# titu1994/tfdiffeq

Hardware: AMD Instinct MI355X
Metric: state-elements/sec (batch x dim / wall-s) Dopri5 float64 (higher is better)
Workload: dtype f64

## Files before the change

include/mi_ode.h:

```cpp
#ifndef MI_ODE_H
#define MI_ODE_H

#include <stddef.h>
#include <stdint.h>

#ifdef __cplusplus
extern "C" {
#endif

#define MI_ODE_ABI_VERSION 13
#define MI_ODE_MAX_STAGES 13
#define MI_ODE_MAX_K (MI_ODE_MAX_STAGES + 1)
#define MI_ODE_MAX_LINCOMB 14
#define MI_ODE_MAX_SEGMENTS 8

#define MI_ODE_OK 0
#define MI_ODE_ST_DT_UNDERFLOW 0x1u
#define MI_ODE_ST_NONFINITE 0x2u
#define MI_ODE_ST_MAX_STEPS 0x4u
#define MI_ODE_ST_SYNC_TIMEOUT 0x10u
#define MI_ODE_ST_BAD_T 0x8u
#define MI_ODE_E_INVALID (-1)
#define MI_ODE_E_HIP (-2)
#define MI_ODE_E_NODEVICE (-3)
// ... 77 lines not shown
  double seg_rtol[MI_ODE_MAX_SEGMENTS], seg_atol[MI_ODE_MAX_SEGMENTS];
  int32_t multistep;
  int32_t ms_max_order;
  int32_t ms_max_iters;
  int32_t ms_min_order;
  const double* ms_ab;
  const double* ms_am;
  const double* ms_am0;
  const double* ms_gamma_star;
} mi_ode_desc;
#define MI_ODE_SEGMENT_ALIGN 256

typedef struct mi_ode_stats {
  int64_t n_attempts, n_accepted, n_rejected, nfe;
  double t, dt;
  double last_ratio;
  uint32_t status;
  int32_t n_polls;
  int64_t n_launches;
  double clock_mhz;
  double handoff_us;
} mi_ode_stats;

typedef struct mi_ode_solver* mi_ode_handle;

int mi_ode_abi_version(void);
const char* mi_ode_status_string(uint32_t status_bits);
const char* mi_ode_last_error(void);
int64_t mi_ode_reduce_workspace_bytes(void);
int64_t mi_ode_sizeof(int32_t which);

int mi_ode_create(const mi_ode_desc* desc, mi_ode_handle* out);
int mi_ode_destroy(mi_ode_handle h);

int mi_ode_begin(mi_ode_handle h, const void* y0_dev, double t0, void* stream);
int mi_ode_advance(mi_ode_handle h, const double* t_out_host, int32_t n_out, void* out_dev, void* stream);
int mi_ode_integrate(mi_ode_handle h, const void* y0_dev, const double* t_host, int32_t T, void* out_dev,
                     mi_ode_stats* stats, void* stream);
int mi_ode_integrate_rows(mi_ode_handle h, const void* rows_plugin, const void* y0_dev, const double* t_host, int32_t T,
                          void* out_dev, int64_t* row_stats_dev, mi_ode_stats* stats, void* stream);
int mi_ode_integrate_rows_t(mi_ode_handle h, const void* rows_t_plugin, const void* y0_dev, const double* t_dev, int32_t T,
                            const int32_t* len_dev, const double* rtol_dev, const double* atol_dev, void* out_dev,
                            int64_t* row_stats_dev, mi_ode_stats* stats, void* stream);
int mi_ode_integrate_fixed_rows_t(mi_ode_handle h, const void* fixed_rows_t_plugin, const void* y0_dev, const double* t_dev, int32_t T,
                                  const int32_t* len_dev, void* out_dev, mi_ode_stats* stats, void* stream);
int mi_ode_fixed_grid_integrate(mi_ode_handle h, const void* y0_dev, const double* t_host, int32_t T,
                                void* out_dev, mi_ode_stats* stats, void* stream);
int mi_ode_fixed_grid_integrate_on(mi_ode_handle h, const void* y0_dev, const double* grid_host, int32_t G,
                                   const double* t_host, int32_t T, double eps, void* out_dev, mi_ode_stats* stats, void* stream);
int mi_ode_rk_step_fused(mi_ode_handle h, const void* y0_dev, const void* f0_dev, double t0, double dt,
                         void* y1_dev, void* f1_dev, double* err_norms_host, void* k_out_dev, void* stream);
int mi_ode_eval_rhs(mi_ode_handle h, const void* y_dev, double t, void* f_dev, void* stream);
int mi_ode_get_stats(mi_ode_handle h, mi_ode_stats* stats, void* stream);
int mi_ode_get_profile(mi_ode_handle h, double* out4);
int mi_ode_get_state(mi_ode_handle h, void* y_dev, void* f_dev, void* stream);

int64_t mi_ode_xrank_bytes(int32_t world_size);
int mi_ode_xrank_selftest(mi_ode_handle h, void* stream);
int mi_ode_xrank_enable(mi_ode_handle h, int32_t on);

#define MI_ODE_IPC_HANDLE_BYTES 64
int mi_ode_xpeer_prepare(mi_ode_handle h, void* ipc_handle_out);
int mi_ode_xpeer_connect(mi_ode_handle h, const void* all_ipc_handles, int32_t world_size);

#define MI_ODE_RCCL_ID_BYTES 128
int mi_ode_rccl_unique_id(void* id_out);
int mi_ode_rccl_connect(mi_ode_handle h, const void* id, int32_t world_size, int32_t rank);

typedef struct mi_ode_adjoint_desc {
  int64_t batch;
  int32_t dim, hidden;
  mi_ode_tableau tableau;
  double rtol, atol;
  double safety, ifactor, dfactor;
  int32_t order, init_order;
  int64_t max_num_steps;
  int32_t time_dependent;
  int32_t reserved;
} mi_ode_adjoint_desc;
typedef struct mi_ode_adjoint* mi_ode_adjoint_handle;
int mi_ode_adjoint_create(const mi_ode_adjoint_desc* desc, mi_ode_adjoint_handle* out);
int mi_ode_adjoint_destroy(mi_ode_adjoint_handle h);
int64_t mi_ode_adjoint_num_params(mi_ode_adjoint_handle h);
int mi_ode_adjoint_segment(mi_ode_adjoint_handle h, const mi_ode_rhs* rhs, const void* y_dev, const void* adj_y_dev,
                           const void* adj_t_dev, const void* adj_params_dev, double t_start, double t_end, void* y_out_dev,
                           void* adj_y_out_dev, void* adj_t_out_dev, void* adj_params_out_dev, mi_ode_stats* stats, void* stream);
int mi_ode_adjoint_dynamics(mi_ode_adjoint_handle h, const mi_ode_rhs* rhs, const void* y_dev, const void* adj_y_dev,
                            void* f_out_dev, void* vjp_y_out_dev, void* vjp_params_out_dev, void* stream);
int mi_ode_adjoint_dynamics_at(mi_ode_adjoint_handle h, const mi_ode_rhs* rhs, double t, const void* y_dev, const void* adj_y_dev,
                               void* f_out_dev, void* vjp_y_out_dev, void* vjp_params_out_dev, void* stream);

int64_t mi_ode_outer_workspace_bytes(int32_t dtype, int64_t batch, int32_t dim);
int mi_ode_outer_reduce(int32_t dtype, int64_t batch, int32_t dim, const void* y_dev, const void* a_dev, double scale,
                        void* out_w_dev, void* out_b_dev, void* workspace_dev, void* stream);

typedef struct mi_ode_linadj_desc {
  int64_t batch;
  int32_t dim;
  int32_t dtype;
  mi_ode_tableau tableau;
  double rtol, atol;
  double safety, ifactor, dfactor;
  int32_t order, init_order;
  int64_t max_num_steps;
} mi_ode_linadj_desc;
typedef struct mi_ode_linadj* mi_ode_linadj_handle;
// ... 267 lines not shown
```

tfdiffeq_amd/_native.py:

```python
import ctypes as C
import os
import subprocess

_HERE = os.path.dirname(os.path.abspath(__file__))
LIB_PATH = os.environ.get('TFDIFFEQ_AMD_LIB') or os.path.join(_HERE, 'libmi_ode.so')
CSRC = os.path.join(_HERE, 'csrc')

MAX_STAGES = 13
MAX_K = MAX_STAGES + 1
MAX_LINCOMB = 14
REC = 8

F32, F64 = 0, 1
RHS_LINEAR, RHS_CUBIC_LINEAR, RHS_LOTKA_VOLTERRA, RHS_LORENZ, RHS_MLP_TANH, RHS_PLUGIN = 1, 2, 3, 4, 5, 6
CTRL_MISC, CTRL_TSIT5 = 0, 1
INTERP_QUARTIC_MID, INTERP_TSIT5, INTERP_TSIT5_REF = 0, 1, 2
ABI_VERSION = 13
MAX_SEGMENTS = 8
SEGMENT_ALIGN = 256
IPC_HANDLE_BYTES = 64
RCCL_ID_BYTES = 128
ST_DT_UNDERFLOW, ST_NONFINITE, ST_MAX_STEPS, ST_BAD_T, ST_SYNC_TIMEOUT = 1, 2, 4, 8, 16
E_INVALID, E_HIP, E_NODEVICE, E_EXCHANGE = -1, -2, -3, -4

# ... 143 lines not shown

class ConvDesc(C.Structure):
    _fields_ = [('dtype', C.c_int32), ('activation', C.c_int32), ('time_dependent', C.c_int32), ('reserved', C.c_int32),
                ('sign', C.c_double), ('batch', C.c_int64),
                ('channels', C.c_int32), ('height', C.c_int32), ('width', C.c_int32), ('filters', C.c_int32),
                ('w1', C.c_void_p), ('b1', C.c_void_p), ('w2', C.c_void_p), ('w2t', C.c_void_p), ('b2', C.c_void_p),
                ('w3', C.c_void_p), ('b3', C.c_void_p)]


class Stats(C.Structure):
    _fields_ = [('n_attempts', C.c_int64), ('n_accepted', C.c_int64), ('n_rejected', C.c_int64), ('nfe', C.c_int64),
                ('t', C.c_double), ('dt', C.c_double), ('last_ratio', C.c_double),
                ('status', C.c_uint32), ('n_polls', C.c_int32), ('n_launches', C.c_int64), ('clock_mhz', C.c_double),
                ('handoff_us', C.c_double)]

    def as_dict(self):
        return {k: getattr(self, k) for k, _ in self._fields_}


_PROTOS = {
    'mi_ode_abi_version': (C.c_int, []),
    'mi_ode_status_string': (C.c_char_p, [C.c_uint32]),
    'mi_ode_last_error': (C.c_char_p, []),
    'mi_ode_reduce_workspace_bytes': (C.c_int64, []),
    'mi_ode_sizeof': (C.c_int64, [C.c_int32]),
    'mi_ode_create': (C.c_int, [C.POINTER(Desc), C.POINTER(C.c_void_p)]),
    'mi_ode_destroy': (C.c_int, [C.c_void_p]),
    'mi_ode_begin': (C.c_int, [C.c_void_p, C.c_void_p, C.c_double, C.c_void_p]),
    'mi_ode_advance': (C.c_int, [C.c_void_p, C.POINTER(C.c_double), C.c_int32, C.c_void_p, C.c_void_p]),
    'mi_ode_integrate': (C.c_int, [C.c_void_p, C.c_void_p, C.POINTER(C.c_double), C.c_int32, C.c_void_p,
                                   C.POINTER(Stats), C.c_void_p]),
    'mi_ode_integrate_rows': (C.c_int, [C.c_void_p, C.c_void_p, C.c_void_p, C.POINTER(C.c_double), C.c_int32, C.c_void_p, C.c_void_p,
                                        C.POINTER(Stats), C.c_void_p]),
    'mi_ode_integrate_rows_t': (C.c_int, [C.c_void_p, C.c_void_p, C.c_void_p, C.c_void_p, C.c_int32, C.c_void_p, C.c_void_p, C.c_void_p,
                                          C.c_void_p, C.c_void_p, C.POINTER(Stats), C.c_void_p]),
    'mi_ode_integrate_fixed_rows_t': (C.c_int, [C.c_void_p, C.c_void_p, C.c_void_p, C.c_void_p, C.c_int32, C.c_void_p, C.c_void_p,
                                                C.POINTER(Stats), C.c_void_p]),
    'mi_ode_fixed_grid_integrate': (C.c_int, [C.c_void_p, C.c_void_p, C.POINTER(C.c_double), C.c_int32, C.c_void_p,
                                              C.POINTER(Stats), C.c_void_p]),
    'mi_ode_fixed_grid_integrate_on': (C.c_int, [C.c_void_p, C.c_void_p, C.POINTER(C.c_double), C.c_int32, C.POINTER(C.c_double), C.c_int32,
                                                 C.c_double, C.c_void_p, C.POINTER(Stats), C.c_void_p]),
    'mi_ode_rk_step_fused': (C.c_int, [C.c_void_p, C.c_void_p, C.c_void_p, C.c_double, C.c_double, C.c_void_p,
                                       C.c_void_p, C.POINTER(C.c_double), C.c_void_p, C.c_void_p]),
    'mi_ode_eval_rhs': (C.c_int, [C.c_void_p, C.c_void_p, C.c_double, C.c_void_p, C.c_void_p]),
    'mi_ode_xrank_bytes': (C.c_int64, [C.c_int32]),
    'mi_ode_xrank_selftest': (C.c_int, [C.c_void_p, C.c_void_p]),
    'mi_ode_xrank_enable': (C.c_int, [C.c_void_p, C.c_int32]),
    'mi_ode_xpeer_prepare': (C.c_int, [C.c_void_p, C.c_void_p]),
    'mi_ode_xpeer_connect': (C.c_int, [C.c_void_p, C.c_void_p, C.c_int32]),
    'mi_ode_rccl_unique_id': (C.c_int, [C.c_void_p]),
    'mi_ode_rccl_connect': (C.c_int, [C.c_void_p, C.c_void_p, C.c_int32, C.c_int32]),
    'mi_ode_get_stats': (C.c_int, [C.c_void_p, C.POINTER(Stats), C.c_void_p]),
    'mi_ode_get_state': (C.c_int, [C.c_void_p, C.c_void_p, C.c_void_p, C.c_void_p]),
    'mi_ode_get_profile': (C.c_int, [C.c_void_p, C.POINTER(C.c_double)]),
    'mi_ode_adjoint_create': (C.c_int, [C.POINTER(AdjointDesc), C.POINTER(C.c_void_p)]),
    'mi_ode_adjoint_destroy': (C.c_int, [C.c_void_p]),
    'mi_ode_adjoint_num_params': (C.c_int64, [C.c_void_p]),
    'mi_ode_adjoint_segment': (C.c_int, [C.c_void_p, C.POINTER(Rhs), C.c_void_p, C.c_void_p, C.c_void_p, C.c_void_p, C.c_double, C.c_double,
                                         C.c_void_p, C.c_void_p, C.c_void_p, C.c_void_p, C.POINTER(Stats), C.c_void_p]),
    'mi_ode_adjoint_dynamics': (C.c_int, [C.c_void_p, C.POINTER(Rhs), C.c_void_p, C.c_void_p, C.c_void_p, C.c_void_p, C.c_void_p,
                                          C.c_void_p]),
    'mi_ode_adjoint_dynamics_at': (C.c_int, [C.c_void_p, C.POINTER(Rhs), C.c_double, C.c_void_p, C.c_void_p, C.c_void_p, C.c_void_p,
                                             C.c_void_p, C.c_void_p]),
    'mi_ode_outer_workspace_bytes': (C.c_int64, [C.c_int32, C.c_int64, C.c_int32]),
    'mi_ode_outer_reduce': (C.c_int, [C.c_int32, C.c_int64, C.c_int32, C.c_void_p, C.c_void_p, C.c_double, C.c_void_p, C.c_void_p,
                                      C.c_void_p, C.c_void_p]),
    'mi_ode_linadj_create': (C.c_int, [C.POINTER(LinAdjDesc), C.POINTER(C.c_void_p)]),
    'mi_ode_linadj_destroy': (C.c_int, [C.c_void_p]),
    'mi_ode_linadj_segment': (C.c_int, [C.c_void_p, C.c_void_p, C.c_void_p, C.c_void_p, C.c_void_p, C.c_void_p, C.c_void_p, C.c_void_p, C.c_double,
                                        C.c_double, C.c_void_p, C.c_void_p, C.c_void_p, C.c_void_p, C.POINTER(C.c_double), C.POINTER(Stats), C.c_void_p]),
    'mi_ode_linadj_profile': (C.c_int, [C.c_void_p, C.POINTER(C.c_double)]),
    'mi_ode_discrete_create': (C.c_int, [C.POINTER(DiscreteDesc), C.POINTER(C.c_void_p)]),
    'mi_ode_discrete_create_td': (C.c_int, [C.POINTER(DiscreteDesc), C.c_int32, C.POINTER(C.c_void_p)]),
    'mi_ode_discrete_destroy': (C.c_int, [C.c_void_p]),
    'mi_ode_discrete_num_params': (C.c_int64, [C.c_void_p]),
    'mi_ode_discrete_sweep': (C.c_int, [C.c_void_p, C.POINTER(Rhs), C.POINTER(C.c_double), C.c_void_p, C.c_void_p, C.c_void_p, C.c_void_p,
                                        C.POINTER(Stats), C.c_void_p]),
    'mi_ode_discrete64_create': (C.c_int, [C.POINTER(DiscreteDesc), C.c_int32, C.POINTER(C.c_void_p)]),
    'mi_ode_discrete64_destroy': (C.c_int, [C.c_void_p]),
    'mi_ode_discrete64_num_params': (C.c_int64, [C.c_void_p]),
    'mi_ode_discrete64_sweep': (C.c_int, [C.c_void_p, C.POINTER(Rhs), C.POINTER(C.c_double), C.c_void_p, C.c_void_p, C.c_void_p, C.c_void_p,
                                          C.POINTER(Stats), C.c_void_p]),
    'mi_ode_discrete64_profile': (C.c_int, [C.c_void_p, C.POINTER(C.c_double)]),
    'mi_ode_discrete_row_sweep': (C.c_int, [C.POINTER(DiscreteRowDesc), C.POINTER(Rhs), C.c_void_p, C.c_void_p, C.c_void_p, C.c_void_p,
                                            C.POINTER(Stats), C.c_void_p]),
    'mi_ode_discrete_row_sweep_t': (C.c_int, [C.POINTER(DiscreteRowTDesc), C.POINTER(Rhs), C.c_void_p, C.c_void_p, C.c_void_p, C.c_void_p,
                                              C.POINTER(Stats), C.c_void_p]),
    'mi_ode_discrete_row_t_sizeof': (C.c_int64, []),
    'mi_ode_adjoint_rows': (C.c_int, [C.POINTER(AdjointRowsDesc), C.POINTER(Rhs), C.c_void_p, C.c_void_p, C.c_void_p, C.c_void_p, C.c_void_p,
                                      C.POINTER(Stats), C.c_void_p]),
    'mi_ode_adjoint_rows_sizeof': (C.c_int64, []),
    'mi_ode_adjoint_rows_t': (C.c_int, [C.POINTER(AdjointRowsTDesc), C.POINTER(Rhs), C.c_void_p, C.c_void_p, C.c_void_p, C.c_void_p,
                                        C.POINTER(Stats), C.c_void_p]),
    'mi_ode_adjoint_rows_t_sizeof': (C.c_int64, []),
    'mi_ode_discrete_linear_create': (C.c_int, [C.POINTER(DiscreteLinearDesc), C.POINTER(C.c_void_p)]),
    'mi_ode_discrete_linear_destroy': (C.c_int, [C.c_void_p]),
    'mi_ode_discrete_linear_sweep': (C.c_int, [C.c_void_p, C.POINTER(Rhs), C.POINTER(C.c_double), C.c_void_p, C.c_void_p, C.c_void_p, C.c_void_p,
                                               C.c_void_p, C.POINTER(Stats), C.c_void_p]),
    'mi_ode_discrete_linear_profile': (C.c_int, [C.c_void_p, C.POINTER(C.c_double)]),
    'mi_ode_discrete_linear_grid_validate': (C.c_int, [C.POINTER(DiscreteLinearGridDesc), C.POINTER(C.c_double), C.POINTER(C.c_int32),
                                                       C.POINTER(C.c_double)]),
    'mi_ode_discrete_linear_grid_create': (C.c_int, [C.POINTER(DiscreteLinearGridDesc), C.POINTER(C.c_void_p)]),
    'mi_ode_discrete_linear_grid_destroy': (C.c_int, [C.c_void_p]),
    'mi_ode_discrete_linear_grid_sweep': (C.c_int, [C.c_void_p, C.POINTER(Rhs), C.POINTER(C.c_double), C.POINTER(C.c_int32), C.POINTER(C.c_double),
                                                    C.c_void_p, C.c_void_p, C.c_void_p, C.c_void_p, C.c_void_p, C.POINTER(Stats), C.c_void_p]),
    'mi_ode_discrete_linear_grid_profile': (C.c_int64, [C.c_void_p, C.POINTER(C.c_double), C.POINTER(C.c_int64)]),
# ... 146 lines not shown
```

tfdiffeq_amd/csrc/mi_ode_api.hip:

```cpp
#include <dlfcn.h>
#include <math.h>
#include <stdarg.h>
#include <stdio.h>
#include <stdlib.h>
#include <string.h>

#include "mi_ode_control.h"
#include "mi_ode_host.h"
#include "mi_ode_plane.h"
#include "mi_ode_step_fused.h"
#include "mi_ode_persist.h"
#include "mi_ode_adams.h"
#include "mi_ode_adams_vc.h"
#include "mi_ode_adams_planes.h"
#include "mi_ode_mlp.h"
#include "mi_ode_plugin.h"

using namespace mi;

static thread_local char g_err[512] = "";

void mi_set_error(const char* fmt, ...) {
  va_list ap;
  va_start(ap, fmt);
  vsnprintf(g_err, sizeof(g_err), fmt, ap);
  va_end(ap);
}

extern "C" const char* mi_ode_last_error(void) { return g_err; }
extern "C" int mi_ode_abi_version(void) { return MI_ODE_ABI_VERSION; }

extern "C" const char* mi_ode_status_string(uint32_t s) {
  if (s & MI_ODE_ST_BAD_T) return "t must be strictly increasing or decrasing";
  if (s & MI_ODE_ST_NONFINITE) return "non-finite values in state `y`";
  if (s & MI_ODE_ST_MAX_STEPS) return "max_num_steps exceeded";
  if (s & MI_ODE_ST_DT_UNDERFLOW) return "underflow in dt";
  if (s & MI_ODE_ST_SYNC_TIMEOUT) return "engine: grid hand-off timed out (whole-integration kernel)";
  return "ok";
}

extern "C" int64_t mi_ode_reduce_workspace_bytes(void) { return (int64_t)kMaxBlocks * kRec * sizeof(double); }
extern "C" int64_t mi_ode_sizeof(int32_t which) {
  switch (which) {
    case 0: return (int64_t)sizeof(mi_ode_desc);
    case 1: return (int64_t)sizeof(mi_ode_stats);
    case 2: return (int64_t)sizeof(mi_ode_tableau);
    case 3: return (int64_t)sizeof(mi_ode_rhs);
    case 4: return (int64_t)sizeof(mi_ode_solver);
    case 5: return (int64_t)sizeof(mi_ode_ctrl_params);
    case 6: return (int64_t)sizeof(mi_ode_adjoint_desc);
    case 7: return (int64_t)sizeof(mi_ode_opq_desc);
    case 8: return (int64_t)sizeof(mi_ode_linadj_desc);
    case 9: return (int64_t)sizeof(mi_ode_discrete_desc);
    case 10: return (int64_t)sizeof(mi_ode_discrete_row_desc);
    case 11: return (int64_t)sizeof(mi_ode_discrete_linear_desc);
    case 12: return (int64_t)sizeof(mi_ode_discrete_linear_grid_desc);
    default: return -1;
  }
}

typedef int (*nccl_get_unique_id_fn)(void*);
// ... 279 lines not shown
      if (!h->d.adaptive && (h->d.multistep != 0 || (h->d.tableau.n_stages != 0 && h->d.tableau.n_stages != 3))) {
        mi_set_error("fused MLP kernels on a fixed grid: euler or rk4 (3/8 rule) in one launch (k_fixed_mlp); no multistep kernel");
        return MI_ODE_E_INVALID;
      }
      if (D < 1 || D > 64 || hd < 1 || hd > 128 || !r.w[0] || !r.w[1] || !r.w[2]) {
        mi_set_error("fused MLP kernel supports dim <= 64, hidden <= 128 (got %d, %d)", D, hd);
        return MI_ODE_E_INVALID;
      }
      h->mlp_dp = D <= 16 ? 16 : 64;
      h->mlp_hp = hd <= 16 ? 16 : 128;
      if (!h->is_f32 && h->mlp_dp != (h->mlp_hp == 16 ? 16 : 64)) { h->mlp_dp = 64; h->mlp_hp = 128; }
      h->family = FAM_MLP; return 0;
    }
    default:
      mi_set_error("RHS kind %d has no fused kernel yet", r.kind);
      return MI_ODE_E_INVALID;
  }
}

static bool multistep_family(const mi_ode_solver* h) {
  const bool rowlocal = h->family == FAM_CUBIC2 || h->family == FAM_LINEAR2 || h->family == FAM_LV || h->family == FAM_LORENZ ||
                        h->family == FAM_PLUGIN;
  const bool coop = (h->family == FAM_LINEAR_MFMA || h->family == FAM_LINEAR_VALU) && h->d.dim >= 1 && h->d.dim <= 256;
  return rowlocal || coop || h->family == FAM_MLP_COOP || h->family == FAM_PLUGIN_COOP;
}
static long long multistep_grid(const mi_ode_solver* h) {
  if (h->family == FAM_LINEAR_MFMA || h->family == FAM_LINEAR_VALU) {
    const long long tpw = 256 / h->d.dim;
    return (h->d.batch + tpw - 1) / tpw;
  }
  if (h->family == FAM_MLP_COOP) {
    const long long tpw = RhsMlpCoop<float>::tpw(h->rhs, (int)h->d.dim);
    return (h->d.batch + tpw - 1) / tpw;
  }
  if (h->family == FAM_PLUGIN_COOP) {
    const long long tpw = 256 / h->d.dim;
    return (h->d.batch + tpw - 1) / tpw;
  }
  return (h->d.batch + 255) / 256;
}
static void multistep_rhs(const mi_ode_solver* h, RhsParams& r) {
  if (h->family == FAM_LINEAR_MFMA || h->family == FAM_LINEAR_VALU) r.hidden = (int)h->d.dim;
  if (h->family == FAM_MLP_COOP) r.cube = (int)h->d.dim;
}

static void fill_step_args(mi_ode_solver* h, StepArgs& A) {
  memset(&A, 0, sizeof(A));
  A.ctl = h->ctl; A.planes = h->planes; A.stride = h->stride; A.batch = h->d.batch; A.dim = (int)h->d.dim;
  A.interp = h->d.interp; A.out = h->cur_out; A.t_out = h->t_out_dev; A.n_plane = h->n;
  fill_tableau(A, h->d.tableau, h->S);
  A.partials = h->partials; A.rhs = h->rhs;
  A.ticket = h->fused_ctl ? h->ticket : nullptr;
  A.cp = h->cp;
}

static void fill_mlp_args(mi_ode_solver* h, MlpArgs& M) {
  memset(&M, 0, sizeof(M));
  fill_step_args(h, M.step);
  M.rtol = h->d.rtol; M.atol = h->d.atol; M.hidden = h->d.rhs.hidden;
}

static void close_peers(mi_ode_solver* h) {
  for (int q = 0; q < h->xpeer_world && q < 64; ++q)
    if (h->xpeer_open[q] != nullptr && h->xpeer_open[q] != h->xpeer_local) (void)hipIpcCloseMemHandle(h->xpeer_open[q]);
  memset(h->xpeer_open, 0, sizeof(h->xpeer_open));
  h->xpeer_world = 0;
  if (h->xpeer_tab_dev) { (void)hipFree(h->xpeer_tab_dev); h->xpeer_tab_dev = nullptr; }
}

extern "C" int mi_ode_destroy(mi_ode_handle h) {
  if (h != nullptr) {
    close_peers(h);
    if (h->xpeer_local) { (void)hipFree(h->xpeer_local); h->xpeer_local = nullptr; }
    if (h->nccl_comm && g_nccl.ok) { (void)g_nccl.destroy(h->nccl_comm); h->nccl_comm = nullptr; }
  }
  if (h != nullptr && h->xrank_registered) { (void)hipHostUnregister(h->d.xrank_host); h->xrank_registered = 0; }
  if (h != nullptr && h->gbuf) { (void)hipFree(h->gbuf); h->gbuf = nullptr; }
  if (h == nullptr) return 0;
  if (h->planes) (void)hipFree(h->planes);
  if (h->partials) (void)hipFree(h->partials);
  if (h->adams_tab) (void)hipFree(h->adams_tab);
  if (h->mlp_pack) (void)hipFree(h->mlp_pack);
  if (h->lin_pack) (void)hipFree(h->lin_pack);
  if (h->adams_res) (void)hipHostFree(h->adams_res);
  if (h->rank_rec && h->own_exchange) (void)hipFree(h->rank_rec);
  if (h->gathered && h->own_exchange) (void)hipFree(h->gathered);
  if (h->ctl) (void)hipFree(h->ctl);
  if (h->ticket) (void)hipFree(h->ticket);
  if (h->t_out_dev) (void)hipFree(h->t_out_dev);
  if (h->ev_ready) for (int i = 0; i < 64; ++i) { (void)hipEventDestroy(h->ev_a[i]); (void)hipEventDestroy(h->ev_b[i]); (void)hipEventDestroy(h->ev_c[i]); }
  if (h->ctl_host) (void)hipHostFree(h->ctl_host);
  if (h->t_out_host) (void)hipHostFree(h->t_out_host);
  delete h;
  return 0;
}

extern "C" int mi_ode_create(const mi_ode_desc* desc, mi_ode_handle* out) {
  if (desc == nullptr || out == nullptr) { mi_set_error("null argument"); return MI_ODE_E_INVALID; }
  *out = nullptr;
  int ndev = 0;
  if (hipGetDeviceCount(&ndev) != hipSuccess || ndev == 0) { mi_set_error("no HIP device"); return MI_ODE_E_NODEVICE; }
  if (desc->dtype != MI_ODE_F32 && desc->dtype != MI_ODE_F64) { mi_set_error("bad dtype"); return MI_ODE_E_INVALID; }
  if (desc->batch <= 0 || desc->dim <= 0) { mi_set_error("empty state"); return MI_ODE_E_INVALID; }
  const mi_ode_tableau& tb = desc->tableau;
  if (tb.n_stages < 0 || tb.n_stages > MI_ODE_MAX_STAGES) { mi_set_error("bad n_stages"); return MI_ODE_E_INVALID; }
  if (desc->adaptive) {
    const bool classic = tb.fsal && (tb.n_stages == 3 || tb.n_stages == 6);
    const bool wide = (tb.fsal && tb.n_stages == 13) || (!tb.fsal && tb.n_stages == 1);
    if (!classic && !wide && desc->multistep != 3) { mi_set_error("fused adaptive engine: no kernels for a %d-row %s tableau", tb.n_stages, tb.fsal ? "FSAL-shaped" : "non-FSAL"); return MI_ODE_E_INVALID; }
    if (desc->interp != MI_ODE_INTERP_QUARTIC_MID && tb.n_stages != 6) { mi_set_error("tsit5 dense output needs 7 stage derivatives"); return MI_ODE_E_INVALID; }
  }
  mi_ode_solver* h = new mi_ode_solver();
  memset(h, 0, sizeof(*h));
  h->d = *desc;
  if (h->d.world_size < 1) h->d.world_size = 1;
  h->is_f32 = desc->dtype == MI_ODE_F32;
  h->elt = h->is_f32 ? 4 : 8;
  h->n = desc->batch * desc->dim;
  h->stride = ((h->n * (long long)h->elt + 255) / 256) * 256;
  h->S = tb.n_stages;
  int dev = 0;
  hipDeviceProp_t prop;
  if (hipGetDevice(&dev) != hipSuccess || hipGetDeviceProperties(&prop, dev) != hipSuccess) {
    mi_set_error("cannot query device");
    mi_ode_destroy(h);
    return MI_ODE_E_HIP;
  }
  h->num_cus = prop.multiProcessorCount;
  fill_rhs(h->rhs, desc->rhs);
  h->rhs.sign = desc->rhs.sign == 0.0 ? 1.0 : desc->rhs.sign;
  int rc = pick_family(h);
  if (rc != 0) { mi_ode_destroy(h); return rc; }
  if (h->family == FAM_LINEAR_MFMA && h->lin_dp == 256) {
    if (hipMalloc(&h->lin_pack, (size_t)256 * 256 * (size_t)h->elt) != hipSuccess) {
      (void)hipGetLastError();
      mi_set_error("linear tile kernels (dim > 128): cannot allocate the copy of W");
// ... 52 lines not shown
      if (g > cap || g > kPersistMaxGrid) {
        mi_set_error("adams in one launch: %lld workgroups cannot be co-resident on this device (%d)", g, cap);
        mi_ode_destroy(h); return MI_ODE_E_INVALID;
      }
    }
    memcpy(h->adams_gamma_star, desc->ms_gamma_star, sizeof(h->adams_gamma_star));
    hipError_t ea = hipHostMalloc((void**)&h->adams_res, 4 * sizeof(long long), hipHostMallocDefault);
    if (ea != hipSuccess) { mi_set_error("multistep result record: %s", hipGetErrorString(ea)); mi_ode_destroy(h); return MI_ODE_E_HIP; }
    for (int i = 0; i < 4; ++i) h->adams_res[i] = 0;
    h->d.ms_gamma_star = nullptr;
  } else
  if (desc->multistep != 0) {
    const bool rowlocal_cat = multistep_family(h);
    if (desc->adaptive || !rowlocal_cat || (desc->multistep != 1 && desc->multistep != 2) || desc->ms_ab == nullptr || desc->ms_am == nullptr ||
        desc->ms_am0 == nullptr || desc->ms_max_order < 1 || desc->ms_max_order > kAdamsMaxOrder || desc->ms_max_iters < 1 ||
        desc->ms_min_order < 1 || h->d.world_size > 1 || h->nseg > 1) {
      mi_set_error("multistep: fixed grid, a row-local catalogue system or a matrix RHS of dim <= 256, one rank, one tensor; 1 <= max_order <= %d, max_iters >= 1, coefficient tables", kAdamsMaxOrder);
      mi_ode_destroy(h); return MI_ODE_E_INVALID;
    }
    const long long g = multistep_grid(h);
    if (desc->multistep == 2 && g > 1) {
      const int cap = h->is_f32 ? mi_adams_capacity_f32(h) : mi_adams_capacity_f64(h);
      if (g > cap || g > kPersistMaxGrid) {
        mi_set_error("fixed_adams in one launch: %lld workgroups cannot be co-resident on this device (%d)", g, cap);
        mi_ode_destroy(h); return MI_ODE_E_INVALID;
      }
    }
    double tab[2 * 13 * 12 + 13];
    memcpy(tab, desc->ms_ab, sizeof(double) * 13 * 12);
    memcpy(tab + 13 * 12, desc->ms_am, sizeof(double) * 13 * 12);
    memcpy(tab + 2 * 13 * 12, desc->ms_am0, sizeof(double) * 13);
    hipError_t ea = hipMalloc((void**)&h->adams_tab, sizeof(tab));
    if (ea == hipSuccess) ea = hipMemcpy(h->adams_tab, tab, sizeof(tab), hipMemcpyHostToDevice);
    if (ea == hipSuccess) ea = hipHostMalloc((void**)&h->adams_res, 2 * sizeof(long long), hipHostMallocDefault);
    if (ea != hipSuccess) { mi_set_error("multistep tables: %s", hipGetErrorString(ea)); mi_ode_destroy(h); return MI_ODE_E_HIP; }
    h->adams_res[0] = h->adams_res[1] = 0;
    h->d.ms_ab = h->d.ms_am = h->d.ms_am0 = nullptr;
  }
  {
    const bool can = desc->adaptive && (h->family == FAM_CUBIC2 || h->family == FAM_LINEAR2 || h->family == FAM_LV ||
                                        h->family == FAM_LORENZ || h->family == FAM_LINEAR_MFMA || h->family == FAM_MLP ||
                                        h->family == FAM_PLUGIN);
    if (h->family == FAM_PLUGIN && desc->fusion == 1) { mi_set_error("RHS plugins have no per-stage kernels (fusion = 1)"); mi_ode_destroy(h); return MI_ODE_E_INVALID; }
    if (h->family == FAM_MLP && desc->fusion == 1) { mi_set_error("the MLP family only has a whole-attempt kernel"); mi_ode_destroy(h); return MI_ODE_E_INVALID; }
    const bool can_fixed = !desc->adaptive && (h->family == FAM_CUBIC2 || h->family == FAM_LINEAR2 || h->family == FAM_LV ||
                                               h->family == FAM_LORENZ || h->family == FAM_LINEAR_MFMA || h->family == FAM_MLP ||
                                               h->family == FAM_PLUGIN);
    if (desc->fusion == 2 && !can && !can_fixed) { mi_set_error("fusion=2: no whole-attempt kernel for this problem"); mi_ode_destroy(h); return MI_ODE_E_INVALID; }
    h->step_fused = (can && desc->fusion != 1) ? 1 : 0;
    h->ts_dense = (desc->interp != MI_ODE_INTERP_QUARTIC_MID) ? 1 : 0;
    const bool light_many = (h->family != FAM_LINEAR_MFMA && h->family != FAM_MLP) && h->step_grid > 32;
    h->fused_ctl = (h->step_fused && h->d.world_size <= 1 && desc->allgather == nullptr && desc->fusion != 3 &&
                    !(light_many && desc->fusion == 0)) ? 1 : 0;
  }
  {
    const bool rowlocal = h->family == FAM_CUBIC2 || h->family == FAM_LINEAR2 || h->family == FAM_LV || h->family == FAM_LORENZ ||
                          h->family == FAM_PLUGIN;
    const bool mfma = h->family == FAM_LINEAR_MFMA && h->step_fused;
    const bool mlp = h->family == FAM_MLP;
    const bool coop = (h->family == FAM_MLP_COOP || h->family == FAM_PLUGIN_COOP) && desc->multistep == 0;
    h->init_tiles16 = mfma ? 1 : 0;
    long long g = (mfma || mlp) ? (long long)h->step_grid : coop ? multistep_grid(h) : (desc->batch + 255) / 256;
    const bool single = h->d.world_size <= 1 && desc->allgather == nullptr;
    if (desc->xrank_host != nullptr) {
      if (h->d.world_size > kXMaxWorld || desc->xrank_bytes < mi_ode_xrank_bytes(h->d.world_size)) {
        mi_set_error("xrank_host: world_size <= %d and at least %lld bytes are needed", kXMaxWorld, (long long)mi_ode_xrank_bytes(h->d.world_size));
        mi_ode_destroy(h); return MI_ODE_E_INVALID;
      }
      void* dptr = nullptr;
      hipError_t re = hipHostRegister(desc->xrank_host, (size_t)desc->xrank_bytes, hipHostRegisterMapped | hipHostRegisterPortable);
      if (re == hipSuccess) { h->xrank_registered = 1; re = hipHostGetDevicePointer(&dptr, desc->xrank_host, 0); }
      if (re != hipSuccess) {
        (void)hipGetLastError();
        if (h->xrank_registered) { (void)hipHostUnregister(desc->xrank_host); h->xrank_registered = 0; }
        dptr = nullptr;
      }
      h->xrank_dev = (double*)dptr;
    }
    const bool clamp_ok = mfma && single && (double)((desc->batch + 15) / 16) * (double)h->lin_dp * (double)h->lin_dp <= 8.0e6;
    if (clamp_ok && g > kPersistMaxGrid) g = kPersistMaxGrid;
    bool capable = desc->adaptive && (rowlocal || mfma || mlp || coop) && g <= kPersistMaxGrid;
    if (capable) {
      const int cap = mlp ? (h->is_f32 ? mi_persist_capacity_mlp_f32(h) : mi_persist_capacity_mlp_f64(h))
                          : (h->is_f32 ? mi_persist_capacity_f32(h) : mi_persist_capacity_f64(h));
      if (clamp_ok && cap > 0 && g > cap) g = cap;
      capable = cap > 0 && g <= cap;
    }
    if (!capable && desc->adaptive && (rowlocal || coop)) {
      h->persist_planes = 1;
      h->persist_planes_block = 256;
      if (const char* eb = getenv("MI_ODE_PERSIST_PLANES_BLOCK")) { const int v = atoi(eb); if ((v == 256 || v == 512) && !coop) h->persist_planes_block = v; }
      const int cap = h->is_f32 ? mi_persist_capacity_f32(h) : mi_persist_capacity_f64(h);
      long long gp = cap < kPersistMaxGrid ? cap : kPersistMaxGrid;
      if (gp > h->num_cus && !coop) gp = h->num_cus;
      if (const char* eg = getenv("MI_ODE_PERSIST_PLANES_GRID")) { const long long v = atoll(eg); if (v >= 1 && v <= gp) gp = v; }
      const long long gneed = coop ? multistep_grid(h) : (desc->batch + h->persist_planes_block - 1) / h->persist_planes_block;
      if (gp > gneed) gp = gneed;
      if (h->nseg > 1 && gp < h->nseg) gp = 0;
      if (cap > 0 && gp >= 1) { capable = true; g = gp; }
      else h->persist_planes = 0;
      if (h->persist_planes && h->nseg > 1) {
        long long total = 0;
        for (int k = 0; k < h->nseg; ++k) total += desc->seg_rows[k];
        int used = 0;
        for (int k = 0; k < h->nseg; ++k) {
          long long share = (long long)((double)g * (double)desc->seg_rows[k] / (double)total);
          const long long need = (desc->seg_rows[k] + h->persist_planes_block - 1) / h->persist_planes_block;
          if (share > need) share = need;
          if (share < 1) share = 1;
          const int left_for_rest = h->nseg - 1 - k;
          if (used + share > g - left_for_rest) share = g - left_for_rest - used;
          h->seg_blk[k] = used;
          used += (int)share;
        }
        h->seg_blk[h->nseg] = used;
        g = used;
      }
    }
    h->persist_capable = capable ? 1 : 0;
    const bool can = capable && (single || h->xrank_dev != nullptr);
    if (desc->fusion == 4 && !can && single) { mi_set_error("fusion=4: no whole-integration kernel for this problem (row-local or MFMA-linear RHS, single rank, every workgroup co-resident)"); mi_ode_destroy(h); return MI_ODE_E_INVALID; }
    h->persist = (can && (desc->fusion == 4 || desc->fusion == 0)) ? 1 : 0;
    if (coop && desc->adaptive && !h->persist) {
      mi_set_error("cooperative kernel: %lld workgroups cannot be co-resident on this device (the whole-call kernel is its only schedule)", g);
      mi_ode_destroy(h); return MI_ODE_E_INVALID;
    }
    if (h->nseg > 1 && !h->persist) {
      mi_set_error("tuple states run on the whole-call kernel only, and its grid (%lld workgroups) is not co-resident on this device", g);
      mi_ode_destroy(h); return MI_ODE_E_INVALID;
    }
    h->persist_grid = (int)g;
    h->persist_sleep_first = g <= 32 ? 16 : 32;
    h->persist_sleep_poll = 2;
    if (const char* e0 = getenv("MI_ODE_PERSIST_SLEEP0")) h->persist_sleep_first = atoi(e0);
    if (const char* e1 = getenv("MI_ODE_PERSIST_SLEEP1")) h->persist_sleep_poll = atoi(e1);
    h->persist_spin_limit = 1 << 17;
    h->persist_spin_first = 1 << 12;
    if (const char* e3 = getenv("MI_ODE_PERSIST_SPIN_FIRST")) h->persist_spin_first = atoi(e3);
    if (const char* e2 = getenv("MI_ODE_PERSIST_SPIN_LIMIT")) h->persist_spin_limit = atoi(e2);
    h->persist_xspin_limit = 1 << 22;
    if (const char* e4 = getenv("MI_ODE_PERSIST_XSPIN_LIMIT")) h->persist_xspin_limit = atoi(e4);
    if (getenv("MI_ODE_PERSIST_SPIN_LIMIT") && !getenv("MI_ODE_PERSIST_XSPIN_LIMIT")) h->persist_xspin_limit = h->persist_spin_limit;
  }
  h->cp.rtol = desc->rtol; h->cp.atol = desc->atol;
  h->cp.safety = desc->safety; h->cp.ifactor = desc->ifactor; h->cp.dfactor = desc->dfactor;
  h->cp.inv_ifactor = 1.0 / desc->ifactor; h->cp.inv_dfactor = 1.0 / desc->dfactor;
  h->cp.max_num_steps = desc->max_num_steps > 0 ? desc->max_num_steps : 2147483647LL;
  h->cp.n_local = h->n;
  h->cp.order = desc->order; h->cp.init_order = desc->init_order;
  h->cp.controller = desc->controller;
  h->cp.is_f32 = h->is_f32;
  h->cp.n_stages = h->S;
  h->cp.auto_first_step = isnan(desc->first_step) ? 1 : 0;
  h->ip.kind = desc->interp;
  h->ip.nk = h->S + 1;
  for (int j = 0; j < kMaxK; ++j) h->ip.c_mid[j] = tb.c_mid[j];
  hipError_t e = hipSuccess;
  e = hipMalloc((void**)&h->planes, (size_t)h->stride * (2 + h->S + 1));
  if (e == hipSuccess) e = hipMalloc((void**)&h->partials, (size_t)kMaxBlocks * kRec * sizeof(double));
  if (e == hipSuccess) e = hipMemset(h->partials, 0, (size_t)kMaxBlocks * kRec * sizeof(double));
  if (desc->exchange_send_dev != nullptr && desc->exchange_recv_dev != nullptr) {
    h->rank_rec = desc->exchange_send_dev;
    h->gathered = desc->exchange_recv_dev;
    h->own_exchange = 0;
  } else {
    h->own_exchange = 1;
    if (e == hipSuccess) e = hipMalloc((void**)&h->rank_rec, kRec * sizeof(double));
    if (e == hipSuccess) e = hipMalloc((void**)&h->gathered, (size_t)h->d.world_size * kRec * sizeof(double));
  }
  if (e == hipSuccess) e = hipMalloc((void**)&h->ctl, sizeof(Ctl));
  if (e == hipSuccess) e = hipMalloc((void**)&h->gbuf, 2 * kPRec * sizeof(double));
  if (e == hipSuccess) e = hipMemset(h->gbuf, 0, 2 * kPRec * sizeof(double));
  if (e == hipSuccess) e = hipMalloc((void**)&h->ticket, 64);
  if (e == hipSuccess) e = hipMemset(h->ticket, 0, 64);
  if (e == hipSuccess) e = hipHostMalloc((void**)&h->ctl_host, sizeof(Ctl), hipHostMallocDefault);
  if (e != hipSuccess) {
    mi_set_error("workspace allocation failed: %s", hipGetErrorString(e));
    mi_ode_destroy(h);
    return MI_ODE_E_HIP;
  }
  memset(h->ctl_host, 0, sizeof(Ctl));
  if (h->d.profile) {
    for (int i = 0; i < 64 && e == hipSuccess; ++i) {
      e = hipEventCreate(&h->ev_a[i]);
      if (e == hipSuccess) e = hipEventCreate(&h->ev_b[i]);
      if (e == hipSuccess) e = hipEventCreate(&h->ev_c[i]);
    }
    if (e != hipSuccess) { mi_set_error("event creation failed"); mi_ode_destroy(h); return MI_ODE_E_HIP; }
    h->ev_ready = 1;
  }
  *out = h;
  return 0;
}

static int ensure_t_out(mi_ode_solver* h, int n) {
  if (n > h->t_out_cap) {
    if (h->t_out_dev) (void)hipFree(h->t_out_dev);
    h->t_out_dev = nullptr;
    int cap = n < 64 ? 64 : n;
    MI_HIP(hipMalloc((void**)&h->t_out_dev, (size_t)cap * sizeof(double)));
    h->t_out_cap = cap;
  }
  if (n > h->t_out_host_cap) {
    if (h->t_out_host) (void)hipHostFree(h->t_out_host);
    h->t_out_host = nullptr;
    int cap = n < 64 ? 64 : n;
    MI_HIP(hipHostMalloc((void**)&h->t_out_host, (size_t)cap * sizeof(double), hipHostMallocDefault));
    h->t_out_host_cap = cap;
  }
  return 0;
}

static int begin_impl(mi_ode_handle h, const void* y0_dev, double t0, void* first_out_dev, void* stream);

extern "C" int mi_ode_begin(mi_ode_handle h, const void* y0_dev, double t0, void* stream) {
  return begin_impl(h, y0_dev, t0, nullptr, stream);
}

static int begin_impl(mi_ode_handle h, const void* y0_dev, double t0, void* first_out_dev, void* stream) {
  if (h == nullptr || y0_dev == nullptr) { mi_set_error("null argument"); return MI_ODE_E_INVALID; }
  if (!h->d.adaptive) { mi_set_error("mi_ode_begin on a fixed-grid handle"); return MI_ODE_E_INVALID; }
  if (h->d.multistep != 0) { mi_set_error("multistep handles run through mi_ode_integrate / mi_ode_fixed_grid_integrate only"); return MI_ODE_E_INVALID; }
  if (h->nseg > 1) { mi_set_error("tuple states: mi_ode_integrate with at least two times only (whole-call kernel)"); return MI_ODE_E_INVALID; }
  hipStream_t st = (hipStream_t)stream;
  MI_HIP(hipStreamSynchronize(st));
  Ctl* c = h->ctl_host;
  memset(c, 0, sizeof(Ctl));
  c->t0 = c->t1 = t0;
  c->dt = h->cp.auto_first_step ? 0.0 : h->d.first_step;
  c->idx_y0 = 0; c->idx_y1 = 1;
  for (int j = 0; j < kMaxK; ++j) c->idx_k[j] = 2 + j;
  h->n_launches = 0; h->n_polls = 0;
  h->enq_attempts = 0; h->prof_done = 0;
  MI_HIP(hipMemcpyAsync(h->ctl, c, sizeof(Ctl), hipMemcpyHostToDevice, st));
  if (h->family == FAM_MLP) {
    MlpArgs M;
    fill_mlp_args(h, M);
    M.x_y0 = y0_dev; M.copy_a = h->planes; M.copy_b = first_out_dev;
    int rcm = h->is_f32 ? mi_launch_mlp_f32(h, MLP_F0, M, st) : mi_launch_mlp_f64(h, MLP_F0, M, st);
    if (rcm != 0) return rcm;
    rcm = enqueue_controller(h, PH_F0, st);
    if (rcm != 0) return rcm;
    if (h->cp.auto_first_step) {
      fill_mlp_args(h, M);
      rcm = h->is_f32 ? mi_launch_mlp_f32(h, MLP_INITB, M, st) : mi_launch_mlp_f64(h, MLP_INITB, M, st);
      if (rcm != 0) return rcm;
      rcm = enqueue_controller(h, PH_INITB, st);
      if (rcm != 0) return rcm;
    }
    h->begun = 1;
    return 0;
  }
  if (h->init_tiles16) {
    InitArgs I;
    memset(&I, 0, sizeof(I));
    fill_step_args(h, I.s);
    I.y0 = y0_dev; I.copy_b = first_out_dev;
    int rci = h->is_f32 ? mi_launch_init_linear_f32(h, 0, I, st) : mi_launch_init_linear_f64(h, 0, I, st);
    if (rci != 0) return rci;
    rci = enqueue_controller(h, PH_F0, st);
    if (rci != 0) return rci;
    if (h->cp.auto_first_step) {
      rci = h->is_f32 ? mi_launch_init_linear_f32(h, 1, I, st) : mi_launch_init_linear_f64(h, 1, I, st);
      if (rci != 0) return rci;
      rci = enqueue_controller(h, PH_INITB, st);
      if (rci != 0) return rci;
    }
    h->begun = 1;
    return 0;
  }
  StageArgs A;
  fill_common(h, A);
  A.explicit_mode = 1; A.ctl = nullptr;
  A.x_y0 = y0_dev; A.x_t0 = t0; A.x_dt = 0.0;
  A.x_kout = h->planes + 2 * h->stride;
  A.copy_a = h->planes;
  A.copy_b = first_out_dev;
  int rc = launch_stage(h, M_F0, 0, A, st);
  if (rc != 0) return rc;
  rc = enqueue_controller(h, PH_F0, st);
  if (rc != 0) return rc;
  if (h->cp.auto_first_step) {
    fill_common(h, A);
    A.k_out_slot = 1;
    A.alpha = 1.0;
    rc = launch_stage(h, M_INITB, 1, A, st);
    if (rc != 0) return rc;
    rc = enqueue_controller(h, PH_INITB, st);
    if (rc != 0) return rc;
  }
  h->begun = 1;
  return 0;
}

extern "C" int mi_ode_advance(mi_ode_handle h, const double* t_out_host, int32_t n_out, void* out_dev, void* stream) {
  if (h == nullptr || (n_out > 0 && (t_out_host == nullptr || out_dev == nullptr))) { mi_set_error("null argument"); return MI_ODE_E_INVALID; }
  if (h->d.multistep != 0) { mi_set_error("multistep handles run through mi_ode_integrate / mi_ode_fixed_grid_integrate only"); return MI_ODE_E_INVALID; }
  if (!h->begun) { mi_set_error("mi_ode_advance before mi_ode_begin"); return MI_ODE_E_INVALID; }
  hipStream_t st = (hipStream_t)stream;
  if (n_out <= 0) return 0;
  for (int i = 1; i < n_out; ++i)
    if (!(t_out_host[i] > t_out_host[i - 1])) { mi_set_error("output times must increase"); return MI_ODE_ST_BAD_T; }
  int rc = ensure_t_out(h, n_out);
  if (rc != 0) return rc;
  if (h->t_out_busy) { MI_HIP(hipStreamSynchronize(st)); h->t_out_busy = 0; }
  memcpy(h->t_out_host, t_out_host, (size_t)n_out * sizeof(double));
  MI_HIP(hipMemcpyAsync(h->t_out_dev, h->t_out_host, (size_t)n_out * sizeof(double), hipMemcpyHostToDevice, st));
  h->cp.t_out = h->t_out_dev;
  h->cur_out = out_dev;
  MI_HIP(hipMemsetAsync(h->ticket, 0, 4, st));
// ... 267 lines not shown
      mi_set_error("hipIpcOpenMemHandle(rank %d) failed: %s", q, hipGetErrorString(e));
      close_peers(h);
      return MI_ODE_E_HIP;
    }
    h->xpeer_open[q] = p;
  }
  hipError_t e = hipMalloc((void**)&h->xpeer_tab_dev, (size_t)kXMaxWorld * sizeof(double*));
  if (e == hipSuccess) e = hipMemcpy(h->xpeer_tab_dev, h->xpeer_open, (size_t)world_size * sizeof(double*), hipMemcpyHostToDevice);
  if (e != hipSuccess) { mi_set_error("peer table upload failed: %s", hipGetErrorString(e)); close_peers(h); return MI_ODE_E_HIP; }
  return 0;
}

extern "C" int mi_ode_rccl_unique_id(void* id_out) {
  if (id_out == nullptr) { mi_set_error("null argument"); return MI_ODE_E_INVALID; }
  int rc = load_rccl();
  if (rc != 0) return rc;
  NcclUniqueId id;
  memset(&id, 0, sizeof(id));
  const int nrc = g_nccl.get_id(&id);
  if (nrc != 0) { mi_set_error("ncclGetUniqueId failed: %s", g_nccl.err ? g_nccl.err(nrc) : "?"); return MI_ODE_E_EXCHANGE; }
  memcpy(id_out, &id, sizeof(id));
  return 0;
}

extern "C" int mi_ode_rccl_connect(mi_ode_handle h, const void* id, int32_t world_size, int32_t rank) {
  if (h == nullptr) { mi_set_error("null argument"); return MI_ODE_E_INVALID; }
  if (id == nullptr) {
    if (h->nccl_comm && g_nccl.ok) (void)g_nccl.destroy(h->nccl_comm);
    h->nccl_comm = nullptr;
    return 0;
  }
  if (world_size != h->d.world_size || rank != h->d.rank) { mi_set_error("rccl_connect: world_size / rank differ from the handle's"); return MI_ODE_E_INVALID; }
  int rc = load_rccl();
  if (rc != 0) return rc;
  if (h->nccl_comm) { (void)g_nccl.destroy(h->nccl_comm); h->nccl_comm = nullptr; }
  NcclUniqueId uid;
  memcpy(&uid, id, sizeof(uid));
  void* comm = nullptr;
  const int nrc = g_nccl.init_rank(&comm, world_size, uid, rank);
  if (nrc != 0 || comm == nullptr) { mi_set_error("ncclCommInitRank failed: %s", g_nccl.err ? g_nccl.err(nrc) : "?"); return MI_ODE_E_EXCHANGE; }
  h->nccl_comm = comm;
  h->fused_ctl = 0;
  return 0;
}

extern "C" int mi_ode_get_stats(mi_ode_handle h, mi_ode_stats* stats, void* stream) {
  if (h == nullptr || stats == nullptr) { mi_set_error("null argument"); return MI_ODE_E_INVALID; }
  int rc = poll_ctl(h, (hipStream_t)stream);
  if (rc != 0) return rc;
  fill_stats(h, stats);
  return 0;
}

extern "C" int mi_ode_get_profile(mi_ode_handle h, double* out4) {
  if (h == nullptr || out4 == nullptr) { mi_set_error("null argument"); return MI_ODE_E_INVALID; }
  out4[0] = h->prof_last_ms; out4[1] = (double)h->prof_n; out4[2] = h->prof_all_ms; out4[3] = (double)h->prof_n;
  return 0;
}

extern "C" int mi_ode_get_state(mi_ode_handle h, void* y_dev, void* f_dev, void* stream) {
  if (h == nullptr) { mi_set_error("null argument"); return MI_ODE_E_INVALID; }
  if (h->d.multistep != 0) { mi_set_error("get_state: the one-launch multistep kernels keep their state in registers (the solution rows are the output)"); return MI_ODE_E_INVALID; }
  hipStream_t st = (hipStream_t)stream;
  int rc = poll_ctl(h, st);
  if (rc != 0) return rc;
  const Ctl* c = h->ctl_host;
  if (y_dev) MI_HIP(hipMemcpyAsync(y_dev, h->planes + (long long)c->idx_y0 * h->stride, (size_t)h->n * h->elt, hipMemcpyDeviceToDevice, st));
  if (f_dev) MI_HIP(hipMemcpyAsync(f_dev, h->planes + (long long)c->idx_k[0] * h->stride, (size_t)h->n * h->elt, hipMemcpyDeviceToDevice, st));
  return 0;
}

static int fixed_impl(mi_ode_handle h, const void* y0_dev, const double* grid_host, int32_t G, const double* t_host, int32_t T, double eps,
                      void* out_dev, mi_ode_stats* stats, void* stream);

extern "C" int mi_ode_fixed_grid_integrate(mi_ode_handle h, const void* y0_dev, const double* t_host, int32_t T,
                                           void* out_dev, mi_ode_stats* stats, void* stream) {
  return fixed_impl(h, y0_dev, t_host, T, t_host, T, 0.0, out_dev, stats, stream);
}

extern "C" int mi_ode_fixed_grid_integrate_on(mi_ode_handle h, const void* y0_dev, const double* grid_host, int32_t G,
                                              const double* t_host, int32_t T, double eps, void* out_dev, mi_ode_stats* stats,
                                              void* stream) {
  if (grid_host == nullptr || G < 1) { mi_set_error("bad grid"); return MI_ODE_E_INVALID; }
  return fixed_impl(h, y0_dev, grid_host, G, t_host, T, eps, out_dev, stats, stream);
}

static int fixed_impl(mi_ode_handle h, const void* y0_dev, const double* grid_host, int32_t G, const double* t_host, int32_t T, double eps,
                      void* out_dev, mi_ode_stats* stats, void* stream) {
  if (h == nullptr || y0_dev == nullptr || t_host == nullptr || out_dev == nullptr || T < 1) { mi_set_error("bad argument"); return MI_ODE_E_INVALID; }
  if (h->d.adaptive) { mi_set_error("fixed-grid call on an adaptive handle"); return MI_ODE_E_INVALID; }
  hipStream_t st = (hipStream_t)stream;
  const bool euler = h->S == 0;
  if (!euler && h->S != 3 && h->d.multistep == 0) { mi_set_error("fixed grid: tableau must be euler (0 rows) or rk4 3/8 (3 rows)"); return MI_ODE_E_INVALID; }
  for (int i = 1; i < T; ++i)
    if (!(t_host[i] > t_host[i - 1])) {
      if (stats) { memset(stats, 0, sizeof(*stats)); stats->status = MI_ODE_ST_BAD_T; }
      return MI_ODE_ST_BAD_T;
    }
  const bool own_grid = grid_host != t_host || eps != 0.0;
  if (own_grid) {
    for (int i = 1; i < G; ++i)
      if (!(grid_host[i] > grid_host[i - 1])) { mi_set_error("the time grid must increase"); return MI_ODE_ST_BAD_T; }
    if (!(grid_host[0] == t_host[0] && grid_host[G - 1] == t_host[T - 1])) {
      mi_set_error("the time grid must start at t[0] and end at t[-1]");
      return MI_ODE_ST_BAD_T;
    }
  }
  h->n_launches = 0; h->n_polls = 0;
  const size_t pbytes = (size_t)h->n * h->elt;
  if (h->d.multistep != 0 && (h->d.fusion == 1 || !multistep_family(h))) {
    mi_set_error("multistep handles run on the one-launch kernels only");
    return MI_ODE_E_INVALID;
  }
  if ((h->family == FAM_CUBIC2 || h->family == FAM_LINEAR2 || h->family == FAM_LV || h->family == FAM_LORENZ ||
       h->family == FAM_LINEAR_MFMA || h->family == FAM_MLP || h->family == FAM_PLUGIN ||
       h->family == FAM_MLP_COOP || h->family == FAM_PLUGIN_COOP || (h->family == FAM_LINEAR_VALU && h->d.multistep != 0)) && h->d.fusion != 1) {
    int rcf = ensure_t_out(h, T + (own_grid ? G : 0));
    if (rcf != 0) return rcf;
    MI_HIP(hipStreamSynchronize(st));
    memcpy(h->t_out_host, t_host, (size_t)T * sizeof(double));
// ... 432 lines not shown
```

tfdiffeq_amd/csrc/mi_ode_ctrl_dev.h:

```cpp
#pragma once
#include "mi_ode_dev.h"

namespace mi {

template <bool SC1>
__device__ __forceinline__ double rec_load(const double* p) {
  if constexpr (SC1) return __hip_atomic_load(p, __ATOMIC_RELAXED, __HIP_MEMORY_SCOPE_AGENT);
  else return *p;
}

template <bool SC1 = false>
__device__ __forceinline__ void reduce_block_records(const double* part, int nblocks, double* out ) {
  if (threadIdx.x < 64) {
    double v0 = 0, v1 = 0, v2 = 0, v3 = 0, v4 = 0;
    for (int b = threadIdx.x; b < nblocks; b += 64) {
      const double* p = part + (long long)b * kRec;
      v0 = fmax(v0, rec_load<SC1>(p + R_MAXA)); v1 = fmax(v1, rec_load<SC1>(p + R_MAXB));
      v2 += rec_load<SC1>(p + R_SUMA); v3 += rec_load<SC1>(p + R_SUMB); v4 = fmax(v4, rec_load<SC1>(p + R_FLAG));
    }
    v0 = wave_max(v0); v1 = wave_max(v1); v2 = wave_sum(v2); v3 = wave_sum(v3); v4 = wave_max(v4);
    if (threadIdx.x == 0) {
      out[R_MAXA] = v0; out[R_MAXB] = v1; out[R_SUMA] = v2; out[R_SUMB] = v3; out[R_FLAG] = v4;
      out[R_N] = 0; out[6] = 0; out[7] = 0;
    }
  }
}

__device__ __forceinline__ double nan_min(double a, double b) { return (isnan(a) || isnan(b)) ? NAN : fmin(a, b); }
__device__ __forceinline__ double nan_max(double a, double b) { return (isnan(a) || isnan(b)) ? NAN : fmax(a, b); }

__device__ __forceinline__ double optimal_step(double last_step, double ratio, const CtrlParams& P) {
  if (ratio == 0.0) return last_step * P.ifactor;
  const double inv_dfac = (ratio < 1.0) ? 1.0 : P.inv_dfactor;
  double er, expo;
  if (P.controller == MI_ODE_CTRL_TSIT5) {
    er = ratio;
    expo = 1.0 / (double)P.order;
  } else {
    er = P.is_f32 ? (double)sqrtf((float)ratio) : sqrt(ratio);
    expo = (double)(float)(1.0 / (double)P.order);
  }
  const double factor = nan_max(P.inv_ifactor, nan_min(pow(er, expo) / P.safety, inv_dfac));
  return last_step / factor;
}

struct AttemptState {
  double t0, t1, dt, ratio, emit_t0, emit_t1, emit_dt;
  long long n_attempt, n_accept, n_reject, nfe, n_steps_out;
  int next_out, n_out, emit_lo, emit_hi, done, accepted;
  unsigned status;
  __device__ __forceinline__ void load(const Ctl& c) {
    t0 = c.t0; t1 = c.t1; dt = c.dt; ratio = c.ratio; emit_t0 = c.emit_t0; emit_t1 = c.emit_t1; emit_dt = c.emit_dt;
    n_attempt = c.n_attempt; n_accept = c.n_accept; n_reject = c.n_reject; nfe = c.nfe; n_steps_out = c.n_steps_out;
    next_out = c.next_out; n_out = c.n_out; emit_lo = c.emit_lo; emit_hi = c.emit_hi; done = c.done; accepted = c.accepted;
    status = c.status;
  }
  __device__ __forceinline__ void store(Ctl& c) const {
    c.t0 = t0; c.t1 = t1; c.dt = dt; c.ratio = ratio; c.emit_t0 = emit_t0; c.emit_t1 = emit_t1; c.emit_dt = emit_dt;
    c.n_attempt = n_attempt; c.n_accept = n_accept; c.n_reject = n_reject; c.nfe = nfe; c.n_steps_out = n_steps_out;
    c.next_out = next_out; c.n_out = n_out; c.emit_lo = emit_lo; c.emit_hi = emit_hi; c.done = done; c.accepted = accepted;
    c.status = status;
  }
};

__device__ __forceinline__ double error_ratio(const double* rec, const CtrlParams& P) {
  const double N = rec[R_N];
  if (P.is_f32) {
    const float tol = (float)P.atol + (float)P.rtol * (float)fmax(rec[R_MAXA], rec[R_MAXB]);
    return (double)(float)(rec[R_SUMA] / (N * (double)tol * (double)tol));
  }
  const double tol = P.atol + P.rtol * fmax(rec[R_MAXA], rec[R_MAXB]);
  return rec[R_SUMA] / (N * tol * tol);
}

__device__ __forceinline__ void attempt_tail(AttemptState& c, double ratio, bool accept, const CtrlParams& P) {
  c.n_attempt += 1;
  c.nfe += P.n_stages;
  c.n_steps_out += 1;
  const double dt = c.dt, t_start = c.t1;
  c.ratio = ratio;
  const double dt_next = optimal_step(dt, ratio, P);
  c.accepted = accept ? 1 : 0;
  c.emit_lo = c.emit_hi = c.next_out;
  if (accept) {
    c.n_accept += 1;
    const double t_new = t_start + dt;
    c.emit_t0 = t_start; c.emit_t1 = t_new; c.emit_dt = dt;
    c.t0 = t_start; c.t1 = t_new;
    int nx = c.next_out;
    while (nx < c.n_out && !(P.t_out[nx] > t_new)) ++nx;
    if (nx > c.next_out) { c.emit_hi = nx; c.next_out = nx; c.n_steps_out = 0; }
  } else {
    c.n_reject += 1;
    c.t0 = t_start;
  }
  c.dt = dt_next;
  if (c.next_out >= c.n_out) { c.done = 1; return; }
  if (c.n_steps_out >= P.max_num_steps) { c.status |= MI_ODE_ST_MAX_STEPS; c.done = 1; return; }
  if (!(c.t1 + dt_next > c.t1)) { c.status |= MI_ODE_ST_DT_UNDERFLOW; c.done = 1; }
}

__device__ __forceinline__ void attempt_core(AttemptState& c, const double* rec, const CtrlParams& P) {
  const double ratio = error_ratio(rec, P);
  attempt_tail(c, ratio, ratio <= 1.0, P);
}

constexpr int kMaxSeg = MI_ODE_MAX_SEGMENTS;
struct SegState { double d1[kMaxSeg]; };

__device__ __forceinline__ double py_max(const double* v, int n) {
  double best = v[0];
  for (int i = 1; i < n; ++i)
    if (v[i] > best) best = v[i];
  return best;
}

__device__ __forceinline__ void controller_apply_seg(Ctl* c, SegState* ss, const double (*rec)[kRec], int nseg, int phase, const CtrlParams& P) {
  if (phase == PH_F0) {
    c->nfe += 1;
    double d0[kMaxSeg], d1[kMaxSeg], q[kMaxSeg];
    bool nonfinite = false;
    for (int k = 0; k < nseg; ++k) {
      const double N = rec[k][R_N];
      nonfinite = nonfinite || rec[k][R_FLAG] != 0.0;
      if (P.is_f32) {
        d0[k] = (double)(sqrtf((float)rec[k][R_SUMA]) / powf((float)N, 0.5f));
        d1[k] = (double)(sqrtf((float)rec[k][R_SUMB]) / powf((float)N, 0.5f));
        q[k] = (double)((float)d0[k] / (float)d1[k]);
      } else {
        d0[k] = sqrt(rec[k][R_SUMA]) / pow(N, 0.5);
        d1[k] = sqrt(rec[k][R_SUMB]) / pow(N, 0.5);
        q[k] = d0[k] / d1[k];
      }
      ss->d1[k] = d1[k];
    }
    c->y0_nonfinite = nonfinite;
    const double m0 = py_max(d0, nseg), m1 = py_max(d1, nseg);
    double h0;
    if (P.is_f32) h0 = ((float)m0 < 1e-5f || (float)m1 < 1e-5f) ? (double)1e-6f : (double)(0.01f * (float)py_max(q, nseg));
    else h0 = (m0 < 1e-5 || m1 < 1e-5) ? 1e-6 : 0.01 * py_max(q, nseg);
    c->d0 = d0[0]; c->d1 = d1[0]; c->h0 = h0;
    return;
  }
  if (phase == PH_INITB) {
    c->nfe += 1;
    double both[2 * kMaxSeg], d2[kMaxSeg];
    for (int k = 0; k < nseg; ++k) {
      const double N = rec[k][R_N];
      if (P.is_f32) d2[k] = (double)((sqrtf((float)rec[k][R_SUMA]) / powf((float)N, 0.5f)) / (float)c->h0);
      else d2[k] = (sqrt(rec[k][R_SUMA]) / pow(N, 0.5)) / c->h0;
      both[k] = ss->d1[k]; both[nseg + k] = d2[k];
    }
    double first;
    if (P.is_f32) {
      const float h0 = (float)c->h0;
      float h1;
      if ((float)py_max(ss->d1, nseg) <= 1e-15f && (float)py_max(d2, nseg) <= 1e-15f) h1 = (float)nan_max((double)1e-6f, (double)(h0 * 1e-3f));
      else h1 = powf(0.01f / (float)py_max(both, 2 * nseg), (float)(1.0 / (double)(P.init_order + 1)));
      first = nan_min((double)(100.0f * h0), (double)h1);
    } else {
      const double h0 = c->h0;
      double h1;
      if (py_max(ss->d1, nseg) <= 1e-15 && py_max(d2, nseg) <= 1e-15) h1 = nan_max(1e-6, h0 * 1e-3);
      else h1 = pow(0.01 / py_max(both, 2 * nseg), 1.0 / (double)(P.init_order + 1));
      first = nan_min(100.0 * h0, h1);
    }
    c->dt = first;
    return;
  }
}

__device__ __forceinline__ void attempt_core_seg(AttemptState& c, const double (*rec)[kRec], int nseg, const CtrlParams& P,
                                                 const double* seg_rtol, const double* seg_atol) {
  if (P.controller == MI_ODE_CTRL_TSIT5) {
    double num = 0.0, den = 0.0;
    for (int k = 0; k < nseg; ++k) {
      double tol;
      if (P.is_f32) tol = (double)((float)P.atol + (float)P.rtol * (float)fmax(rec[k][R_MAXA], rec[k][R_MAXB]));
      else tol = P.atol + P.rtol * fmax(rec[k][R_MAXA], rec[k][R_MAXB]);
      num += rec[k][R_SUMA] / (tol * tol);
      den += rec[k][R_N];
    }
    const double ratio = P.is_f32 ? (double)(float)(num / den) : num / den;
    attempt_tail(c, ratio, ratio <= 1.0, P);
    return;
  }
  double ratios[kMaxSeg];
  bool accept = true;
  for (int k = 0; k < nseg; ++k) {
    CtrlParams Pk = P;
    if (seg_rtol != nullptr) { Pk.rtol = seg_rtol[k]; Pk.atol = seg_atol[k]; }
    ratios[k] = error_ratio(rec[k], Pk);
    accept = accept && (ratios[k] <= 1.0);
  }
  attempt_tail(c, py_max(ratios, nseg), accept, P);
}

__device__ __forceinline__ void controller_apply(Ctl* c, const double* rec, int phase, const CtrlParams& P) {
  const double N = rec[R_N];

  if (phase == PH_F0) {
    c->nfe += 1;
    c->y0_nonfinite = rec[R_FLAG] != 0.0;
    double d0, d1, h0;
    if (P.is_f32) {
      const float f0 = sqrtf((float)rec[R_SUMA]) / powf((float)N, 0.5f);
      const float f1 = sqrtf((float)rec[R_SUMB]) / powf((float)N, 0.5f);
      const float h = (f0 < 1e-5f || f1 < 1e-5f) ? 1e-6f : 0.01f * (f0 / f1);
      d0 = f0; d1 = f1; h0 = h;
    } else {
      d0 = sqrt(rec[R_SUMA]) / pow(N, 0.5);
      d1 = sqrt(rec[R_SUMB]) / pow(N, 0.5);
      h0 = (d0 < 1e-5 || d1 < 1e-5) ? 1e-6 : 0.01 * (d0 / d1);
    }
    c->d0 = d0; c->d1 = d1; c->h0 = h0;
    return;
  }
  if (phase == PH_INITB) {
    c->nfe += 1;
    double first;
    if (P.is_f32) {
      const float h0 = (float)c->h0, d1 = (float)c->d1;
      const float d2 = (sqrtf((float)rec[R_SUMA]) / powf((float)N, 0.5f)) / h0;
      float h1;
      if (d1 <= 1e-15f && d2 <= 1e-15f) h1 = fmaxf(1e-6f, h0 * 1e-3f);
      else h1 = powf(0.01f / fmaxf(d1, d2), (float)(1.0 / (double)(P.init_order + 1)));
      first = (double)fminf(100.0f * h0, h1);
    } else {
      const double h0 = c->h0, d1 = c->d1;
      const double d2 = (sqrt(rec[R_SUMA]) / pow(N, 0.5)) / h0;
      double h1;
      if (d1 <= 1e-15 && d2 <= 1e-15) h1 = fmax(1e-6, h0 * 1e-3);
      else h1 = pow(0.01 / fmax(d1, d2), 1.0 / (double)(P.init_order + 1));
      first = fmin(100.0 * h0, h1);
    }
    c->dt = first;
    return;
  }

  AttemptState a;
  a.load(*c);
  attempt_core(a, rec, P);
  if (a.accepted) {
    c->emit_y0 = c->idx_y0; c->emit_y1 = c->idx_y1;
    for (int j = 0; j <= P.n_stages; ++j) c->emit_k[j] = c->idx_k[j];
    const int iy = c->idx_y0; c->idx_y0 = c->idx_y1; c->idx_y1 = iy;
    const int ik = c->idx_k[0]; c->idx_k[0] = c->idx_k[P.n_stages]; c->idx_k[P.n_stages] = ik;
  }
  a.store(*c);
}

}
```

tfdiffeq_amd/csrc/mi_ode_dev.h:

```cpp
#pragma once
#include <hip/hip_runtime.h>
#include <stdint.h>
#include "../../include/mi_ode.h"

#ifndef MI_LIN_FMA
#define MI_LIN_FMA 1
#endif

namespace mi {

template <bool FMA, typename T>
__device__ __forceinline__ T madd(T c, T k, T acc) {
  if constexpr (FMA) {
    if constexpr (sizeof(T) == 8) return __builtin_fma(c, k, acc);
    else return __builtin_fmaf(c, k, acc);
  } else {
    return acc + c * k;
  }
}
template <typename T>
__device__ __forceinline__ T lin_madd(T c, T k, T acc) { return madd<(MI_LIN_FMA != 0), T>(c, k, acc); }

constexpr int kMaxK = MI_ODE_MAX_K;
constexpr int kNumPlanes = 2 + kMaxK;
constexpr int kMaxBlocks = 2048;
constexpr int kRec = 8;
enum { R_MAXA = 0, R_MAXB = 1, R_SUMA = 2, R_SUMB = 3, R_FLAG = 4, R_N = 5 };

struct Ctl {
  double t0, t1, dt;
  double h0, d0, d1;
  double ratio;
  double emit_t0, emit_t1, emit_dt;
  long long n_attempt, n_accept, n_reject, nfe, n_steps_out;
  int idx_y0, idx_y1;
  int idx_k[kMaxK];
  int emit_y0, emit_y1, emit_k[kMaxK];
  int emit_lo, emit_hi;
  int next_out, n_out;
  int done;
  unsigned status;
  int y0_nonfinite;
  int accepted;
  long long prof[4];
  long long clk_cycles, clk_ticks;
};

enum Mode {
  M_STAGE = 0,
  M_LAST_FSAL = 1,
  M_F0 = 2,
  M_INITB = 3,
  M_FX_EULER = 4,
  M_FX_RK4_2 = 5,
  M_FX_RK4_3 = 6,
  M_FX_RK4_4 = 7
};

struct RhsParams {
  double s[8];
  const void* w[3];
  const void* b[3];
  double sign;
  int hidden;
  int cube;
};

struct StageArgs {
  Ctl* ctl;
  char* planes;
  long long stride;
  const void* x_y0;
  void* x_y1;
  const void* x_k[kMaxK];
  void* x_kout;
  double x_t0, x_dt;
  int explicit_mode;
  int k_out_slot;
  long long batch;
  int dim;
  int pad_;
  double a[kMaxK];
  double e[kMaxK + 1];
  double alpha;
  double rtol, atol;
  double* partials;
  void* copy_a;
  void* copy_b;
  RhsParams rhs;
};

template <typename T>
struct Resolved {
  const T* y0;
  T* y1;
  const T* k[kMaxK];
  T* k_out;
  T hs;
// ... 119 lines not shown
  for (int off = 32; off > 0; off >>= 1) v = fmax(v, __shfl_down(v, off, 64));
  return v;
}

__device__ __forceinline__ void block_reduce_thread0(const Acc& a, double* red, double (&r)[5]) {
  const int lane = threadIdx.x & 63, wave = threadIdx.x >> 6, nw = (blockDim.x + 63) >> 6;
  double v0 = wave_max(a.maxa), v1 = wave_max(a.maxb), v2 = wave_sum(a.suma), v3 = wave_sum(a.sumb);
  double v4 = wave_max((double)a.flag);
  __syncthreads();
  if (lane == 0) {
    red[wave] = v0; red[16 + wave] = v1; red[32 + wave] = v2; red[48 + wave] = v3; red[64 + wave] = v4;
  }
  __syncthreads();
  r[0] = r[1] = r[2] = r[3] = r[4] = 0;
  if (threadIdx.x == 0) {
    for (int w = 0; w < nw; ++w) {
      r[0] = fmax(r[0], red[w]); r[1] = fmax(r[1], red[16 + w]); r[2] += red[32 + w]; r[3] += red[48 + w];
      r[4] = fmax(r[4], red[64 + w]);
    }
  }
}

template <bool SC1 = false>
__device__ __forceinline__ void block_reduce_store(const Acc& a, double* red, double* rec_out) {
  double r[5];
  block_reduce_thread0(a, red, r);
  if (threadIdx.x == 0) {
    if constexpr (SC1) {
      __hip_atomic_store(rec_out + R_MAXA, r[0], __ATOMIC_RELAXED, __HIP_MEMORY_SCOPE_AGENT);
      __hip_atomic_store(rec_out + R_MAXB, r[1], __ATOMIC_RELAXED, __HIP_MEMORY_SCOPE_AGENT);
      __hip_atomic_store(rec_out + R_SUMA, r[2], __ATOMIC_RELAXED, __HIP_MEMORY_SCOPE_AGENT);
      __hip_atomic_store(rec_out + R_SUMB, r[3], __ATOMIC_RELAXED, __HIP_MEMORY_SCOPE_AGENT);
      __hip_atomic_store(rec_out + R_FLAG, r[4], __ATOMIC_RELAXED, __HIP_MEMORY_SCOPE_AGENT);
    } else {
      rec_out[R_MAXA] = r[0]; rec_out[R_MAXB] = r[1]; rec_out[R_SUMA] = r[2]; rec_out[R_SUMB] = r[3];
      rec_out[R_FLAG] = r[4]; rec_out[R_N] = 0; rec_out[6] = 0; rec_out[7] = 0;
    }
  }
}

enum Phase { PH_F0 = 0, PH_INITB = 1, PH_ATTEMPT = 2 };

struct CtrlParams {
  double rtol, atol, safety, ifactor, dfactor;
  double inv_ifactor, inv_dfactor;
  long long max_num_steps;
  long long n_local;
  int order, init_order;
  int controller;
  int is_f32;
  int n_stages;
  int auto_first_step;
  const double* t_out;
};

struct InterpParams {
  int kind;
  int nk;
  double c_mid[MI_ODE_MAX_LINCOMB];
};

}
```

tfdiffeq_amd/csrc/mi_ode_host.h:

```cpp
#pragma once
#include <hip/hip_runtime.h>
#include "mi_ode_dev.h"
namespace mi { struct AdamsArgs; struct AdamsVcArgs; }

namespace mi {
struct StepArgs;
struct MlpArgs;
struct FixedArgs;
struct PersistArgs;
struct InitArgs;

enum Family {
  FAM_NONE = 0,
  FAM_CUBIC2,
  FAM_LINEAR2,
  FAM_LV,
  FAM_LORENZ,
  FAM_LINEAR_VALU,
  FAM_LINEAR_MFMA,
  FAM_MLP,
  FAM_PLUGIN,
  FAM_MLP_COOP,
  FAM_PLUGIN_COOP
};
// ... 16 lines not shown
  size_t elt;
  long long n;
  long long stride;
  int S;
  int num_cus;
  char* planes;
  double* partials;
  double* rank_rec;
  double* gathered;
  mi::Ctl* ctl;
  unsigned* ticket;
  int fused_ctl;
  double* t_out_dev;
  void* cur_out;
  int t_out_cap;
  mi::Ctl* ctl_host;
  double* t_out_host;
  int t_out_host_cap;
  int t_out_busy;
  int stage_grid, stage_block;
  int step_fused;
  int step_grid, step_block;
  int persist;
  int persist_planes;
  int persist_planes_block;
  int persist_capable;
  int persist_grid;
  int persist_sleep_first, persist_sleep_poll;
  int persist_spin_limit;
  int persist_xspin_limit;
  int persist_spin_first;
  int init_tiles16;
  double* xrank_dev;
  double* gbuf;
  int xrank_on;
  int xrank_registered;
  void* xpeer_local;
  void* xpeer_open[64];
  double** xpeer_tab_dev;
  int xpeer_world;
  void* nccl_comm;
  unsigned xrank_tests;
  unsigned seq;
  int ts_dense;
  int mlp_dp, mlp_hp;
  double* mlp_pack;
  int nseg;
  int seg_blk[MI_ODE_MAX_SEGMENTS + 1];
  double* adams_tab;
  long long* adams_res;
  double adams_gamma_star[13];
  int lin_dp;
  void* lin_pack;
  long long n_launches;
  int n_polls;
  int begun;
  long long last_call_attempts;
  int own_exchange;
  hipEvent_t ev_a[64], ev_b[64], ev_c[64];
  int ev_ready;
  long long enq_attempts;
  long long prof_done;
  double prof_last_ms, prof_all_ms;
  long long prof_n;
  mi::RhsParams rhs;
  mi::CtrlParams cp;
  mi::InterpParams ip;
};

int mi_launch_stage_f64(mi_ode_solver* h, int mode, int nk, mi::StageArgs& A, hipStream_t st);
int mi_launch_stage_f32(mi_ode_solver* h, int mode, int nk, mi::StageArgs& A, hipStream_t st);
int mi_launch_step_f64(mi_ode_solver* h, mi::StepArgs& A, hipStream_t st);
int mi_launch_step_f32(mi_ode_solver* h, mi::StepArgs& A, hipStream_t st);
int mi_launch_fixed_f64(mi_ode_solver* h, mi::FixedArgs& A, hipStream_t st);
int mi_launch_adams_f64(mi_ode_solver* h, mi::AdamsArgs& A, int grid, hipStream_t st);
int mi_launch_adams_f32(mi_ode_solver* h, mi::AdamsArgs& A, int grid, hipStream_t st);
int mi_adams_capacity_f64(mi_ode_solver* h);
int mi_launch_adams_vc_f64(mi_ode_solver* h, mi::AdamsVcArgs& A, int grid, hipStream_t st);
int mi_launch_adams_vc_f32(mi_ode_solver* h, mi::AdamsVcArgs& A, int grid, hipStream_t st);
int mi_adams_vc_capacity_f64(mi_ode_solver* h);
int mi_adams_vc_capacity_f32(mi_ode_solver* h);
int mi_adams_capacity_f32(mi_ode_solver* h);
int mi_launch_fixed_f32(mi_ode_solver* h, mi::FixedArgs& A, hipStream_t st);
int mi_launch_persist_f64(mi_ode_solver* h, mi::PersistArgs& A, int grid, hipStream_t st);
int mi_launch_persist_f32(mi_ode_solver* h, mi::PersistArgs& A, int grid, hipStream_t st);
int mi_launch_init_linear_f64(mi_ode_solver* h, int phase, mi::InitArgs& I, hipStream_t st);
int mi_launch_init_linear_f32(mi_ode_solver* h, int phase, mi::InitArgs& I, hipStream_t st);
int mi_persist_capacity_f64(mi_ode_solver* h);
int mi_persist_capacity_f32(mi_ode_solver* h);
int mi_launch_persist_mlp_f32(mi_ode_solver* h, mi::PersistArgs& A, int grid, hipStream_t st);
int mi_persist_capacity_mlp_f32(mi_ode_solver* h);
int mi_launch_mlp_f32(mi_ode_solver* h, int mode, mi::MlpArgs& M, hipStream_t st);
int mi_launch_fixed_mlp_f32(mi_ode_solver* h, mi::FixedArgs& A, hipStream_t st);
int mi_launch_persist_mlp_f64(mi_ode_solver* h, mi::PersistArgs& A, int grid, hipStream_t st);
int mi_persist_capacity_mlp_f64(mi_ode_solver* h);
int mi_launch_mlp_f64(mi_ode_solver* h, int mode, mi::MlpArgs& M, hipStream_t st);
int mi_launch_fixed_mlp_f64(mi_ode_solver* h, mi::FixedArgs& A, hipStream_t st);
int mi_mlp64_pack_doubles(int dp, int hp);
int mi_stage_geometry_f64(mi_ode_solver* h);
int mi_stage_geometry_f32(mi_ode_solver* h);

void mi_set_error(const char* fmt, ...);
#define MI_HIP(call)                                                                     \
  do {                                                                                   \
    hipError_t e_ = (call);                                                              \
    if (e_ != hipSuccess) {                                                              \
      mi_set_error("%s failed: %s (%s:%d)", #call, hipGetErrorString(e_), __FILE__, __LINE__); \
      return MI_ODE_E_HIP;                                                               \
    }                                                                                    \
  } while (0)

namespace mi {

template <class Args>
inline void fill_tableau(Args& A, const mi_ode_tableau& tb, int S) {
  for (int i = 0; i < S; ++i) {
    A.alpha[i] = tb.alpha[i];
    for (int j = 0; j <= i; ++j) A.beta[i][j] = tb.beta[i][j];
  }
  for (int j = 0; j <= S; ++j) { A.e[j] = tb.c_error[j]; A.cmid[j] = tb.c_mid[j]; A.csol[j] = tb.c_sol[j]; }
}

template <class Desc>
inline void fill_ctrl(CtrlParams& cp, const Desc& d, long long n_local, int is_f32, int n_stages) {
  cp.rtol = d.rtol; cp.atol = d.atol; cp.safety = d.safety; cp.ifactor = d.ifactor; cp.dfactor = d.dfactor;
  cp.inv_ifactor = 1.0 / d.ifactor; cp.inv_dfactor = 1.0 / d.dfactor;
  cp.max_num_steps = d.max_num_steps > 0 ? d.max_num_steps : 2147483647LL;
  cp.n_local = n_local;
  cp.order = d.order; cp.init_order = d.init_order;
  cp.controller = MI_ODE_CTRL_MISC; cp.is_f32 = is_f32; cp.n_stages = n_stages; cp.auto_first_step = 1;
}

inline void fill_rhs(RhsParams& r, const mi_ode_rhs& rhs) {
  for (int i = 0; i < 8; ++i) r.s[i] = rhs.scalars[i];
  for (int i = 0; i < 3; ++i) { r.w[i] = rhs.w[i]; r.b[i] = rhs.b[i]; }
  r.hidden = rhs.hidden;
}

}
```

tfdiffeq_amd/csrc/mi_ode_launch.inc:

```
#include <stdio.h>
#include <stdlib.h>
#include "mi_ode_host.h"
#include "mi_ode_stage_linear.h"
#include "mi_ode_stage_rowlocal.h"
#include "mi_ode_step_fused.h"
#include "mi_ode_persist.h"
#include "mi_ode_adams.h"
#include "mi_ode_adams_vc.h"
#include "mi_ode_plugin.h"

namespace {
using namespace mi;
typedef MI_T T;

bool lin_streamed(const mi_ode_solver* h) { return h->family == FAM_LINEAR_MFMA && h->lin_dp == 256; }
int lin_pack(mi_ode_solver* h, RhsParams& r, hipStream_t st) {
  if (!lin_streamed(h)) return 0;
  if (h->lin_pack == nullptr) { mi_set_error("linear tile kernels (dim > 128): no copy of W"); return MI_ODE_E_INVALID; }
  hipLaunchKernelGGL((k_lin_pack<T, 256>), dim3(64), dim3(256), 0, st, (const T*)h->rhs.w[0], (int)h->d.dim, (T*)h->lin_pack);
  if (hipGetLastError() != hipSuccess) { mi_set_error("k_lin_pack launch failed"); return MI_ODE_E_HIP; }
  r.w[0] = h->lin_pack;
  return 0;
}
template <class Fn>
void lin_allow_lds(Fn fn, size_t lds) {
  if (lds > 64 * 1024 && hipFuncSetAttribute((const void*)fn, hipFuncAttributeMaxDynamicSharedMemorySize, (int)lds) != hipSuccess) (void)hipGetLastError();
}

template <int D, int NK, int MODE>
int launch_mfma(mi_ode_solver* h, StageArgs& A, hipStream_t st) {
  auto kern = k_stage_linear_mfma<T, D, NK, MODE, false>;
  const size_t lds = linear_mfma_lds_bytes<T, D, MODE>();
  static bool attr_set = false;
  if (!attr_set) {
    if (lds > 48 * 1024)
      MI_HIP(hipFuncSetAttribute((const void*)kern, hipFuncAttributeMaxDynamicSharedMemorySize, (int)lds));
    attr_set = true;
  }
  hipLaunchKernelGGL(kern, dim3(h->stage_grid), dim3(D * 4), lds, st, A);
  return 0;
}

template <int NK, int MODE>
int launch_combo(mi_ode_solver* h, StageArgs& A, hipStream_t st) {
  const dim3 grid(h->stage_grid), block(h->stage_block);
  switch (h->family) {
    case FAM_CUBIC2:
      hipLaunchKernelGGL((k_stage_rowlocal<T, NK, MODE, RhsCubic2<T>>), grid, block, 0, st, A);
      break;
    case FAM_LINEAR2:
      hipLaunchKernelGGL((k_stage_rowlocal<T, NK, MODE, RhsLinear2<T>>), grid, block, 0, st, A);
      break;
    case FAM_LV:
      hipLaunchKernelGGL((k_stage_rowlocal<T, NK, MODE, RhsLotkaVolterra<T>>), grid, block, 0, st, A);
      break;
    case FAM_LORENZ:
      hipLaunchKernelGGL((k_stage_rowlocal<T, NK, MODE, RhsLorenz<T>>), grid, block, 0, st, A);
      break;
    case FAM_LINEAR_MFMA:
      if (A.dim == h->lin_dp && h->lin_dp <= 128) {
        switch (A.dim) {
          case 16: return launch_mfma<16, NK, MODE>(h, A, st);
          case 32: return launch_mfma<32, NK, MODE>(h, A, st);
          case 64: return launch_mfma<64, NK, MODE>(h, A, st);
          case 128: return launch_mfma<128, NK, MODE>(h, A, st);
          default: mi_set_error("MFMA linear kernel: unsupported dim %d", A.dim); return MI_ODE_E_INVALID;
        }
      }
      [[fallthrough]];
    case FAM_LINEAR_VALU: {
      int p2 = 1;
      while (p2 < A.dim) p2 <<= 1;
      const size_t lds = (size_t)(256 / p2) * A.dim * sizeof(T);
      hipLaunchKernelGGL((k_stage_linear_valu<T, NK, MODE>), grid, block, lds, st, A, p2);
      break;
    }
    default:
      mi_set_error("no fused stage kernel for this RHS family");
      return MI_ODE_E_INVALID;
  }
  return 0;
}

template <int D, int S, bool TS>
int launch_step_mfma(mi_ode_solver* h, StepArgs& A, hipStream_t st) {
  const size_t lds = step_linear_lds_bytes<T, D>();
  if constexpr (D == 256) {
    StepArgs B = A;
    const int rc = lin_pack(h, B.rhs, st);
    if (rc != 0) return rc;
    lin_allow_lds(k_step_linear_mfma<T, D, S, TS>, lds);
    hipLaunchKernelGGL((k_step_linear_mfma<T, D, S, TS>), dim3(h->step_grid), dim3(D * 4), lds, st, B);
  } else {
    hipLaunchKernelGGL((k_step_linear_mfma<T, D, S, TS>), dim3(h->step_grid), dim3(D * 4), lds, st, A);
  }
  return 0;
}

template <int S, bool FSAL>
int launch_step_wide(mi_ode_solver* h, StepArgs& A, hipStream_t st) {
  const dim3 grid(h->step_grid), block(h->step_block);
  switch (h->family) {
    case FAM_CUBIC2: hipLaunchKernelGGL((k_step_rowlocal<T, S, false, RhsCubic2<T>, FSAL>), grid, block, 0, st, A); break;
    case FAM_LINEAR2: hipLaunchKernelGGL((k_step_rowlocal<T, S, false, RhsLinear2<T>, FSAL>), grid, block, 0, st, A); break;
    case FAM_LV: hipLaunchKernelGGL((k_step_rowlocal<T, S, false, RhsLotkaVolterra<T>, FSAL>), grid, block, 0, st, A); break;
    case FAM_LORENZ: hipLaunchKernelGGL((k_step_rowlocal<T, S, false, RhsLorenz<T>, FSAL>), grid, block, 0, st, A); break;
    case FAM_LINEAR_MFMA:
      if constexpr (FSAL && S > 1) {
        switch (h->lin_dp) {
          case 16: return launch_step_mfma<16, S, false>(h, A, st);
          case 32: return launch_step_mfma<32, S, false>(h, A, st);
          case 64: return launch_step_mfma<64, S, false>(h, A, st);
          case 128: return launch_step_mfma<128, S, false>(h, A, st);
          default: break;
        }
      }
      mi_set_error("no whole-attempt tile kernel for this tableau / dim"); return MI_ODE_E_INVALID;
    default: mi_set_error("no whole-attempt kernel for a %d-row tableau in this RHS family", S); return MI_ODE_E_INVALID;
  }
  return 0;
}

template <int S, bool FSAL>
const void* persist_fn_wide(const mi_ode_solver* h) {
  switch (h->family) {
    case FAM_CUBIC2: return (const void*)k_persist_rowlocal<T, S, false, RhsCubic2<T>, FSAL>;
    case FAM_LINEAR2: return (const void*)k_persist_rowlocal<T, S, false, RhsLinear2<T>, FSAL>;
    case FAM_LV: return (const void*)k_persist_rowlocal<T, S, false, RhsLotkaVolterra<T>, FSAL>;
    case FAM_LORENZ: return (const void*)k_persist_rowlocal<T, S, false, RhsLorenz<T>, FSAL>;
    case FAM_MLP_COOP: return (const void*)k_persist_rowlocal<T, S, false, RhsMlpCoop<T>, FSAL>;
    default: return nullptr;
  }
}

template <int S, bool TS>
int launch_step(mi_ode_solver* h, StepArgs& A, hipStream_t st) {
  const dim3 grid(h->step_grid), block(h->step_block);
  switch (h->family) {
    case FAM_CUBIC2: hipLaunchKernelGGL((k_step_rowlocal<T, S, TS, RhsCubic2<T>>), grid, block, 0, st, A); break;
    case FAM_LINEAR2: hipLaunchKernelGGL((k_step_rowlocal<T, S, TS, RhsLinear2<T>>), grid, block, 0, st, A); break;
    case FAM_LV: hipLaunchKernelGGL((k_step_rowlocal<T, S, TS, RhsLotkaVolterra<T>>), grid, block, 0, st, A); break;
    case FAM_LORENZ: hipLaunchKernelGGL((k_step_rowlocal<T, S, TS, RhsLorenz<T>>), grid, block, 0, st, A); break;
    case FAM_LINEAR_MFMA:
      switch (h->lin_dp) {
        case 16: return launch_step_mfma<16, S, TS>(h, A, st);
        case 32: return launch_step_mfma<32, S, TS>(h, A, st);
        case 64: return launch_step_mfma<64, S, TS>(h, A, st);
        case 128: return launch_step_mfma<128, S, TS>(h, A, st);
        case 256: return launch_step_mfma<256, S, TS>(h, A, st);
        default: mi_set_error("step kernel: unsupported dim %d", A.dim); return MI_ODE_E_INVALID;
      }
    default:
      mi_set_error("no whole-attempt kernel for this RHS family");
      return MI_ODE_E_INVALID;
  }
  return 0;
}

template <int S, bool TS>
const void* persist_fn(const mi_ode_solver* h) {
  switch (h->family) {
    case FAM_CUBIC2: return (const void*)k_persist_rowlocal<T, S, TS, RhsCubic2<T>>;
    case FAM_LINEAR2: return (const void*)k_persist_rowlocal<T, S, TS, RhsLinear2<T>>;
    case FAM_LV: return (const void*)k_persist_rowlocal<T, S, TS, RhsLotkaVolterra<T>>;
    case FAM_LORENZ: return (const void*)k_persist_rowlocal<T, S, TS, RhsLorenz<T>>;
    case FAM_MLP_COOP: return (const void*)k_persist_rowlocal<T, S, TS, RhsMlpCoop<T>>;
    default: return nullptr;
  }
}

template <int S, bool TS, bool FSAL>
const void* persist_planes_fn(const mi_ode_solver* h) {
  switch (h->family) {
    case FAM_CUBIC2: return (const void*)k_persist_rowlocal_planes<T, S, TS, RhsCubic2<T>, FSAL>;
    case FAM_LINEAR2: return (const void*)k_persist_rowlocal_planes<T, S, TS, RhsLinear2<T>, FSAL>;
    case FAM_LV: return (const void*)k_persist_rowlocal_planes<T, S, TS, RhsLotkaVolterra<T>, FSAL>;
    case FAM_LORENZ: return (const void*)k_persist_rowlocal_planes<T, S, TS, RhsLorenz<T>, FSAL>;
    case FAM_MLP_COOP: return (const void*)k_persist_rowlocal_planes<T, S, TS, RhsMlpCoop<T>, FSAL>;
    default: return nullptr;
  }
}

template <int S, bool TS>
const void* persist_fn_mfma(const mi_ode_solver* h) {
  switch (h->lin_dp) {
    case 16: return (const void*)k_persist_linear_mfma<T, 16, S, TS>;
    case 32: return (const void*)k_persist_linear_mfma<T, 32, S, TS>;
    case 64: return (const void*)k_persist_linear_mfma<T, 64, S, TS>;
    case 128: return (const void*)k_persist_linear_mfma<T, 128, S, TS>;
    case 256: if constexpr (S <= 6) return (const void*)k_persist_linear_mfma<T, 256, S, TS>; else return nullptr;
    default: return nullptr;
  }
}

const void* persist_fn_any(const mi_ode_solver* h) {
  if (h->family == FAM_PLUGIN) return h->persist_planes ? h->plugin->persist_planes_fn(h->S, h->ts_dense) : h->plugin->persist_fn(h->S, h->ts_dense);
  if (h->family == FAM_PLUGIN_COOP) return h->persist_planes ? h->plugin->persist_planes_fn(h->S, h->ts_dense) : h->plugin->persist_fn(h->S, h->ts_dense);
  if (h->family == FAM_LINEAR_MFMA) {
    if (h->S == 6) return h->ts_dense ? persist_fn_mfma<6, true>(h) : persist_fn_mfma<6, false>(h);
    if (h->S == 3 && !h->ts_dense) return persist_fn_mfma<3, false>(h);
    if (h->S == 13 && h->d.tableau.fsal && !h->ts_dense) return persist_fn_mfma<13, false>(h);
    return nullptr;
  }
  if (h->persist_planes) {
    if (h->S == 6) return h->ts_dense ? persist_planes_fn<6, true, true>(h) : persist_planes_fn<6, false, true>(h);
    if (h->S == 3 && !h->ts_dense) return persist_planes_fn<3, false, true>(h);
    if (h->S == 13 && h->d.tableau.fsal && !h->ts_dense) return persist_planes_fn<13, false, true>(h);
    if (h->S == 1 && !h->d.tableau.fsal && !h->ts_dense) return persist_planes_fn<1, false, false>(h);
    return nullptr;
  }
  if (h->S == 6) return h->ts_dense ? persist_fn<6, true>(h) : persist_fn<6, false>(h);
  if (h->S == 3 && !h->ts_dense) return persist_fn<3, false>(h);
  if (h->S == 13 && h->d.tableau.fsal && !h->ts_dense) return persist_fn_wide<13, true>(h);
  if (h->S == 1 && !h->d.tableau.fsal && !h->ts_dense) return persist_fn_wide<1, false>(h);
  return nullptr;
}

size_t persist_dyn_lds(const mi_ode_solver* h) {
  if (h->family != FAM_LINEAR_MFMA) return 0;
  return (size_t)2 * 16 * lin_ld<T>(h->lin_dp) * sizeof(T);
}
int persist_block(const mi_ode_solver* h) {
  if (h->family == FAM_LINEAR_MFMA) return h->lin_dp * 4;
  if (h->family == FAM_MLP_COOP || h->family == FAM_PLUGIN_COOP) return 256;
  if (h->nseg > 1) return MI_ODE_SEGMENT_ALIGN;
  if (h->persist_planes) return h->persist_planes_block;
  return h->d.batch <= 64 ? 64 : 256;
}

template <int D, int PHASE>
int launch_init_mfma(mi_ode_solver* h, InitArgs& I, hipStream_t st) {
  const size_t lds = step_linear_lds_bytes<T, D>();
  if constexpr (D == 256) {
    InitArgs J = I;
    const int rc = lin_pack(h, J.s.rhs, st);
    if (rc != 0) return rc;
    lin_allow_lds(k_init_linear_mfma<T, D, PHASE>, lds);
// ... 35 lines not shown
  hipError_t e = hipGetLastError();
  if (e != hipSuccess) {
    mi_set_error("stage kernel launch failed (mode %d nk %d): %s", mode, nk, hipGetErrorString(e));
    return MI_ODE_E_HIP;
  }
  return 0;
}

int MI_CAT(mi_launch_step_, MI_SUFFIX)(mi_ode_solver* h, mi::StepArgs& A, hipStream_t st) {
  int rc;
  if (h->S == 6) rc = h->ts_dense ? launch_step<6, true>(h, A, st) : launch_step<6, false>(h, A, st);
  else if (h->S == 3) rc = h->ts_dense ? launch_step<3, true>(h, A, st) : launch_step<3, false>(h, A, st);
  else if (h->S == 13 && h->d.tableau.fsal && !h->ts_dense) rc = launch_step_wide<13, true>(h, A, st);
  else if (h->S == 1 && !h->d.tableau.fsal && !h->ts_dense) rc = launch_step_wide<1, false>(h, A, st);
  else { mi_set_error("step kernel: no instantiation for this tableau"); return MI_ODE_E_INVALID; }
  if (rc != 0) return rc;
  h->n_launches += 1;
  hipError_t e = hipGetLastError();
  if (e != hipSuccess) { mi_set_error("step kernel launch failed: %s", hipGetErrorString(e)); return MI_ODE_E_HIP; }
  return 0;
}

int MI_CAT(mi_persist_capacity_, MI_SUFFIX)(mi_ode_solver* h) {
  const void* fn = persist_fn_any(h);
  if (fn == nullptr) return 0;
  int per_cu = 0;
  if (lin_streamed(h)) lin_allow_lds(fn, persist_dyn_lds(h));
  if (hipOccupancyMaxActiveBlocksPerMultiprocessor(&per_cu, fn, persist_block(h), persist_dyn_lds(h)) != hipSuccess || per_cu < 1) { (void)hipGetLastError(); return 0; }
  return h->num_cus * per_cu;
}

int MI_CAT(mi_launch_init_linear_, MI_SUFFIX)(mi_ode_solver* h, int phase, mi::InitArgs& I, hipStream_t st) {
  int rc = MI_ODE_E_INVALID;
  switch (h->lin_dp * 2 + (phase ? 1 : 0)) {
    case 16 * 2: rc = launch_init_mfma<16, 0>(h, I, st); break;
    case 16 * 2 + 1: rc = launch_init_mfma<16, 1>(h, I, st); break;
    case 32 * 2: rc = launch_init_mfma<32, 0>(h, I, st); break;
    case 32 * 2 + 1: rc = launch_init_mfma<32, 1>(h, I, st); break;
    case 64 * 2: rc = launch_init_mfma<64, 0>(h, I, st); break;
    case 64 * 2 + 1: rc = launch_init_mfma<64, 1>(h, I, st); break;
    case 128 * 2: rc = launch_init_mfma<128, 0>(h, I, st); break;
    case 128 * 2 + 1: rc = launch_init_mfma<128, 1>(h, I, st); break;
    case 256 * 2: rc = launch_init_mfma<256, 0>(h, I, st); break;
    case 256 * 2 + 1: rc = launch_init_mfma<256, 1>(h, I, st); break;
    default: mi_set_error("init kernel: unsupported dim %d", (int)h->d.dim); return MI_ODE_E_INVALID;
  }
  if (rc != 0) return rc;
  h->n_launches += 1;
  hipError_t e = hipGetLastError();
  if (e != hipSuccess) { mi_set_error("init kernel launch failed: %s", hipGetErrorString(e)); return MI_ODE_E_HIP; }
  return 0;
}

int MI_CAT(mi_launch_persist_, MI_SUFFIX)(mi_ode_solver* h, mi::PersistArgs& A, int grid, hipStream_t st) {
  const void* fn = persist_fn_any(h);
  if (fn == nullptr) { mi_set_error("no whole-integration kernel for this problem"); return MI_ODE_E_INVALID; }
  mi::PersistArgs B = A;
  const int rcp = lin_pack(h, B.s.rhs, st);
  if (rcp != 0) return rcp;
  void* args[] = {(void*)&B};
  hipError_t e = hipLaunchKernel(fn, dim3((unsigned)grid), dim3((unsigned)persist_block(h)), args, persist_dyn_lds(h), st);
  if (e != hipSuccess) { mi_set_error("whole-integration kernel launch failed: %s", hipGetErrorString(e)); return MI_ODE_E_HIP; }
  h->n_launches += 1;
  return 0;
}

namespace {
template <int D>
int launch_fixed_mfma(mi_ode_solver* h, mi::FixedArgs& A, hipStream_t st) {
  const size_t lds = (size_t)2 * 16 * lin_ld<T>(D) * sizeof(T);
  static int per_cu = 0;
  if (per_cu == 0) {
    lin_allow_lds(k_fixed_linear_mfma<T, D>, lds);
    if (hipOccupancyMaxActiveBlocksPerMultiprocessor(&per_cu, (const void*)k_fixed_linear_mfma<T, D>, D * 4, lds) != hipSuccess || per_cu < 1) per_cu = 1;
    if (per_cu > 8) per_cu = 8;
  }
  const long long nt = (A.batch + 15) / 16;
  long long g = (long long)h->num_cus * per_cu;
  if (g > nt) g = nt;
  if (g < 1) g = 1;
  if (getenv("MI_ODE_DEBUG")) fprintf(stderr, "[mi_ode] k_fixed_linear_mfma<%d>: %d workgroups/CU, grid %lld, %lld tiles\n", D, per_cu, g, nt);
  if constexpr (D == 256) {
    mi::FixedArgs B = A;
    const int rc = lin_pack(h, B.rhs, st);
    if (rc != 0) return rc;
    hipLaunchKernelGGL((k_fixed_linear_mfma<T, D>), dim3((unsigned)g), dim3(D * 4), lds, st, B);
  } else {
    hipLaunchKernelGGL((k_fixed_linear_mfma<T, D>), dim3((unsigned)g), dim3(D * 4), lds, st, A);
  }
  return 0;
}
}

namespace {
const void* adams_fn(const mi_ode_solver* h) {
  if (h->family == FAM_PLUGIN || h->family == FAM_PLUGIN_COOP) return h->plugin->multistep_fn(h->d.multistep);
  switch (h->family) {
    case FAM_CUBIC2: return (const void*)k_fixed_adams_rowlocal<T, RhsCubic2<T>>;
    case FAM_LINEAR2: return (const void*)k_fixed_adams_rowlocal<T, RhsLinear2<T>>;
    case FAM_LV: return (const void*)k_fixed_adams_rowlocal<T, RhsLotkaVolterra<T>>;
    case FAM_LORENZ: return (const void*)k_fixed_adams_rowlocal<T, RhsLorenz<T>>;
    case FAM_LINEAR_MFMA: case FAM_LINEAR_VALU:
      return h->d.dim <= 256 ? (const void*)k_fixed_adams_rowlocal<T, RhsLinearCoop<T>> : nullptr;
    case FAM_MLP_COOP: return (const void*)k_fixed_adams_rowlocal<T, RhsMlpCoop<T>>;
    default: return nullptr;
  }
}
}

int MI_CAT(mi_adams_capacity_, MI_SUFFIX)(mi_ode_solver* h) {
  const void* fn = adams_fn(h);
  int per_cu = 0;
// ... 169 lines not shown
```

tfdiffeq_amd/csrc/mi_ode_linadj.hip:

```cpp
#include <hip/hip_runtime.h>
#include <math.h>
#include <stdio.h>
#include <stdlib.h>
#include <string.h>
#include "mi_ode_handoff_host.h"
#include "mi_ode_linadj.h"

using namespace mi;

struct mi_ode_linadj {
  mi_ode_linadj_desc d;
  int dp;
  int is_f32;
  size_t elt;
  HandoffHost c;
  const void* fn;
  long long ntiles;
  char* planes;
  long long stride;
  double *pw, *cvec, *g0, *lmat, *mmat, *theta, *ktab;
  void *gpart, *wpad;
  long long* skew;
  Ctl* ctl_dev;
  LinAdjResult* res;
  long long n_launches;
};

namespace {

template <typename T>
const void* la_fn(int dp, size_t* lds, int* block) {
  *block = dp * 4;
  switch (dp) {
    case 16: *lds = linadj_lds_bytes<T, 16>(); return (const void*)k_linadj<T, 16>;
    case 32: *lds = linadj_lds_bytes<T, 32>(); return (const void*)k_linadj<T, 32>;
    case 64: *lds = linadj_lds_bytes<T, 64>(); return (const void*)k_linadj<T, 64>;
    default: *lds = linadj_lds_bytes<T, 128>(); return (const void*)k_linadj<T, 128>;
  }
}

int la_pad_dim(int dim) { return dim <= 16 ? 16 : (dim <= 32 ? 32 : (dim <= 64 ? 64 : 128)); }

void stage_polynomials(const mi_ode_tableau& tb, double (*pi)[kLaP]) {
  for (int s = 0; s < kLaP; ++s)
    for (int p = 0; p < kLaP; ++p) pi[s][p] = 0.0;
  pi[0][0] = 1.0;
  for (int s = 1; s <= kLaS; ++s) {
    pi[s][0] = 1.0;
    for (int j = 0; j < s; ++j)
      for (int p = 1; p < kLaP; ++p) pi[s][p] += tb.beta[s - 1][j] * pi[j][p - 1];
  }
}

}

extern "C" int mi_ode_linadj_destroy(mi_ode_linadj_handle h) {
  if (h == nullptr) return 0;
  if (h->planes) (void)hipFree(h->planes);
  if (h->pw) (void)hipFree(h->pw);
  if (h->cvec) (void)hipFree(h->cvec);
  if (h->g0) (void)hipFree(h->g0);
  if (h->lmat) (void)hipFree(h->lmat);
  if (h->mmat) (void)hipFree(h->mmat);
  if (h->theta) (void)hipFree(h->theta);
  if (h->ktab) (void)hipFree(h->ktab);
  if (h->gpart) (void)hipFree(h->gpart);
  if (h->wpad) (void)hipFree(h->wpad);
  if (h->skew) (void)hipFree(h->skew);
  if (h->c.partials) (void)hipFree(h->c.partials);
  if (h->ctl_dev) (void)hipFree(h->ctl_dev);
  if (h->res) (void)hipHostFree(h->res);
  delete h;
  return 0;
}

extern "C" int mi_ode_linadj_create(const mi_ode_linadj_desc* desc, mi_ode_linadj_handle* out) {
  if (desc == nullptr || out == nullptr) { mi_set_error("null argument"); return MI_ODE_E_INVALID; }
  *out = nullptr;
  const mi_ode_tableau& tb = desc->tableau;
  if (desc->batch < 1 || desc->dim < 1 || desc->dim > 128 || (desc->dtype != MI_ODE_F32 && desc->dtype != MI_ODE_F64)) {
    mi_set_error("linear adjoint: batch >= 1, 1 <= dim <= 128, dtype float32 or float64"); return MI_ODE_E_INVALID;
  }
  if (tb.n_stages != kLaS || !tb.fsal) {
    mi_set_error("linear adjoint: a 6-row FSAL-shaped tableau (dopri5) only - other methods take the generic path"); return MI_ODE_E_INVALID;
  }
  mi_ode_linadj* h = new mi_ode_linadj();
  memset(h, 0, sizeof(*h));
  HandoffHost& c = h->c;
  h->d = *desc;
  h->is_f32 = desc->dtype == MI_ODE_F32;
  h->elt = h->is_f32 ? 4 : 8;
  h->dp = la_pad_dim(desc->dim);
  h->fn = h->is_f32 ? la_fn<float>(h->dp, &c.lds, &c.block) : la_fn<double>(h->dp, &c.lds, &c.block);
  h->ntiles = (desc->batch + 15) / 16;
  int cus = 0;
  const int rc = handoff_device(&h->fn, 1, c.block, c.lds, &cus, "linear adjoint");
  if (rc != 0) { mi_ode_linadj_destroy(h); return rc; }
  int g = handoff_cap_grid(h->ntiles, cus, kLaMaxG);
  if (g < 1) g = 1;
  if (const char* eg = getenv("MI_ODE_LINADJ_GRID")) { const int v = atoi(eg); if (v >= 1 && v <= g) g = v; }
  c.grid = g;
  const size_t D = (size_t)h->dp, E = D * D + D;
  const size_t n = (size_t)desc->batch * (size_t)desc->dim;
  h->stride = (long long)((n * h->elt + 255) / 256 * 256);
  hipError_t e = hipMalloc((void**)&h->planes, 8 * (size_t)h->stride);
  if (e == hipSuccess) e = hipMalloc((void**)&h->pw, kLaP * D * D * sizeof(double));
  if (e == hipSuccess) e = hipMalloc((void**)&h->cvec, kLaP * D * sizeof(double));
  if (e == hipSuccess) e = hipMalloc((void**)&h->g0, 2 * E * sizeof(double));
  if (e == hipSuccess) e = hipMalloc((void**)&h->lmat, kLaP * D * D * sizeof(double));
  if (e == hipSuccess) e = hipMalloc((void**)&h->mmat, kLaPP * E * sizeof(double));
  if (e == hipSuccess) e = hipMalloc((void**)&h->theta, 2 * E * sizeof(double));
  if (e == hipSuccess) e = hipMalloc((void**)&h->ktab, 4 * kLaPP * sizeof(double));
  if (e == hipSuccess) e = hipMalloc((void**)&h->gpart, (size_t)c.grid * E * h->elt);
  if (e == hipSuccess) e = hipMalloc((void**)&h->wpad, 2 * D * D * h->elt);
  if (e == hipSuccess) e = hipMalloc((void**)&h->ctl_dev, sizeof(Ctl));
  if (e == hipSuccess) e = hipHostMalloc((void**)&h->res, sizeof(LinAdjResult), hipHostMallocDefault);
  if (e == hipSuccess && getenv("MI_ODE_LINADJ_PROF") != nullptr) e = hipMalloc((void**)&h->skew, 32 * (size_t)kLaMaxG * 2 * sizeof(long long));
  e = handoff_alloc(c, e, 1 << 20);
  if (e == hipSuccess) e = hipMemset(h->mmat, 0, kLaPP * E * sizeof(double));
  if (e == hipSuccess) e = hipMemset(h->cvec, 0, kLaP * D * sizeof(double));
  if (e == hipSuccess) e = hipMemset(h->lmat, 0, kLaP * D * D * sizeof(double));
  double pi[kLaP][kLaP], ktab[4][kLaPP];
  stage_polynomials(tb, pi);
  for (int p = 0; p < kLaP; ++p)
    for (int q = 0; q < kLaP; ++q) {
      double ks = 0.0, ke = 0.0, km = 0.0;
      for (int s = 0; s < kLaP; ++s) {
        const double pp = pi[s][p] * pi[s][q];
        ks += tb.c_sol[s] * pp; ke += tb.c_error[s] * pp; km += tb.c_mid[s] * pp;
      }
      ktab[0][p * kLaP + q] = ks; ktab[1][p * kLaP + q] = ke; ktab[2][p * kLaP + q] = km;
      ktab[3][p * kLaP + q] = pi[kLaS][p] * pi[kLaS][q];
    }
  if (e == hipSuccess) e = hipMemcpy(h->ktab, ktab, sizeof(ktab), hipMemcpyHostToDevice);
  if (e != hipSuccess) {
    mi_set_error("linear adjoint workspace: %s", hipGetErrorString(e));
    (void)hipGetLastError();
    mi_ode_linadj_destroy(h);
    return MI_ODE_E_HIP;
  }
  memset(h->res, 0, sizeof(LinAdjResult));
  *out = h;
  return 0;
}

extern "C" int mi_ode_linadj_segment(mi_ode_linadj_handle h, const void* w_dev, const void* b_dev, const void* y_dev, const void* adj_y_dev,
                                     const void* adj_t_dev, const void* adj_params_dev, const void* grad_out_dev, double t_start, double t_end,
                                     void* adj_y_out_dev, void* adj_t_out_dev, void* adj_params_out_dev, void* dldt_out_dev, double* host_scalars,
                                     mi_ode_stats* stats, void* stream) {
  if (h == nullptr || w_dev == nullptr || y_dev == nullptr || adj_y_dev == nullptr || adj_t_dev == nullptr || adj_params_dev == nullptr ||
      adj_y_out_dev == nullptr || adj_t_out_dev == nullptr || adj_params_out_dev == nullptr) { mi_set_error("null argument"); return MI_ODE_E_INVALID; }
  if (!(t_end != t_start)) {
    if (stats) { memset(stats, 0, sizeof(*stats)); stats->status = MI_ODE_ST_BAD_T; }
    return MI_ODE_ST_BAD_T;
  }
  hipStream_t st = (hipStream_t)stream;
  LinAdjArgs A;
  memset(&A, 0, sizeof(A));
  StepArgs& S = A.p.s;
  S.ctl = h->ctl_dev; S.batch = h->d.batch; S.dim = h->d.dim; S.n_plane = h->d.batch * (long long)h->d.dim;
  S.interp = MI_ODE_INTERP_QUARTIC_MID;
  fill_tableau(S, h->d.tableau, kLaS);
  S.out = adj_y_out_dev;
  const bool reversed = t_end < t_start;
  S.rhs.w[0] = w_dev; S.rhs.b[0] = b_dev;
  S.rhs.sign = reversed ? -1.0 : 1.0;
  fill_ctrl(S.cp, h->d, S.n_plane, h->is_f32, kLaS);
  A.p.t0 = reversed ? -t_start : t_start;
  A.t_end = reversed ? -t_end : t_end;
  A.p.t_small[0] = A.t_end;
  A.p.n_out = 1;
  A.p.nseg = 1;
  handoff_fill(A.p, h->c);
  A.p.xspin_limit = h->c.spin_limit;
  A.y_in = y_dev; A.a_in = adj_y_dev; A.th_in = adj_params_dev; A.adjt_in = adj_t_dev;
  A.th_out = adj_params_out_dev; A.adjt_out = adj_t_out_dev;
// ... 71 lines not shown
```

tfdiffeq_amd/csrc/mi_ode_persist.h:

```cpp
#pragma once
#include "mi_ode_step_fused.h"

namespace mi {

#ifdef MI_PERSIST_PROF
#define MI_TICK(var) const long long var = (long long)wall_clock64()
#define MI_TOCK(slot, a, b) do { if (threadIdx.x == 0 && blockIdx.x == 0) s_c.prof[slot] += (b) - (a); } while (0)
#define MI_SKEW(g, which) do { if (threadIdx.x == 0 && (g) < 8u) ((long long*)(A.s.partials + 8192))[((g) * gridDim.x + blockIdx.x) * 2 + (which)] = (long long)wall_clock64(); } while (0)
#else
#define MI_TICK(var)
#define MI_TOCK(slot, a, b)
#define MI_SKEW(g, which)
#endif
#ifdef MI_PERSIST_PROF
#define MI_HANDOFF_T0()
#define MI_HANDOFF_T1()
#else
#define MI_HANDOFF_T0() long long ho_t0_ = 0; if (threadIdx.x == 0 && blockIdx.x == 0) ho_t0_ = (long long)wall_clock64()
#define MI_HANDOFF_T1() do { if (threadIdx.x == 0 && blockIdx.x == 0) s_c.prof[3] += (long long)wall_clock64() - ho_t0_; } while (0)
#endif

constexpr int kPersistTSmall = 8;
constexpr int kPersistTout = 1024;
constexpr int kEmitShareRows = 8;
// ... 55 lines not shown
    const long long* src = (const long long*)&c;
    long long* dst = (long long*)A.ctl_host;
    for (int i = 0; i < (int)(sizeof(Ctl) / sizeof(long long)); ++i)
      __hip_atomic_store(dst + i, src[i], __ATOMIC_RELAXED, __HIP_MEMORY_SCOPE_SYSTEM);
  }
}

__device__ __forceinline__ void set_outputs_apply(Ctl* c, int n_out) {
  c->next_out = 0; c->n_out = n_out; c->n_steps_out = 0; c->emit_lo = c->emit_hi = 0;
  c->done = 0;
  if (c->status != 0) { c->done = 1; return; }
  if (n_out <= 0) { c->done = 1; return; }
  if (c->y0_nonfinite && c->n_attempt == 0) { c->status |= MI_ODE_ST_NONFINITE; c->done = 1; return; }
  if (!(c->t1 + c->dt > c->t1)) { c->status |= MI_ODE_ST_DT_UNDERFLOW; c->done = 1; }
}

typedef unsigned long long u64x2_t __attribute__((ext_vector_type(2)));
constexpr int kPRec = 16;
constexpr int kPersistMaxGrid = kMaxBlocks * kRec / (2 * kPRec);

__device__ __forceinline__ void store_ll_sc1(double* p, double value, unsigned seq) {
  const unsigned long long b = (unsigned long long)__double_as_longlong(value);
  u64x2_t v = {(b & 0xffffffffull) | ((unsigned long long)seq << 32), (b >> 32) | ((unsigned long long)seq << 32)};
  asm volatile("global_store_dwordx4 %0, %1, off sc1" ::"v"(p), "v"(v) : "memory");
}

__device__ __forceinline__ bool load_record_sc1(const double* p, unsigned seq, double (&val)[5]) {
  u64x2_t v[5];
  asm volatile(
      "global_load_dwordx4 %0, %5, off sc1\n\t"
      "global_load_dwordx4 %1, %5, off offset:16 sc1\n\t"
      "global_load_dwordx4 %2, %5, off offset:32 sc1\n\t"
      "global_load_dwordx4 %3, %5, off offset:48 sc1\n\t"
      "global_load_dwordx4 %4, %5, off offset:64 sc1\n\t"
      "s_waitcnt vmcnt(0)"
      : "=&v"(v[0]), "=&v"(v[1]), "=&v"(v[2]), "=&v"(v[3]), "=&v"(v[4])
      : "v"(p)
      : "memory");
  bool ok = true;
#pragma unroll
  for (int i = 0; i < 5; ++i) {
    ok = ok && ((unsigned)(v[i].x >> 32) == seq) && ((unsigned)(v[i].y >> 32) == seq);
    val[i] = __longlong_as_double((long long)((v[i].x & 0xffffffffull) | (v[i].y << 32)));
  }
  return ok;
}
__device__ __forceinline__ bool load_ll_sc1(const double* p, unsigned seq, double& val) {
  const unsigned long long w0 = (unsigned long long)__hip_atomic_load((const long long*)p, __ATOMIC_RELAXED, __HIP_MEMORY_SCOPE_AGENT);
  const unsigned long long w1 = (unsigned long long)__hip_atomic_load((const long long*)p + 1, __ATOMIC_RELAXED, __HIP_MEMORY_SCOPE_AGENT);
  val = __longlong_as_double((long long)((w0 & 0xffffffffull) | (w1 << 32)));
  return (unsigned)(w0 >> 32) == seq && (unsigned)(w1 >> 32) == seq;
}

__device__ __forceinline__ int uniform_i(int v) { return __builtin_amdgcn_readfirstlane(v); }
__device__ __forceinline__ double uniform_d(double v) {
  const long long b = __double_as_longlong(v);
  const unsigned lo = (unsigned)__builtin_amdgcn_readfirstlane((int)(unsigned)b);
  const unsigned hi = (unsigned)__builtin_amdgcn_readfirstlane((int)(unsigned)((unsigned long long)b >> 32));
  return __longlong_as_double((long long)(((unsigned long long)hi << 32) | lo));
}
template <typename P>
__device__ __forceinline__ P* uniform_p(P* p) {
  const unsigned long long b = (unsigned long long)p;
  const unsigned lo = (unsigned)__builtin_amdgcn_readfirstlane((int)(unsigned)b);
  const unsigned hi = (unsigned)__builtin_amdgcn_readfirstlane((int)(unsigned)(b >> 32));
  return (P*)(((unsigned long long)hi << 32) | lo);
}

struct PersistPub {
  double dt, t1, emit_t0, emit_t1, emit_dt;
  int accepted, emit_lo, emit_hi, done;
};

constexpr int kXRec = 16;
constexpr int kXMaxWorld = 64;

template <int MAXG, int TOUT>
struct PersistSharedT {
  static constexpr int kMaxGrid = MAXG, kTout = TOUT;
  Ctl c;
  PersistPub pub;
  AttemptState st;
  double red[80];
  double coef[kLinCoefMax];
  double vals[5][MAXG];
  double tout[TOUT];
  double xr[6][kXMaxWorld + 1];
  double seg_rec[kMaxSeg][kRec];
  SegState seg;
  int ok;
};
using PersistShared = PersistSharedT<kPersistMaxGrid, kPersistTout>;

__device__ __forceinline__ void ll_store(unsigned long long* p, double v, unsigned seq) {
  const unsigned long long b = (unsigned long long)__double_as_longlong(v);
  __hip_atomic_store(p, (b & 0xffffffffull) | ((unsigned long long)seq << 32), __ATOMIC_RELAXED, __HIP_MEMORY_SCOPE_SYSTEM);
  __hip_atomic_store(p + 1, (b >> 32) | ((unsigned long long)seq << 32), __ATOMIC_RELAXED, __HIP_MEMORY_SCOPE_SYSTEM);
}
__device__ __forceinline__ bool ll_load_record(const unsigned long long* p, unsigned seq, double (&v)[6]) {
  unsigned long long w[12];
#pragma unroll
  for (int i = 0; i < 12; ++i) w[i] = __hip_atomic_load(p + i, __ATOMIC_RELAXED, __HIP_MEMORY_SCOPE_SYSTEM);
  bool ok = true;
#pragma unroll
  for (int i = 0; i < 12; ++i) ok = ok && ((unsigned)(w[i] >> 32) == seq);
#pragma unroll
  for (int i = 0; i < 6; ++i) v[i] = __longlong_as_double((long long)((w[2 * i] & 0xffffffffull) | (w[2 * i + 1] << 32)));
  return ok;
}

template <class SH>
__device__ __forceinline__ void cross_rank(const PersistArgs& A, SH& sh, unsigned gen, double (&r)[5], double& n_tot,
                                           double n_local) {
  const int W = A.world;
  const unsigned seq = A.seq_base + gen + 1u;
  const unsigned bad = seq ^ 0x80000000u;
  double* g = A.gbuf + (long long)(gen & 1u) * kPRec;
  if (blockIdx.x == 0) {
    const unsigned long long* poll = nullptr;
    if (A.xpeers != nullptr) {
// ... 546 lines not shown
        T kn[D];
        rhs(sign * (P.t0 + (T)A.s.alpha[SG - 1] * hs), ys, kn);
#pragma unroll
        for (int d = 0; d < D; ++d) k[SG][d] = sign * kn[d];
      };
      for_stages<1, S>(stage);
      if (!live) continue;
      Row y1, f1;
#pragma unroll
      for (int d = 0; d < D; ++d) {
        T kk[S + 1];
#pragma unroll
        for (int j = 0; j <= S; ++j) kk[j] = k[j][d];
        T err, ymid;
        step_finish<T, S>(y0.v[d], kk, hs, A.s, err, ymid, !TS && P.j_hi > P.j_lo);
        if constexpr (!FSAL) ys[d] = step_y1_general<T, S>(y0.v[d], kk, hs, A.s);
        y1.v[d] = ys[d];
        f1.v[d] = k[S][d];
        acc.maxa = fmax(acc.maxa, (double)fabs(y0.v[d]));
        acc.maxb = fmax(acc.maxb, (double)fabs(ys[d]));
        acc.suma += (double)err * (double)err;
        step_emit<T, S, TS>(A.s, P, y0.v[d], ys[d], kk, ymid, e0 + d, t_out);
      }
      *(Row*)(P.y1 + e0) = y1;
      *(Row*)(P.f1 + e0) = f1;
    }
    ok = grid_reduce(A, acc, sh, gen++, r, n_tot);
    if (threadIdx.x == 0) {
      AttemptState st = sh.st;
      if (!ok) { st.status |= MI_ODE_ST_SYNC_TIMEOUT; st.done = 1; st.accepted = 0; }
      else if (nseg > 1) { seg_counts(); attempt_core_seg(st, sh.seg_rec, nseg, cp, A.seg_tol ? A.seg_rtol : nullptr, A.seg_atol); }
      else { fill_record(rec, r, n_tot); attempt_core(st, rec, cp); }
      publish(st);
      sh.st = st;
    }
    __syncthreads();
    if (uniform_i(sh.pub.accepted)) { cur_y = P.y1; cur_f = P.f1; }
  }

  if (cur_y == y_user) {
    for (long long row = first; row < batch; row += pitch) {
      long long e0;
      if (locate(row, e0)) *(Row*)(ya + e0) = *(const Row*)(y_user + e0);
    }
  }
  if (blockIdx.x == 0 && threadIdx.x == 0) {
    sh.st.store(s_c);
    s_c.idx_y0 = (cur_y == yb) ? 1 : 0; s_c.idx_y1 = (cur_y == yb) ? 0 : 1;
    s_c.idx_k[0] = (cur_f == fa) ? 2 : 2 + S; s_c.idx_k[S] = (cur_f == fa) ? 2 + S : 2;
    persist_write_back(A, s_c);
  }
}

template <typename T, int D, int S, bool TS>
__global__ __launch_bounds__(D * 4) void k_persist_linear_mfma(PersistArgs A) {
  extern __shared__ __attribute__((aligned(16))) char smem_raw[];
  __shared__ PersistShared sh;
  Ctl& s_c = sh.c;
  LinCtx<T, D> cx;
  cx.init(A.s.rhs, (T*)smem_raw, A.s.dim);
  CtrlParams cp = A.s.cp;
  cp.t_out = persist_stage_tout(A, sh.tout);
  const double* t_out = cp.t_out;
  unsigned gen = 0;
  double r[5], rec[kRec], n_tot = 0.0;
  if (threadIdx.x == 0) { persist_init_ctl(s_c, A); sh.ok = 1; }
  __syncthreads();

  T* const ya = (T*)(A.s.planes);
  T* const yb = (T*)(A.s.planes + A.s.stride);
  T* const fa = (T*)(A.s.planes + 2 * A.s.stride);
  T* const fb = (T*)(A.s.planes + (long long)(2 + S) * A.s.stride);
  const T* const y_user = (const T*)A.y0;

  bool ok;
  {
    Acc acc;
    MI_TICK(tf0);
    lin_f0_pass<T, D, true>(A.s, y_user, fa, (T*)nullptr, (T*)A.out0, cx, acc);
    MI_TICK(tf1);
    MI_TOCK(0, tf0, tf1);
    MI_SKEW(gen, 0);
    MI_HANDOFF_T0();
    ok = grid_reduce(A, acc, sh, gen++, r, n_tot);
    MI_HANDOFF_T1();
    MI_SKEW(gen - 1u, 1);
    if (threadIdx.x == 0 && ok) { fill_record(rec, r, n_tot); controller_apply(&s_c, rec, PH_F0, cp); }
    __syncthreads();
  }
  if (cp.auto_first_step && ok) {
    Acc acc;
    MI_TICK(ti0);
    lin_initb_pass<T, D, true>(A.s, y_user, fa, (T)uniform_d(s_c.h0), cx, acc);
    MI_TICK(ti1);
    MI_TOCK(1, ti0, ti1);
    MI_SKEW(gen, 0);
    MI_HANDOFF_T0();
    ok = grid_reduce(A, acc, sh, gen++, r, n_tot);
    MI_HANDOFF_T1();
    MI_SKEW(gen - 1u, 1);
    if (threadIdx.x == 0 && ok) { fill_record(rec, r, n_tot); controller_apply(&s_c, rec, PH_INITB, cp); }
  }
  auto publish = [&](const AttemptState& st) {
    sh.pub.dt = st.dt; sh.pub.t1 = st.t1; sh.pub.accepted = st.accepted; sh.pub.done = st.done;
    int j = st.next_out;
    const double t_new = st.t1 + st.dt;
    while (j < st.n_out && !(t_out[j] > t_new)) ++j;
    sh.pub.emit_lo = st.next_out; sh.pub.emit_hi = j;
  };
  if (threadIdx.x == 0) {
    if (!ok) { s_c.status |= MI_ODE_ST_SYNC_TIMEOUT; s_c.done = 1; }
    else set_outputs_apply(&s_c, A.n_out);
    AttemptState st;
    st.load(s_c);
    st.accepted = 0;
    publish(st);
    sh.st = st;
  }
  __syncthreads();

  const T* cur_y = y_user;
  T* cur_f = fa;
  while (!uniform_i(sh.pub.done)) {
    StepPlanes<T, S> P;
    const double dt_u = uniform_d(sh.pub.dt), t1_u = uniform_d(sh.pub.t1);
    P.y0 = cur_y; P.f0 = cur_f;
    P.y1 = (cur_y == ya) ? yb : ya;
    P.f1 = (cur_f == fa) ? fb : fa;
    P.hs = (T)dt_u; P.t0 = (T)t1_u;
    P.t_start = t1_u; P.dt64 = dt_u; P.t_new = t1_u + dt_u;
    P.j_lo = uniform_i(sh.pub.emit_lo); P.j_hi = uniform_i(sh.pub.emit_hi);
    Acc acc;
    MI_TICK(ta0);
#ifdef MI_TRACE
    if (blockIdx.x == 0 && (threadIdx.x == 0 || threadIdx.x == 256) && gen == 3u) { cx.tr = (long long*)(A.s.partials + 8192) + (threadIdx.x ? 256 : 0); cx.tn = 0; }
    else cx.tr = nullptr;
#endif
    lin_attempt_pass<T, D, S, TS, true>(A.s, P, cx, acc, t_out, (T*)sh.coef);
#ifdef MI_TRACE
    if (cx.tr != nullptr) {
      for (int q = 0; q + 3 < cx.tn && q < 4 * 14; q += 4)
        printf("[trace] wave %d eval %2d: write+barrier %5lld  mfma %5lld  barrier2 %5lld  | since prev eval end %5lld\n", (int)threadIdx.x >> 6, q / 4,
               cx.tr[q + 1] - cx.tr[q], cx.tr[q + 2] - cx.tr[q + 1], cx.tr[q + 3] - cx.tr[q + 2], q ? cx.tr[q] - cx.tr[q - 1] : 0LL);
    }
#endif
    MI_TICK(ta1);
    MI_SKEW(gen, 0);
    MI_HANDOFF_T0();
    ok = grid_reduce(A, acc, sh, gen++, r, n_tot);
    MI_HANDOFF_T1();
    MI_SKEW(gen - 1u, 1);
    MI_TICK(ta2);
    MI_TOCK(2, ta0, ta1); MI_TOCK(3, ta1, ta2);
    if (threadIdx.x == 0) {
      AttemptState st = sh.st;
      if (!ok) { st.status |= MI_ODE_ST_SYNC_TIMEOUT; st.done = 1; st.accepted = 0; }
      else { fill_record(rec, r, n_tot); attempt_core(st, rec, cp); }
      publish(st);
      sh.st = st;
    }
    __syncthreads();
    if (uniform_i(sh.pub.accepted)) { cur_y = P.y1; cur_f = P.f1; }
  }

  if (cur_y == y_user) {
    const long long n = A.s.batch * A.s.dim;
    for (long long i = (long long)blockIdx.x * blockDim.x + threadIdx.x; i < n; i += (long long)gridDim.x * blockDim.x) ya[i] = y_user[i];
  }
  if (blockIdx.x == 0 && threadIdx.x == 0) {
    sh.st.store(s_c);
    s_c.idx_y0 = (cur_y == yb) ? 1 : 0; s_c.idx_y1 = (cur_y == yb) ? 0 : 1;
    s_c.idx_k[0] = (cur_f == fa) ? 2 : 2 + S; s_c.idx_k[S] = (cur_f == fa) ? 2 + S : 2;
    persist_write_back(A, s_c);
  }
}

template <typename T, int D>
constexpr size_t persist_linear_lds_bytes() {
  return (size_t)2 * 16 * lin_ld<T>(D) * sizeof(T);
}

template <int UNUSED>
__global__ __launch_bounds__(64) void k_xrank_selftest(PersistArgs A, int rounds, int* result) {
  __shared__ PersistShared sh;
  if (threadIdx.x == 0) sh.ok = 1;
  __syncthreads();
  bool good = true;
  for (int round = 0; round < rounds; ++round) {
    double r[5], n_tot = 0.0;
#pragma unroll
    for (int i = 0; i < 5; ++i) r[i] = (double)(A.rank * 10 + i + round);
    cross_rank(A, sh, (unsigned)round, r, n_tot, (double)(A.rank + 1));
    if (threadIdx.x == 0) {
      const int W = A.world;
      double s0 = 0, s1 = 0, n = 0;
      for (int q = 0; q < W; ++q) { s0 += (double)(q * 10 + 2 + round); s1 += (double)(q * 10 + 3 + round); n += (double)(q + 1); }
      good = good && sh.ok && r[0] == (double)((W - 1) * 10 + round) && r[1] == (double)((W - 1) * 10 + 1 + round) && r[2] == s0 &&
             r[3] == s1 && r[4] == (double)((W - 1) * 10 + 4 + round) && n_tot == n;
    }
    __syncthreads();
    if (!sh.ok) break;
  }
  if (threadIdx.x == 0) *result = good ? 1 : 0;
}

}
```

tfdiffeq_amd/csrc/mi_ode_step_fused.h:

```cpp
#pragma once
#include <type_traits>
#include "mi_ode_ctrl_dev.h"
#include "mi_ode_dense.h"
#include "mi_ode_dev.h"
#include "mi_ode_stage_linear.h"
#include "mi_ode_stage_rowlocal.h"

#ifndef MI_ABL
#define MI_ABL 0
#endif

namespace mi {

struct StepArgs {
  Ctl* ctl;
  char* planes;
  long long stride;
  long long batch;
  int dim;
  int interp;
  void* out;
  const double* t_out;
  long long n_plane;
  double beta[MI_ODE_MAX_STAGES][MI_ODE_MAX_STAGES];
  double alpha[MI_ODE_MAX_STAGES];
  double e[kMaxK];
  double csol[kMaxK];
  double cmid[kMaxK];
  double* partials;
  RhsParams rhs;
  unsigned* ticket;
  CtrlParams cp;
};

__device__ __forceinline__ void finish_attempt(const StepArgs& A, const Acc& acc, double* red) {
  if (A.ticket == nullptr) {
    block_reduce_store<false>(acc, red, A.partials + (long long)blockIdx.x * kRec);
    return;
  }
  block_reduce_store<true>(acc, red, A.partials + (long long)blockIdx.x * kRec);
  __shared__ int s_last;
  if (threadIdx.x == 0) {
    asm volatile("s_waitcnt vmcnt(0)" ::: "memory");
    const unsigned t = __hip_atomic_fetch_add(A.ticket, 1u, __ATOMIC_RELAXED, __HIP_MEMORY_SCOPE_AGENT);
    s_last = (t == gridDim.x - 1);
  }
  __syncthreads();
  if (!s_last) return;
  __shared__ double rec[kRec];
  reduce_block_records<true>(A.partials, (int)gridDim.x, rec);
  if (threadIdx.x == 0) {
    rec[R_N] = (double)A.cp.n_local;
    controller_apply(A.ctl, rec, PH_ATTEMPT, A.cp);
    __hip_atomic_store(A.ticket, 0u, __ATOMIC_RELAXED, __HIP_MEMORY_SCOPE_AGENT);
  }
}

template <typename T, int S>
struct StepPlanes {
  const T* y0;
  const T* f0;
  T* y1;
  T* f1;
  T hs, t0;
  double t_start, t_new, dt64;
  int j_lo, j_hi;
};

template <typename T, int S>
__device__ __forceinline__ bool resolve_step(const StepArgs& A, StepPlanes<T, S>& P) {
  const Ctl* c = A.ctl;
  if (c->done) return false;
  char* base = A.planes;
  P.y0 = (const T*)(base + (long long)c->idx_y0 * A.stride);
  P.y1 = (T*)(base + (long long)c->idx_y1 * A.stride);
  P.f0 = (const T*)(base + (long long)c->idx_k[0] * A.stride);
  P.f1 = (T*)(base + (long long)c->idx_k[S] * A.stride);
  P.hs = (T)c->dt;
  P.t0 = (T)c->t1;
  P.t_start = c->t1; P.dt64 = c->dt; P.t_new = c->t1 + c->dt;
  int j = c->next_out;
  P.j_lo = j;
  if (A.t_out != nullptr)
    while (j < c->n_out && !(A.t_out[j] > P.t_new)) ++j;
  P.j_hi = j;
  return true;
// ... 245 lines not shown
  bool has_bias;
  bool plain;
  T* s_ys;
  int cur = 0;
#ifdef MI_TRACE
  long long* tr = nullptr;
  int tn = 0;
  __device__ __forceinline__ void stamp() { if (tr != nullptr && tn < 256) tr[tn++] = (long long)__builtin_readcyclecounter(); }
#else
  __device__ __forceinline__ void stamp() {}
#endif

  __device__ __forceinline__ void init(const RhsParams& rhs, T* lds, int dim) {
    if constexpr (STREAM) {
      const int tid = threadIdx.x;
      lane = tid & 63; wave = tid >> 6; li = lane & 15; lg = lane >> 4;
      col = 16 * wave + li;
      d = dim; colok = col < dim;
      if constexpr (UNI) { wp = (const CH*)rhs.w[0] + (long long)__builtin_amdgcn_readfirstlane(wave) * NCH * 64; wl = lane; }
      else { wp = (const CH*)rhs.w[0] + (long long)wave * NCH * 64 + lane; wl = 0; }
      trips = (dim + 16 * VEC - 1) / (16 * VEC);
      active = __builtin_amdgcn_readfirstlane(16 * wave) < dim;
      if (active) { r0 = wp[wl]; r1 = wp[64 + wl]; }
      bf[0] = (T)0;
      const T* bias = (const T*)rhs.b[0];
      has_bias = bias != nullptr;
      bias_v = (has_bias && colok) ? bias[col] : (T)0;
      sign = (T)rhs.sign;
      plain = bias == nullptr && rhs.sign == 1.0;
      s_ys = lds;
    } else {
      init_matrix((const T*)rhs.w[0], (const T*)rhs.b[0], rhs.sign, false, lds, dim);
    }
  }
  __device__ __forceinline__ void init_matrix(const T* W, const T* bias, double sgn, bool transposed, T* lds, int dim) {
    static_assert(!STREAM, "streamed W: init() takes the packed copy");
    const int tid = threadIdx.x;
    lane = tid & 63; wave = tid >> 6; li = lane & 15; lg = lane >> 4;
    col = 16 * wave + li;
    d = dim; colok = col < dim;
    const int cc = colok ? col : 0;
#pragma unroll
    for (int s = 0; s < KS; ++s) {
      const int kk = lg * KS + s, kc = kk < dim ? kk : 0;
      const T v = transposed ? W[(long long)cc * dim + kc] : W[(long long)kc * dim + cc];
      bf[s] = (colok && kk < dim) ? v : (T)0;
    }
    has_bias = bias != nullptr;
    bias_v = (has_bias && colok) ? bias[col] : (T)0;
    sign = (T)sgn;
    plain = bias == nullptr && sgn == 1.0;
    s_ys = lds;
  }
  __device__ __forceinline__ void init_padded(const T* Mpad, const T* bias, double sgn, T* lds, int dim) {
    static_assert(!STREAM, "streamed W: init() takes the packed copy");
    const int tid = threadIdx.x;
    lane = tid & 63; wave = tid >> 6; li = lane & 15; lg = lane >> 4;
    col = 16 * wave + li;
    d = dim; colok = col < dim;
#pragma unroll
    for (int s = 0; s < KS; ++s) bf[s] = Mpad[(lg * KS + s) * D + col];
    has_bias = bias != nullptr;
    bias_v = (has_bias && colok) ? bias[col] : (T)0;
    sign = (T)sgn;
    plain = bias == nullptr && sgn == 1.0;
    s_ys = lds;
  }
  __device__ __forceinline__ int row_of(int i) const { return TR::acc_row(lane, i); }
  __device__ __forceinline__ unsigned off_of(int i) const { return (unsigned)(TR::acc_row(lane, i) * d + col); }
  __device__ __forceinline__ int rows_here(long long tile_i, long long batch) const {
    const long long left = batch - tile_i * R_;
    return left < R_ ? (int)left : R_;
  }

  __device__ __forceinline__ void rhs_eval(const T (&ys)[4], T (&kn)[4]) { rhs_eval(ys, kn, [] {}); }
  template <class F>
  __device__ __forceinline__ void rhs_eval(const T (&ys)[4], T (&kn)[4], F&& under_chain) {
    stamp();
    T* tile = s_ys + cur * TILE;
    int aoff = cur * TILE + li * LD + lg * (STREAM ? 4 * VEC * trips : KS);
    if constexpr (STREAM) asm volatile("" : "+v"(aoff));
    cur ^= 1;
#pragma unroll
    for (int i = 0; i < 4; ++i) tile[TR::acc_row(lane, i) * LD + col] = ys[i];
    if (!(MI_ABL & 4)) lds_barrier();
    stamp();
    under_chain();
    acc_t c0 = {0, 0, 0, 0};
    const T* ap = s_ys + aoff;
#if (MI_ABL & 1)
    c0[0] = ap[0] * bf[0]; c0[1] = ap[1] * bf[0]; c0[2] = ap[2] * bf[0]; c0[3] = ap[3] * bf[0];
#else
    if constexpr (STREAM) {
      static_assert(NCH % 4 == 0, "two chunk pairs per trip");
      const CH* wq = wp;
#ifndef MI_STREAM_ABL
#define MI_STREAM_ABL 0
#endif
#if (MI_STREAM_ABL & 2)
      CH fa = *(const CH*)ap;
#define MI_LDA(p) fa
#else
#define MI_LDA(p) (*(const CH*)(p))
#endif
#if (MI_STREAM_ABL & 1)
#define MI_LDW(p, keep) keep
// ... 45 lines not shown
#pragma unroll
      for (int i = 0; i < 4; ++i) {
        T k_ = c0[i];
        if (has_bias) k_ = k_ + bias_v;
        kn[i] = sign * k_;
      }
    }
    stamp();
  }
};

template <typename T, int D>
__global__ __launch_bounds__(256) void k_lin_pack(const T* W, int dim, T* pack) {
  constexpr int VEC = MfmaTraits<T>::VEC, KS = D / 4, NCH = KS / VEC;
  for (int e = blockIdx.x * blockDim.x + threadIdx.x; e < D * D; e += gridDim.x * blockDim.x) {
    const int v = e % VEC, lane = (e / VEC) % 64, m = (e / (VEC * 64)) % NCH, w = e / (VEC * 64 * NCH);
    const int ks = 4 * VEC * ((dim + 16 * VEC - 1) / (16 * VEC));
    const int k = (lane >> 4) * ks + m * VEC + v, c = 16 * w + (lane & 15);
    pack[e] = (m * VEC < ks && k < dim && c < dim) ? W[(long long)k * dim + c] : (T)0;
  }
}

template <int S>
struct LinCoef {
  static constexpr int kErr = S * (S + 1) / 2, kMid = kErr + S + 1, kCount = kMid + S + 1;
  static constexpr int row(int s) { return s * (s - 1) / 2; }
};
constexpr int kLinCoefMax = 128;

template <typename T, int S>
__device__ __forceinline__ void lin_fill_coef(const StepArgs& A, T hs, T* coef) {
  using CF = LinCoef<S>;
  for (int q = threadIdx.x; q < CF::kCount; q += blockDim.x) {
    double c;
    if (q < CF::kErr) {
      int s_ = 1;
      while (CF::row(s_ + 1) <= q) ++s_;
      c = A.beta[s_ - 1][q - CF::row(s_)];
    } else if (q < CF::kMid) c = A.e[q - CF::kErr];
    else c = A.cmid[q - CF::kMid];
    coef[q] = hs * (T)c;
  }
}

template <bool SC0, typename T>
__device__ __forceinline__ T stream_load(const T* p) {
  if constexpr (SC0) return __hip_atomic_load(p, __ATOMIC_RELAXED, __HIP_MEMORY_SCOPE_WORKGROUP);
  else return *p;
}

template <typename T, int D, int S, bool TS, bool SC0>
__device__ __forceinline__ void lin_attempt_pass(const StepArgs& A, const StepPlanes<T, S>& P, LinCtx<T, D>& cx, Acc& acc,
                                                 const double* t_out, T* coef , int blk = (int)blockIdx.x,
                                                 int nblk = (int)gridDim.x) {
  constexpr int R_ = LinCtx<T, D>::R_;
  using CF = LinCoef<S>;
  const long long ntiles = (A.batch + R_ - 1) / R_;
  lin_fill_coef<T, S>(A, P.hs, coef);
  lds_barrier();
  constexpr bool PF = LinCtx<T, D>::PF;
  T y0n[4], f0n[4];
  auto fetch = [&](long long t_i) {
    const T* ty = P.y0 + t_i * R_ * cx.d;
    const T* tf = P.f0 + t_i * R_ * cx.d;
    const int nr = cx.rows_here(t_i, A.batch);
#pragma unroll
    for (int i = 0; i < 4; ++i) {
      const bool ok = cx.row_of(i) < nr && cx.colok && !(MI_ABL & 8);
      y0n[i] = ok ? stream_load<SC0>(ty + cx.off_of(i)) : (T)0;
      f0n[i] = ok ? stream_load<SC0>(tf + cx.off_of(i)) : (T)0;
    }
  };
  if (PF && (long long)blk < ntiles) fetch(blk);
  const T c_first = coef[CF::row(1)];
  T cnx[PF ? S + 1 : 1];

  for (long long tile_i = blk; tile_i < ntiles; tile_i += nblk) {
    const long long row0 = tile_i * R_;
    T y0e[4], k[S + 1][4], ys[4];
    if constexpr (!PF) fetch(tile_i);
#pragma unroll
    for (int i = 0; i < 4; ++i) { y0e[i] = y0n[i]; k[0][i] = f0n[i]; }
    if (PF && tile_i + nblk < ntiles) fetch(tile_i + nblk);

    auto stage = [&](auto sg_c) {
      constexpr int SG = decltype(sg_c)::value;
      T cb[SG];
#pragma unroll
      for (int j = 0; j < SG; ++j) cb[j] = (SG == 1) ? c_first : (PF ? cnx[PF ? j : 0] : coef[CF::row(SG) + j]);
#pragma unroll
      for (int i = 0; i < 4; ++i) {
        T a_ = cb[0] * k[0][i];
#pragma unroll
        for (int j = 1; j < SG; ++j) a_ = lin_madd(cb[j], k[j][i], a_);
        ys[i] = y0e[i] + a_;
      }
      cx.rhs_eval(ys, k[SG], [&] {
        if constexpr (PF) {
#pragma unroll
          for (int j = 0; j <= SG; ++j) cnx[j] = coef[(SG < S ? CF::row(SG + 1) : CF::kErr) + j];
        }
      });
    };
    for_stages<1, S>(stage);
    const bool need_mid = !TS && P.j_hi > P.j_lo;
    T err4[4], ym4[4];
#pragma unroll
    for (int j = 0; j <= S; ++j) {
      const T ce = PF ? cnx[PF ? j : 0] : coef[CF::kErr + j];
#pragma unroll
      for (int i = 0; i < 4; ++i) err4[i] = (j == 0) ? ce * k[0][i] : lin_madd(ce, k[j][i], err4[i]);
    }
    if (need_mid) {
#pragma unroll
      for (int j = 0; j <= S; ++j) {
        const T cm = coef[CF::kMid + j];
#pragma unroll
        for (int i = 0; i < 4; ++i) ym4[i] = (j == 0) ? cm * k[0][i] : ym4[i] + cm * k[j][i];
      }
    }
    const int nr = cx.rows_here(tile_i, A.batch);
    T* ty1 = P.y1 + row0 * cx.d;
    T* tf1 = P.f1 + row0 * cx.d;
#pragma unroll
    for (int i = 0; i < 4; ++i) {
      if (cx.row_of(i) < nr && cx.colok) {
        T kk[S + 1];
#pragma unroll
        for (int j = 0; j <= S; ++j) kk[j] = k[j][i];
        const T err = err4[i];
        const T ymid = need_mid ? y0e[i] + ym4[i] : y0e[i];
        const long long idx = row0 * cx.d + cx.off_of(i);
        if (!(MI_ABL & 8) || err == (T)123.456) {
          ty1[cx.off_of(i)] = ys[i];
          tf1[cx.off_of(i)] = k[S][i];
        }
        step_emit<T, S, TS>(A, P, y0e[i], ys[i], kk, ymid, idx, t_out);
        acc.maxa = fmax(acc.maxa, (double)fabs(y0e[i]));
        acc.maxb = fmax(acc.maxb, (double)fabs(ys[i]));
        acc.suma += (double)err * (double)err;
      }
    }
  }
}

template <typename T, int D, bool SC0, bool DOT = false>
__device__ __forceinline__ void lin_f0_pass(const StepArgs& A, const T* y0, T* f0_out, T* copy_a, T* copy_b, LinCtx<T, D>& cx,
                                            Acc& acc, int blk = (int)blockIdx.x, int nblk = (int)gridDim.x, const T* gdot = nullptr,
                                            double* dot = nullptr) {
  constexpr int R_ = LinCtx<T, D>::R_;
  const long long ntiles = (A.batch + R_ - 1) / R_;
  T y0n[4], gn[DOT ? 4 : 1];
  auto fetch = [&](long long t_i) {
    const T* ty = y0 + t_i * R_ * cx.d;
    const int nr = cx.rows_here(t_i, A.batch);
#pragma unroll
    for (int i = 0; i < 4; ++i) {
      const bool ok = cx.row_of(i) < nr && cx.colok;
      y0n[i] = ok ? stream_load<SC0>(ty + cx.off_of(i)) : (T)0;
      if constexpr (DOT) gn[i] = ok ? (gdot + t_i * R_ * cx.d)[cx.off_of(i)] : (T)0;
    }
  };
  constexpr bool PF = LinCtx<T, D>::PF;
  if (PF && (long long)blk < ntiles) fetch(blk);
  for (long long tile_i = blk; tile_i < ntiles; tile_i += nblk) {
    T y0e[4], kn[4], ge[DOT ? 4 : 1];
    if constexpr (!PF) fetch(tile_i);
#pragma unroll
    for (int i = 0; i < 4; ++i) { y0e[i] = y0n[i]; if constexpr (DOT) ge[i] = gn[i]; }
    if (PF && tile_i + nblk < ntiles) fetch(tile_i + nblk);
    cx.rhs_eval(y0e, kn);
    const int nr = cx.rows_here(tile_i, A.batch);
    const long long tb = tile_i * R_ * cx.d;
#pragma unroll
    for (int i = 0; i < 4; ++i) {
      if (cx.row_of(i) < nr && cx.colok) {
        (f0_out + tb)[cx.off_of(i)] = kn[i];
        if (copy_a != nullptr) (copy_a + tb)[cx.off_of(i)] = y0e[i];
        if (copy_b != nullptr) (copy_b + tb)[cx.off_of(i)] = y0e[i];
        const T sc = (T)A.cp.atol + fabs(y0e[i]) * (T)A.cp.rtol;
        const double q0 = (double)(y0e[i] / sc);
        acc.suma += q0 * q0;
        if (!finite_(y0e[i])) acc.flag = 1;
        const double q1 = (double)(kn[i] / sc);
        acc.sumb += q1 * q1;
        if constexpr (DOT) *dot += (double)kn[i] * (double)ge[i];
      }
    }
  }
}

template <typename T, int D, bool SC0>
__device__ __forceinline__ void lin_initb_pass(const StepArgs& A, const T* y0, const T* f0, T h0, LinCtx<T, D>& cx, Acc& acc,
                                               int blk = (int)blockIdx.x, int nblk = (int)gridDim.x) {
  constexpr int R_ = LinCtx<T, D>::R_;
  const long long ntiles = (A.batch + R_ - 1) / R_;
  T y0n[4], f0n[4];
  auto fetch = [&](long long t_i) {
    const T* ty = y0 + t_i * R_ * cx.d;
    const T* tf = f0 + t_i * R_ * cx.d;
    const int nr = cx.rows_here(t_i, A.batch);
#pragma unroll
    for (int i = 0; i < 4; ++i) {
      const bool ok = cx.row_of(i) < nr && cx.colok;
      y0n[i] = ok ? stream_load<SC0>(ty + cx.off_of(i)) : (T)0;
      f0n[i] = ok ? stream_load<SC0>(tf + cx.off_of(i)) : (T)0;
    }
  };
  if ((long long)blk < ntiles) fetch(blk);
  for (long long tile_i = blk; tile_i < ntiles; tile_i += nblk) {
    T y0e[4], f0e[4], ys[4], kn[4];
#pragma unroll
    for (int i = 0; i < 4; ++i) { y0e[i] = y0n[i]; f0e[i] = f0n[i]; ys[i] = y0e[i] + h0 * f0e[i]; }
    if (tile_i + nblk < ntiles) fetch(tile_i + nblk);
    cx.rhs_eval(ys, kn);
    const int nr = cx.rows_here(tile_i, A.batch);
#pragma unroll
    for (int i = 0; i < 4; ++i) {
      if (cx.row_of(i) < nr && cx.colok) {
        const T sc = (T)A.cp.atol + fabs(y0e[i]) * (T)A.cp.rtol;
        const double q = (double)((kn[i] - f0e[i]) / sc);
        acc.suma += q * q;
      }
    }
  }
}

template <typename T, int D, int S, bool TS>
__global__ __launch_bounds__(D * 4) void k_step_linear_mfma(StepArgs A) {
  StepPlanes<T, S> P;
  if (!resolve_step<T, S>(A, P)) return;
  extern __shared__ __attribute__((aligned(16))) char smem_raw[];
  T* s_ys = (T*)smem_raw;
  double* red = (double*)(s_ys + LinCtx<T, D>::kBufs * LinCtx<T, D>::TILE);
  LinCtx<T, D> cx;
  cx.init(A.rhs, s_ys, A.dim);
  Acc acc;
  lin_attempt_pass<T, D, S, TS, false>(A, P, cx, acc, A.t_out, (T*)(red + 80));
  finish_attempt(A, acc, red);
}

struct InitArgs {
  StepArgs s;
  const void* y0;
  void* copy_b;
};

template <typename T, int D, int PHASE>
__global__ __launch_bounds__(D * 4) void k_init_linear_mfma(InitArgs I) {
  const StepArgs& A = I.s;
  const Ctl* c = A.ctl;
  extern __shared__ __attribute__((aligned(16))) char smem_raw[];
  T* s_ys = (T*)smem_raw;
  double* red = (double*)(s_ys + LinCtx<T, D>::kBufs * LinCtx<T, D>::TILE);
  LinCtx<T, D> cx;
  cx.init(A.rhs, s_ys, A.dim);
  Acc acc;
  T* plane_y = (T*)(A.planes + (long long)c->idx_y0 * A.stride);
  T* plane_f = (T*)(A.planes + (long long)c->idx_k[0] * A.stride);
  if constexpr (PHASE == 0) lin_f0_pass<T, D, false>(A, (const T*)I.y0, plane_f, plane_y, (T*)I.copy_b, cx, acc);
  else lin_initb_pass<T, D, false>(A, plane_y, plane_f, (T)c->h0, cx, acc);
  block_reduce_store<false>(acc, red, A.partials + (long long)blockIdx.x * kRec);
}

template <typename T, int D>
__global__ __launch_bounds__(D * 4) void k_fixed_linear_mfma(FixedArgs A) {
  extern __shared__ __attribute__((aligned(16))) char smem_raw[];
  LinCtx<T, D> cx;
  cx.init(A.rhs, (T*)smem_raw, A.dim);
  constexpr int R_ = LinCtx<T, D>::R_;
  const long long ntiles = (A.batch + R_ - 1) / R_;
  const long long n = A.batch * A.dim;
  const T* y0p = (const T*)A.y0;
  T* out = (T*)A.out;
  FixedClk clk;
  clk.begin();
  for (long long tile_i = blockIdx.x; tile_i < ntiles; tile_i += gridDim.x) {
    T y[4];
    long long idx[4];
    bool ok[4];
#pragma unroll
    for (int i = 0; i < 4; ++i) {
      const long long row = tile_i * R_ + cx.row_of(i);
      ok[i] = row < A.batch && cx.colok;
      idx[i] = row * cx.d + cx.col;
      y[i] = ok[i] ? y0p[idx[i]] : (T)0;
      if (ok[i]) out[idx[i]] = y[i];
    }
    int j = 1;
    for (int s = 0; s < A.M; ++s) {
      const T t0 = (T)A.grid[s];
// ... 43 lines not shown
```

tfdiffeq_amd/solvers.py:

```python
import abc
import os
import collections
import ctypes as C
import math
import sys

import numpy as np
import torch

from . import _native as N
from . import dispatch as D
from .misc import (_assert_increasing, _handle_unused_kwargs, _lincomb, _np_dtype, _scalar_tensor, _Exchange)
from .rk_common import _is_fsal_shaped


def _fill_tableau(tb_struct, tableau, c_mid):
    S = len(tableau.alpha)
    if S > N.MAX_STAGES:
        raise ValueError('fused engine supports at most %d tableau rows' % N.MAX_STAGES)
    tb_struct.n_stages = S
    tb_struct.fsal = 1 if (S > 0 and _is_fsal_shaped(tableau)) else 0
    for i in range(S):
        tb_struct.alpha[i] = float(tableau.alpha[i])
        for j, v in enumerate(tableau.beta[i]):
# ... 282 lines not shown
                                                        self._stream()), 'mi_ode_integrate_rows')
        return out, rows, rc

    def integrate_rows_t(self, rt, y0=None, rows_t_plugin=None):
        y0 = self._check_y0(y0)
        for x, dt in ((rt.t, torch.float64), (rt.lengths, torch.int32), (rt.rtol, torch.float64), (rt.atol, torch.float64)):
            if x is not None and (x.device != self.device or x.dtype != dt or not x.is_contiguous()):
                raise ValueError('per-row inputs: contiguous %s tensors on %s are needed' % (dt, self.device))
        if tuple(rt.t.shape) != (self.batch, rt.T) or any(x is not None and tuple(x.shape) != (self.batch,) for x in (rt.lengths, rt.rtol, rt.atol)):
            raise ValueError('per-row inputs: t [%d, T] and [%d] lengths / tolerances are needed' % (self.batch, self.batch))

        def ptr(x):
            return C.c_void_p(x.data_ptr() if x is not None else 0)
        out = torch.empty((rt.T,) + self.shape, dtype=self.dtype, device=self.device)
        rows = torch.empty((self.batch, 4), dtype=torch.int64, device=self.device)
        with torch.cuda.device(self.device):
            rc = N.check(self.lib.mi_ode_integrate_rows_t(self.h, C.c_void_p(rows_t_plugin[1] if rows_t_plugin is not None else 0),
                                                          C.c_void_p(y0.data_ptr()), ptr(rt.t), rt.T, ptr(rt.lengths), ptr(rt.rtol), ptr(rt.atol),
                                                          C.c_void_p(out.data_ptr()), C.c_void_p(rows.data_ptr()), C.byref(self.stats),
                                                          self._stream()), 'mi_ode_integrate_rows_t')
        return out, rows, rc

    def integrate_fixed_rows_t(self, rt, y0=None, plugin=None):
        y0 = self._check_y0(y0)
        for x, dt in ((rt.t, torch.float64), (rt.lengths, torch.int32)):
            if x is not None and (x.device != self.device or x.dtype != dt or not x.is_contiguous()):
                raise ValueError('per-row inputs: contiguous %s tensors on %s are needed' % (dt, self.device))
        if len(self.shape) != 2 or tuple(rt.t.shape) != (self.batch, rt.T) or (rt.lengths is not None and tuple(rt.lengths.shape) != (self.batch,)):
            raise ValueError('per-row inputs: a [%d, dim] state, t [%d, T] and [%d] lengths are needed' % (self.batch, self.batch, self.batch))
        out = torch.empty((rt.T,) + self.shape, dtype=self.dtype, device=self.device)
        with torch.cuda.device(self.device):
            N.check(self.lib.mi_ode_integrate_fixed_rows_t(self.h, C.c_void_p(plugin[1] if plugin is not None else 0), C.c_void_p(y0.data_ptr()),
                                                           C.c_void_p(rt.t.data_ptr()), rt.T,
                                                           C.c_void_p(rt.lengths.data_ptr() if rt.lengths is not None else 0),
                                                           C.c_void_p(out.data_ptr()), C.byref(self.stats), self._stream()),
                    'mi_ode_integrate_fixed_rows_t')
        return out

    def begin(self, t0, y0=None):
        y0 = self._check_y0(y0)
        with torch.cuda.device(self.device):
            N.check(self.lib.mi_ode_begin(self.h, C.c_void_p(y0.data_ptr()), float(t0), self._stream()), 'mi_ode_begin')

    def advance(self, times):
        arr, p = self._times(times)
        out = torch.empty((arr.shape[0],) + self.shape, dtype=self.dtype, device=self.device)
        with torch.cuda.device(self.device):
            rc = N.check(self.lib.mi_ode_advance(self.h, p, arr.shape[0], C.c_void_p(out.data_ptr()), self._stream()),
                         'mi_ode_advance')
            N.check(self.lib.mi_ode_get_stats(self.h, C.byref(self.stats), self._stream()), 'mi_ode_get_stats')
        self._raise_for_status(rc)
        return out

    def profile(self):
        out = (C.c_double * 4)()
        N.check(self.lib.mi_ode_get_profile(self.h, out), 'mi_ode_get_profile')
        return [out[i] for i in range(4)]

    def eval_rhs(self, y, t=0.0):
        f = torch.empty_like(y)
        with torch.cuda.device(self.device):
            N.check(self.lib.mi_ode_eval_rhs(self.h, C.c_void_p(y.data_ptr()), float(t), C.c_void_p(f.data_ptr()),
                                             self._stream()), 'mi_ode_eval_rhs')
        return f

    def rk_step(self, y0, f0, t0, dt, want_k=False):
        y1, f1 = torch.empty_like(y0), torch.empty_like(y0)
        S = self.desc.tableau.n_stages
        k = torch.empty((S + 1,) + tuple(y0.shape), dtype=y0.dtype, device=y0.device) if want_k else None
        norms = (C.c_double * 4)()
        with torch.cuda.device(self.device):
            N.check(self.lib.mi_ode_rk_step_fused(self.h, C.c_void_p(y0.data_ptr()), C.c_void_p(f0.data_ptr()), float(t0),
                                                  float(dt), C.c_void_p(y1.data_ptr()), C.c_void_p(f1.data_ptr()), norms,
                                                  C.c_void_p(k.data_ptr()) if want_k else C.c_void_p(0), self._stream()),
                    'mi_ode_rk_step_fused')
        return y1, f1, [norms[i] for i in range(4)], k


_ENGINE_CACHE = collections.OrderedDict()
_ENGINE_CACHE_MAX = 8


def clear_engine_cache():
    _NO_ENGINE.clear()
    while _ENGINE_CACHE:
        _, eng = _ENGINE_CACHE.popitem()
        eng.close()
    import sys
    disc = sys.modules.get(__package__ + '.discrete')
    if disc is not None:
        disc.clear_engines()


class SyncTimeout(RuntimeError):
    """The in-kernel grid hand-off of a one-launch kernel timed out (the GPU is shared with another persistent kernel).  Nothing
    was committed: callers with a per-step loop (the multistep solvers) take it instead."""


_NO_ENGINE = set()


def _cached_engine_or_none(key, factory):
    if key in _NO_ENGINE:
        return None
    try:
        return _cached_engine(key, factory)
# ... 404 lines not shown
        self.stats = dict(eng.stats.as_dict(), engine=engine, per_trajectory=True,
                          rows={'n_attempts': rows[:, 0], 'n_accepted': rows[:, 1], 'nfe': rows[:, 2], 'status': rows[:, 3]})
        if bits:
            bad = torch.nonzero(rows[:, 3]).flatten().tolist()
            first = bad[0]
            msg = N.status_message(int(rows[first, 3]))
            row = y.reshape(-1, rhs.dim)[first:first + 1].contiguous()
            kept = self.rtol, self.atol
            try:
                if rt is not None:
                    times = rt.t[first, :int(rt.lengths[first]) if rt.lengths is not None else rt.T].cpu().numpy()
                    for name, x in (('rtol', rt.rtol), ('atol', rt.atol)):
                        if x is not None:
                            setattr(self, name, float(x[first]) if self.pooled_ratio else [float(x[first])])
                self._make_engine(route, row).integrate(times, row)
            except AssertionError as e:
                msg = str(e)
            finally:
                self.rtol, self.atol = kept
            raise AssertionError('%s [per_trajectory: %d of %d rows failed; rows %s%s, the message is row %d\'s]' % (
                msg, len(bad), int(rows.shape[0]), ', '.join(str(i) for i in bad[:8]), ', ...' if len(bad) > 8 else '', first))
        return (out,)

    def _integrate_on(self, route, t):
        if route.kind == 'fused_rows':
            return self._integrate_rows(route, t)
        fused = route.kind in ('fused', 'fused_tuple', 'fused_coop')
        eng = self._make_engine(route) if fused else None
        if eng is not None and route.kind == 'fused_coop':
            try:
                out = eng.integrate(t.to(torch.float64).numpy(), self.y0[0]) if len(t) > 1 else None
            except SyncTimeout:
                out = None
            if out is not None:
                self.stats = dict(eng.stats.as_dict(), cross_rank=eng.transport,
                                  engine='cooperative whole-call kernel (one launch, a thread per state element)')
                return (out,)
            eng = None
        if eng is None:
            host = D.after(route, D.device_controlled(self.y0, len(self.tableau.alpha), **self._options())) if fused else route
            if host.told is not None:
                host.told.warn_limits(self.y0[0])
            if host.kind == 'callable':
                return self._integrate_device_controlled(t)
            out = super(_AdaptiveRKSolver, self).integrate(t)
            self.stats = {'engine': 'plane kernels', 'n_attempts': getattr(self, '_n_attempts', 0),
                          'n_accepted': getattr(self, '_n_accepted', 0), 'status': 0}
            return out
        prof0 = eng.profile() if self._profile else None
        try:
            out = eng.integrate(t.to(torch.float64).numpy(), self.y0[0] if self._packed is None else self._packed[0])
        finally:
            self.stats = eng.stats.as_dict()
            self.stats['cross_rank'] = eng.transport
            if eng.transport_log:
                self.stats['cross_rank_log'] = list(eng.transport_log)
            if self._profile:
                self.stats['profile'] = [a - b for a, b in zip(eng.profile(), prof0)]
        if self._packed is not None:
            _, rows, offs = self._packed
            self.stats['components'] = len(rows)
            return tuple(out[:, o:o + r].reshape((out.shape[0],) + tuple(c.shape)) for c, r, o in zip(self.y0, rows, offs))
        return (out,)

    def _integrate_device_controlled(self, t):
        from .graph_step import DeviceControlledRK, _credit_nfe, keep_recorded, recorded_engine
        t64 = t.to(torch.float64)
        self.before_integrate(t64)
        reuse = self._graph == 'reuse'
        eng = recorded_engine(self) if reuse else None
        if eng is None:
            eng = DeviceControlledRK(self, graph=True if reuse else self._graph)
        try:
            outs = eng.integrate(t64.numpy(), self.y0, self.rk_state.f1, float(self.rk_state.dt))
            st = eng.stats.as_dict()
            info = dict(eng.info)
            py_calls = eng.py_calls
        except BaseException:
            eng.close()
            raise
        if reuse and eng.captured and eng.graph is not None:
            keep_recorded(self, eng)
        else:
            eng.close()
        self.stats = st
        self.stats.update(info)
        self.stats['n_polls'] = info.get('polls', 0)
        _credit_nfe(self.func, int(st['nfe']) - py_calls)
        bits = int(st['status'])
        if bits:
            raise AssertionError(N.status_text(bits, self.max_num_steps, st['dt']))
        return outs

    def before_integrate(self, t):
        from .misc import _convert_to_tensor, _select_initial_step
        from .rk_common import _RungeKuttaState
        like = self.y0[0]
        t0 = float(t[0])
        if self.pooled_ratio:
            if self.first_step is None:
                first = np.float64(_select_initial_step(self.func, t0, self.y0, self.init_order, self.rtol, self.atol,
                                                        exchange=self._exchange))
            else:
                first = _convert_to_tensor(self.first_step, dtype=np.float64)
            f0 = self.func(torch.full((), t0, dtype=torch.float64, device=like.device), self.y0)
        else:
# ... 94 lines not shown
```

Baseline: 6.492 billion.

## Collapse linear-RHS Dopri5 attempt into precomputed matrix-power polynomial pass

For a linear f64 RHS solved with an adaptive 6-stage FSAL tableau, precompute powers of W (and bias rows) once per integration. Each attempt then evaluates the solution, error and midpoint as fixed polynomials in W, so it needs only a few matrix products instead of one per stage. The derivative at the new point is left stale and recomputed lazily, either when falling back to the stage-by-stage path (when many outputs land in a step) or in get_state. This adds a setup launch, extra buffers, a product counter and more kernel instantiations, and it changes the rounding behaviour relative to the staged evaluation.

```diff
diff --git a/include/mi_ode.h b/include/mi_ode.h
--- a/include/mi_ode.h
+++ b/include/mi_ode.h
@@ -153,6 +153,7 @@
                          void* y1_dev, void* f1_dev, double* err_norms_host, void* k_out_dev, void* stream);
 int mi_ode_eval_rhs(mi_ode_handle h, const void* y_dev, double t, void* f_dev, void* stream);
 int mi_ode_get_stats(mi_ode_handle h, mi_ode_stats* stats, void* stream);
+int64_t mi_ode_matrix_products(mi_ode_handle h);
 int mi_ode_get_profile(mi_ode_handle h, double* out4);
 int mi_ode_get_state(mi_ode_handle h, void* y_dev, void* f_dev, void* stream);
 
diff --git a/tfdiffeq_amd/_native.py b/tfdiffeq_amd/_native.py
--- a/tfdiffeq_amd/_native.py
+++ b/tfdiffeq_amd/_native.py
@@ -219,6 +219,7 @@
     'mi_ode_rccl_connect': (C.c_int, [C.c_void_p, C.c_void_p, C.c_int32, C.c_int32]),
     'mi_ode_get_stats': (C.c_int, [C.c_void_p, C.POINTER(Stats), C.c_void_p]),
     'mi_ode_get_state': (C.c_int, [C.c_void_p, C.c_void_p, C.c_void_p, C.c_void_p]),
+    'mi_ode_matrix_products': (C.c_int64, [C.c_void_p]),
     'mi_ode_get_profile': (C.c_int, [C.c_void_p, C.POINTER(C.c_double)]),
     'mi_ode_adjoint_create': (C.c_int, [C.POINTER(AdjointDesc), C.POINTER(C.c_void_p)]),
     'mi_ode_adjoint_destroy': (C.c_int, [C.c_void_p]),
diff --git a/tfdiffeq_amd/csrc/mi_ode_api.hip b/tfdiffeq_amd/csrc/mi_ode_api.hip
--- a/tfdiffeq_amd/csrc/mi_ode_api.hip
+++ b/tfdiffeq_amd/csrc/mi_ode_api.hip
@@ -7,6 +7,7 @@
 
 #include "mi_ode_control.h"
 #include "mi_ode_host.h"
+#include "mi_ode_linear_poly_host.h"
 #include "mi_ode_plane.h"
 #include "mi_ode_step_fused.h"
 #include "mi_ode_persist.h"
@@ -392,6 +393,12 @@
   A.partials = h->partials; A.rhs = h->rhs;
   A.ticket = h->fused_ctl ? h->ticket : nullptr;
   A.cp = h->cp;
+  if (h->lin_poly == 2) {
+    const int D = h->lin_dp;
+    A.poly_pk = (const double*)h->lin_pow + LinPowLayout::pk(D, 1);
+    A.poly_q = (const double*)h->lin_pow + LinPowLayout::q(D, 0);
+    A.poly_g = (const double*)h->lin_pow + LinPowLayout::g(D);
+  }
 }
 
 static void fill_mlp_args(mi_ode_solver* h, MlpArgs& M) {
@@ -422,6 +429,7 @@
   if (h->adams_tab) (void)hipFree(h->adams_tab);
   if (h->mlp_pack) (void)hipFree(h->mlp_pack);
   if (h->lin_pack) (void)hipFree(h->lin_pack);
+  if (h->lin_pow) (void)hipFree(h->lin_pow);
   if (h->adams_res) (void)hipHostFree(h->adams_res);
   if (h->rank_rec && h->own_exchange) (void)hipFree(h->rank_rec);
   if (h->gathered && h->own_exchange) (void)hipFree(h->gathered);
@@ -580,6 +588,16 @@
     const bool light_many = (h->family != FAM_LINEAR_MFMA && h->family != FAM_MLP) && h->step_grid > 32;
     h->fused_ctl = (h->step_fused && h->d.world_size <= 1 && desc->allgather == nullptr && desc->fusion != 3 &&
                     !(light_many && desc->fusion == 0)) ? 1 : 0;
+  }
+  if (h->family == FAM_LINEAR_MFMA && h->step_fused && desc->adaptive) {
+    const mi_ode_tableau& tbl = desc->tableau;
+    h->lin_poly = 1;
+    LinPolyTables tabs;
+    if (!h->is_f32 && h->lin_dp <= 128 && h->S == 6 && tbl.fsal && desc->interp == MI_ODE_INTERP_QUARTIC_MID && desc->linear_variant == 4 &&
+        lin_poly_tables(tbl, &tabs)) {
+      h->lin_poly = 2;
+      for (int p = 0; p < 8; ++p) { h->lin_g[0][p] = tabs.g_sol[p]; h->lin_g[1][p] = tabs.g_err[p]; h->lin_g[2][p] = tabs.g_mid[p]; h->lin_g[3][p] = tabs.pi_last[p]; }
+    }
   }
   {
     const bool rowlocal = h->family == FAM_CUBIC2 || h->family == FAM_LINEAR2 || h->family == FAM_LV || h->family == FAM_LORENZ ||
@@ -680,6 +698,9 @@
   h->cp.is_f32 = h->is_f32;
   h->cp.n_stages = h->S;
   h->cp.auto_first_step = isnan(desc->first_step) ? 1 : 0;
+  h->cp.lin_poly = h->lin_poly;
+  h->cp.lin_ndense = kLinNDense;
+  if (const char* en = getenv("MI_ODE_LIN_NDENSE")) { const int v = atoi(en); if (v >= 0 && v <= 64) h->cp.lin_ndense = v; }
   h->ip.kind = desc->interp;
   h->ip.nk = h->S + 1;
   for (int j = 0; j < kMaxK; ++j) h->ip.c_mid[j] = tb.c_mid[j];
@@ -687,6 +708,11 @@
   e = hipMalloc((void**)&h->planes, (size_t)h->stride * (2 + h->S + 1));
   if (e == hipSuccess) e = hipMalloc((void**)&h->partials, (size_t)kMaxBlocks * kRec * sizeof(double));
   if (e == hipSuccess) e = hipMemset(h->partials, 0, (size_t)kMaxBlocks * kRec * sizeof(double));
+  if (e == hipSuccess && h->lin_poly == 2) {
+    e = hipMalloc(&h->lin_pow, LinPowLayout::count(h->lin_dp) * sizeof(double));
+    if (e == hipSuccess) e = hipMemset(h->lin_pow, 0, LinPowLayout::count(h->lin_dp) * sizeof(double));
+    if (e == hipSuccess) e = hipMemcpy((double*)h->lin_pow + LinPowLayout::g(h->lin_dp), h->lin_g, sizeof(h->lin_g), hipMemcpyHostToDevice);
+  }
   if (desc->exchange_send_dev != nullptr && desc->exchange_recv_dev != nullptr) {
     h->rank_rec = desc->exchange_send_dev;
     h->gathered = desc->exchange_recv_dev;
@@ -784,6 +810,10 @@
     memset(&I, 0, sizeof(I));
     fill_step_args(h, I.s);
     I.y0 = y0_dev; I.copy_b = first_out_dev;
+    if (h->lin_poly == 2) {
+      const int rcw = mi_launch_lin_powers_f64(h, st);
+      if (rcw != 0) return rcw;
+    }
     int rci = h->is_f32 ? mi_launch_init_linear_f32(h, 0, I, st) : mi_launch_init_linear_f64(h, 0, I, st);
     if (rci != 0) return rci;
     rci = enqueue_controller(h, PH_F0, st);
@@ -1157,6 +1187,10 @@
   return 0;
 }
 
+extern "C" int64_t mi_ode_matrix_products(mi_ode_handle h) {
+  return (h != nullptr && h->lin_poly && h->ctl_host != nullptr) ? (int64_t)h->ctl_host->n_products : 0;
+}
+
 extern "C" int mi_ode_get_profile(mi_ode_handle h, double* out4) {
   if (h == nullptr || out4 == nullptr) { mi_set_error("null argument"); return MI_ODE_E_INVALID; }
   out4[0] = h->prof_last_ms; out4[1] = (double)h->prof_n; out4[2] = h->prof_all_ms; out4[3] = (double)h->prof_n;
@@ -1171,6 +1205,13 @@
   if (rc != 0) return rc;
   const Ctl* c = h->ctl_host;
   if (y_dev) MI_HIP(hipMemcpyAsync(y_dev, h->planes + (long long)c->idx_y0 * h->stride, (size_t)h->n * h->elt, hipMemcpyDeviceToDevice, st));
+  if (f_dev && c->f_stale) {
+    StageArgs A;
+    fill_common(h, A);
+    A.explicit_mode = 1; A.ctl = nullptr;
+    A.x_y0 = h->planes + (long long)c->idx_y0 * h->stride; A.x_kout = f_dev; A.x_t0 = c->t1; A.x_dt = 0.0;
+    return launch_stage(h, M_STAGE, 0, A, st);
+  }
   if (f_dev) MI_HIP(hipMemcpyAsync(f_dev, h->planes + (long long)c->idx_k[0] * h->stride, (size_t)h->n * h->elt, hipMemcpyDeviceToDevice, st));
   return 0;
 }
diff --git a/tfdiffeq_amd/csrc/mi_ode_ctrl_dev.h b/tfdiffeq_amd/csrc/mi_ode_ctrl_dev.h
--- a/tfdiffeq_amd/csrc/mi_ode_ctrl_dev.h
+++ b/tfdiffeq_amd/csrc/mi_ode_ctrl_dev.h
@@ -49,17 +49,19 @@
   long long n_attempt, n_accept, n_reject, nfe, n_steps_out;
   int next_out, n_out, emit_lo, emit_hi, done, accepted;
   unsigned status;
+  long long n_products;
+  int f_stale;
   __device__ __forceinline__ void load(const Ctl& c) {
     t0 = c.t0; t1 = c.t1; dt = c.dt; ratio = c.ratio; emit_t0 = c.emit_t0; emit_t1 = c.emit_t1; emit_dt = c.emit_dt;
     n_attempt = c.n_attempt; n_accept = c.n_accept; n_reject = c.n_reject; nfe = c.nfe; n_steps_out = c.n_steps_out;
     next_out = c.next_out; n_out = c.n_out; emit_lo = c.emit_lo; emit_hi = c.emit_hi; done = c.done; accepted = c.accepted;
-    status = c.status;
+    status = c.status; n_products = c.n_products; f_stale = c.f_stale;
   }
   __device__ __forceinline__ void store(Ctl& c) const {
     c.t0 = t0; c.t1 = t1; c.dt = dt; c.ratio = ratio; c.emit_t0 = emit_t0; c.emit_t1 = emit_t1; c.emit_dt = emit_dt;
     c.n_attempt = n_attempt; c.n_accept = n_accept; c.n_reject = n_reject; c.nfe = nfe; c.n_steps_out = n_steps_out;
     c.next_out = next_out; c.n_out = n_out; c.emit_lo = emit_lo; c.emit_hi = emit_hi; c.done = done; c.accepted = accepted;
-    c.status = status;
+    c.status = status; c.n_products = n_products; c.f_stale = f_stale;
   }
 };
 
@@ -105,6 +107,19 @@
   attempt_tail(c, ratio, ratio <= 1.0, P);
 }
 
+__device__ __forceinline__ int lin_outputs_in_span(int next_out, int n_out, double t1, double dt, const double* t_out) {
+  int j = next_out;
+  const double t_new = t1 + dt;
+  if (t_out != nullptr)
+    while (j < n_out && !(t_out[j] > t_new)) ++j;
+  return j - next_out;
+}
+__device__ __forceinline__ bool lin_takes_poly(int n_in, const CtrlParams& P) { return P.lin_poly == 2 && n_in <= P.lin_ndense; }
+__device__ __forceinline__ void lin_count_attempt(AttemptState& c, int n_in, bool poly, const CtrlParams& P) {
+  c.n_products += poly ? 2 + n_in : P.n_stages + (c.f_stale ? 1 : 0);
+  if (c.accepted) c.f_stale = poly ? 1 : 0;
+}
+
 constexpr int kMaxSeg = MI_ODE_MAX_SEGMENTS;
 struct SegState { double d1[kMaxSeg]; };
 
@@ -201,6 +216,7 @@
 
   if (phase == PH_F0) {
     c->nfe += 1;
+    if (P.lin_poly) c->n_products += 1;
     c->y0_nonfinite = rec[R_FLAG] != 0.0;
     double d0, d1, h0;
     if (P.is_f32) {
@@ -218,6 +234,7 @@
   }
   if (phase == PH_INITB) {
     c->nfe += 1;
+    if (P.lin_poly) c->n_products += 1;
     double first;
     if (P.is_f32) {
       const float h0 = (float)c->h0, d1 = (float)c->d1;
@@ -240,7 +257,9 @@
 
   AttemptState a;
   a.load(*c);
+  const int n_in = P.lin_poly ? lin_outputs_in_span(a.next_out, a.n_out, a.t1, a.dt, P.t_out) : 0;
   attempt_core(a, rec, P);
+  if (P.lin_poly) lin_count_attempt(a, n_in, lin_takes_poly(n_in, P), P);
   if (a.accepted) {
     c->emit_y0 = c->idx_y0; c->emit_y1 = c->idx_y1;
     for (int j = 0; j <= P.n_stages; ++j) c->emit_k[j] = c->idx_k[j];
diff --git a/tfdiffeq_amd/csrc/mi_ode_dev.h b/tfdiffeq_amd/csrc/mi_ode_dev.h
--- a/tfdiffeq_amd/csrc/mi_ode_dev.h
+++ b/tfdiffeq_amd/csrc/mi_ode_dev.h
@@ -44,6 +44,9 @@
   int accepted;
   long long prof[4];
   long long clk_cycles, clk_ticks;
+  long long n_products;
+  int f_stale;
+  int lin_pad_;
 };
 
 enum Mode {
@@ -269,6 +272,8 @@
   int n_stages;
   int auto_first_step;
   const double* t_out;
+  int lin_poly = 0;
+  int lin_ndense = 0;
 };
 
 struct InterpParams {
diff --git a/tfdiffeq_amd/csrc/mi_ode_host.h b/tfdiffeq_amd/csrc/mi_ode_host.h
--- a/tfdiffeq_amd/csrc/mi_ode_host.h
+++ b/tfdiffeq_amd/csrc/mi_ode_host.h
@@ -92,6 +92,9 @@
   double adams_gamma_star[13];
   int lin_dp;
   void* lin_pack;
+  int lin_poly;
+  void* lin_pow;
+  double lin_g[4][8];
   long long n_launches;
   int n_polls;
   int begun;
@@ -128,6 +131,8 @@
 int mi_launch_init_linear_f32(mi_ode_solver* h, int phase, mi::InitArgs& I, hipStream_t st);
 int mi_persist_capacity_f64(mi_ode_solver* h);
 int mi_persist_capacity_f32(mi_ode_solver* h);
+int mi_launch_lin_powers_f64(mi_ode_solver* h, hipStream_t st);
+int mi_launch_lin_powers_f32(mi_ode_solver* h, hipStream_t st);
 int mi_launch_persist_mlp_f32(mi_ode_solver* h, mi::PersistArgs& A, int grid, hipStream_t st);
 int mi_persist_capacity_mlp_f32(mi_ode_solver* h);
 int mi_launch_mlp_f32(mi_ode_solver* h, int mode, mi::MlpArgs& M, hipStream_t st);
@@ -169,6 +174,7 @@
   cp.n_local = n_local;
   cp.order = d.order; cp.init_order = d.init_order;
   cp.controller = MI_ODE_CTRL_MISC; cp.is_f32 = is_f32; cp.n_stages = n_stages; cp.auto_first_step = 1;
+  cp.lin_poly = 0; cp.lin_ndense = 0;
 }
 
 inline void fill_rhs(RhsParams& r, const mi_ode_rhs& rhs) {
diff --git a/tfdiffeq_amd/csrc/mi_ode_launch.inc b/tfdiffeq_amd/csrc/mi_ode_launch.inc
--- a/tfdiffeq_amd/csrc/mi_ode_launch.inc
+++ b/tfdiffeq_amd/csrc/mi_ode_launch.inc
@@ -1,5 +1,6 @@
 #include <stdio.h>
 #include <stdlib.h>
+#include <string.h>
 #include "mi_ode_host.h"
 #include "mi_ode_stage_linear.h"
 #include "mi_ode_stage_rowlocal.h"
@@ -92,6 +93,12 @@
     lin_allow_lds(k_step_linear_mfma<T, D, S, TS>, lds);
     hipLaunchKernelGGL((k_step_linear_mfma<T, D, S, TS>), dim3(h->step_grid), dim3(D * 4), lds, st, B);
   } else {
+    if constexpr (lin_poly_capable<T, D, S, TS>()) {
+      if (h->lin_poly == 2) {
+        hipLaunchKernelGGL((k_step_linear_mfma<T, D, S, TS, true>), dim3(h->step_grid), dim3(D * 4), lds, st, A);
+        return 0;
+      }
+    }
     hipLaunchKernelGGL((k_step_linear_mfma<T, D, S, TS>), dim3(h->step_grid), dim3(D * 4), lds, st, A);
   }
   return 0;
@@ -183,6 +190,17 @@
 
 template <int S, bool TS>
 const void* persist_fn_mfma(const mi_ode_solver* h) {
+  if constexpr (lin_poly_capable<T, 128, S, TS>()) {
+    if (h->lin_poly == 2) {
+      switch (h->lin_dp) {
+        case 16: return (const void*)k_persist_linear_mfma<T, 16, S, TS, true>;
+        case 32: return (const void*)k_persist_linear_mfma<T, 32, S, TS, true>;
+        case 64: return (const void*)k_persist_linear_mfma<T, 64, S, TS, true>;
+        case 128: return (const void*)k_persist_linear_mfma<T, 128, S, TS, true>;
+        default: break;
+      }
+    }
+  }
   switch (h->lin_dp) {
     case 16: return (const void*)k_persist_linear_mfma<T, 16, S, TS>;
     case 32: return (const void*)k_persist_linear_mfma<T, 32, S, TS>;
@@ -324,12 +342,79 @@
   return 0;
 }
 
+namespace {
+template <int D>
+int launch_lin_powers(mi_ode_solver* h, hipStream_t st) {
+  if constexpr (sizeof(T) != 8) {
+    mi_set_error("polynomial attempt pass: float64 only"); return MI_ODE_E_INVALID;
+  } else {
+    using L = mi::LinPowLayout;
+    T* base = (T*)h->lin_pow;
+    const T* W = (const T*)h->rhs.w[0];
+    const T* b = (const T*)h->rhs.b[0];
+    const int dim = (int)h->d.dim;
+    auto mat = [&](int p, const T** ptr, int* ld) { if (p == 1) { *ptr = W; *ld = dim; } else { *ptr = base + L::rm(D, p); *ld = D; } };
+    auto row = [&](int p, const T** ptr) { *ptr = p == 0 ? b : base + L::q(D, p); };
+    static const int prod[3][3][3] = {{{2, 1, 1}, {0, 0, 0}, {0, 0, 0}}, {{3, 2, 1}, {4, 2, 2}, {0, 0, 0}}, {{5, 4, 1}, {6, 4, 2}, {7, 4, 3}}};
+    static const int rows[3][3][3] = {{{1, 0, 1}, {0, 0, 0}, {0, 0, 0}}, {{2, 0, 2}, {3, 1, 2}, {0, 0, 0}}, {{4, 0, 4}, {5, 1, 4}, {6, 2, 4}}};
+    for (int lv = 0; lv < 3; ++lv) {
+      mi::LinPowArgs A;
+      memset(&A, 0, sizeof(A));
+      A.dim = dim;
+      int n = 0;
+      if (lv == 0) {
+        mi::LinPowJob& J = A.job[n++];
+        J.b = W; J.ldb = dim; J.ar = dim; J.pk = base + L::pk(D, 1);
+        if (b != nullptr) {
+          mi::LinPowJob& K = A.job[n++];
+          K.b = b; K.ldb = dim; K.ar = 1; K.rm = base + L::q(D, 0);
+        }
+      }
+      for (int i = 0; i < 3; ++i) {
+        if (prod[lv][i][0] == 0) continue;
+        mi::LinPowJob& J = A.job[n++];
+        const T *pa, *pb;
+        mat(prod[lv][i][1], &pa, &J.lda); mat(prod[lv][i][2], &pb, &J.ldb);
+        J.a = pa; J.b = pb; J.ar = dim;
+        J.rm = base + L::rm(D, prod[lv][i][0]); J.pk = base + L::pk(D, prod[lv][i][0]);
+      }
+      for (int i = 0; i < 3 && b != nullptr; ++i) {
+        if (rows[lv][i][0] == 0) continue;
+        mi::LinPowJob& J = A.job[n++];
+        const T *pa, *pb;
+        row(rows[lv][i][1], &pa); mat(rows[lv][i][2], &pb, &J.ldb);
+        J.a = pa; J.lda = D; J.b = pb; J.ar = 1;
+        J.rm = base + L::q(D, rows[lv][i][0]); J.pk = nullptr;
+      }
+      hipLaunchKernelGGL((mi::k_lin_powers<T, D>), dim3(D * D / 256, n), dim3(256), 0, st, A);
+    }
+    if (hipGetLastError() != hipSuccess) { mi_set_error("k_lin_powers launch failed"); return MI_ODE_E_HIP; }
+    return 0;
+  }
+}
+}
+
+int MI_CAT(mi_launch_lin_powers_, MI_SUFFIX)(mi_ode_solver* h, hipStream_t st) {
+  if (h->lin_pow == nullptr) { mi_set_error("polynomial attempt pass: no power buffer"); return MI_ODE_E_INVALID; }
+  switch (h->lin_dp) {
+    case 16: return launch_lin_powers<16>(h, st);
+    case 32: return launch_lin_powers<32>(h, st);
+    case 64: return launch_lin_powers<64>(h, st);
+    case 128: return launch_lin_powers<128>(h, st);
+    default: mi_set_error("polynomial attempt pass: tile widths 16 .. 128"); return MI_ODE_E_INVALID;
+  }
+}
+
 int MI_CAT(mi_launch_persist_, MI_SUFFIX)(mi_ode_solver* h, mi::PersistArgs& A, int grid, hipStream_t st) {
   const void* fn = persist_fn_any(h);
   if (fn == nullptr) { mi_set_error("no whole-integration kernel for this problem"); return MI_ODE_E_INVALID; }
   mi::PersistArgs B = A;
   const int rcp = lin_pack(h, B.s.rhs, st);
   if (rcp != 0) return rcp;
+  if (h->family == FAM_LINEAR_MFMA && h->lin_poly == 2) {
+    const int rcw = MI_CAT(mi_launch_lin_powers_, MI_SUFFIX)(h, st);
+    if (rcw != 0) return rcw;
+  }
   void* args[] = {(void*)&B};
   hipError_t e = hipLaunchKernel(fn, dim3((unsigned)grid), dim3((unsigned)persist_block(h)), args, persist_dyn_lds(h), st);
   if (e != hipSuccess) { mi_set_error("whole-integration kernel launch failed: %s", hipGetErrorString(e)); return MI_ODE_E_HIP; }
diff --git a/tfdiffeq_amd/csrc/mi_ode_linadj.hip b/tfdiffeq_amd/csrc/mi_ode_linadj.hip
--- a/tfdiffeq_amd/csrc/mi_ode_linadj.hip
+++ b/tfdiffeq_amd/csrc/mi_ode_linadj.hip
@@ -5,6 +5,7 @@
 #include <string.h>
 #include "mi_ode_handoff_host.h"
 #include "mi_ode_linadj.h"
+#include "mi_ode_linear_poly_host.h"
 
 using namespace mi;
 
@@ -40,17 +41,6 @@
 }
 
 int la_pad_dim(int dim) { return dim <= 16 ? 16 : (dim <= 32 ? 32 : (dim <= 64 ? 64 : 128)); }
-
-void stage_polynomials(const mi_ode_tableau& tb, double (*pi)[kLaP]) {
-  for (int s = 0; s < kLaP; ++s)
-    for (int p = 0; p < kLaP; ++p) pi[s][p] = 0.0;
-  pi[0][0] = 1.0;
-  for (int s = 1; s <= kLaS; ++s) {
-    pi[s][0] = 1.0;
-    for (int j = 0; j < s; ++j)
-      for (int p = 1; p < kLaP; ++p) pi[s][p] += tb.beta[s - 1][j] * pi[j][p - 1];
-  }
-}
 
 }
 
@@ -121,7 +111,7 @@
   if (e == hipSuccess) e = hipMemset(h->cvec, 0, kLaP * D * sizeof(double));
   if (e == hipSuccess) e = hipMemset(h->lmat, 0, kLaP * D * D * sizeof(double));
   double pi[kLaP][kLaP], ktab[4][kLaPP];
-  stage_polynomials(tb, pi);
+  stage_polynomials<kLaP>(tb, kLaS, pi);
   for (int p = 0; p < kLaP; ++p)
     for (int q = 0; q < kLaP; ++q) {
       double ks = 0.0, ke = 0.0, km = 0.0;
diff --git a/tfdiffeq_amd/csrc/mi_ode_linear_poly.h b/tfdiffeq_amd/csrc/mi_ode_linear_poly.h
--- /dev/null
+++ b/tfdiffeq_amd/csrc/mi_ode_linear_poly.h
@@ -0,0 +1,230 @@
+#pragma once
+
+namespace mi {
+
+constexpr int kPolyP = 7;
+constexpr int kLinNDense = 2;
+template <typename T, int D, int S, bool TS>
+constexpr bool lin_poly_capable() { return sizeof(T) == 8 && D <= 128 && S == 6 && !TS; }
+
+struct LinPowJob {
+  const void* a;
+  const void* b;
+  void* rm;
+  void* pk;
+  int lda, ldb, ar, pad_;
+};
+constexpr int kLinPowJobs = 6;
+struct LinPowArgs {
+  LinPowJob job[kLinPowJobs];
+  int dim;
+};
+struct LinPowLayout {
+  static constexpr size_t rm(int D, int p) { return (size_t)p * D * D; }
+  static constexpr size_t pk(int D, int p) { return (size_t)(8 + p - 1) * D * D; }
+  static constexpr size_t q(int D, int p) { return (size_t)15 * D * D + (size_t)p * D; }
+  static constexpr size_t g(int D) { return (size_t)15 * D * D + (size_t)8 * D; }
+  static constexpr size_t count(int D) { return g(D) + 32; }
+};
+
+template <typename T, int D>
+__global__ __launch_bounds__(256) void k_lin_powers(LinPowArgs A) {
+  constexpr int VEC = MfmaTraits<T>::VEC, KS = D / 4, NCH = KS / VEC;
+  const LinPowJob& J = A.job[blockIdx.y];
+  const int e = blockIdx.x * 256 + threadIdx.x;
+  const int r = e / D, c = e % D;
+  if (r >= (J.pk != nullptr ? D : 1)) return;
+  const T* a = (const T*)J.a;
+  const T* b = (const T*)J.b;
+  T acc = (T)0;
+  if (r < J.ar && c < A.dim) {
+    if (a == nullptr) acc = b[(long long)r * J.ldb + c];
+    else
+      for (int k = 0; k < A.dim; ++k) acc = __builtin_fma(a[(long long)r * J.lda + k], b[(long long)k * J.ldb + c], acc);
+  }
+  if (J.rm != nullptr) ((T*)J.rm)[r * D + c] = acc;
+  if (J.pk != nullptr) {
+    const int lg = r / KS, s = r % KS, m = s / VEC, v = s % VEC, w = c / 16, li = c % 16;
+    ((T*)J.pk)[(((w * NCH + m) * 64) + lg * 16 + li) * VEC + v] = acc;
+  }
+}
+
+template <typename T, int D, bool TWO>
+__device__ __forceinline__ void lin_poly_slice(const LinCtx<T, D>& cx, const T* pk, const T* qv, const T (&a0)[kPolyP], const T (&a1)[kPolyP],
+                                               T (&sl0)[D / 4], T (&sl1)[TWO ? D / 4 : 1], T& r0, T& r1) {
+  using CH = typename LinCtx<T, D>::CH;
+  constexpr int KS = D / 4, VEC = LinCtx<T, D>::VEC, NCH = KS / VEC;
+  const CH* m = (const CH*)pk + cx.wave * (NCH * 64) + cx.lane;
+  int dep[2] = {0, 0};
+  asm volatile("" : "+v"(dep[0]), "+v"(dep[1]));
+#pragma unroll
+  for (int c = 0; c < NCH; ++c) {
+    CH v[kPolyP];
+    const CH* mc = m + dep[c & 1];
+#pragma unroll
+    for (int p = 0; p < kPolyP; ++p) v[p] = mc[(size_t)p * (D * D / VEC) + c * 64];
+#pragma unroll
+    for (int q = 0; q < VEC; ++q) {
+      T s0 = (T)0, s1 = (T)0;
+#pragma unroll
+      for (int p = 0; p < kPolyP; ++p) {
+        s0 = __builtin_fma(a0[p], v[p].v[q], s0);
+        if constexpr (TWO) s1 = __builtin_fma(a1[p], v[p].v[q], s1);
+      }
+      sl0[c * VEC + q] = s0;
+      if constexpr (TWO) sl1[c * VEC + q] = s1;
+    }
+    asm volatile("" : "+v"(dep[c & 1]) : "v"(sl0[c * VEC + VEC - 1]));
+  }
+  r0 = (T)0; r1 = (T)0;
+  if (qv != nullptr) {
+#pragma unroll
+    for (int p = 0; p < kPolyP; ++p) {
+      const T qp = qv[p * D + cx.col];
+      r0 = __builtin_fma(a0[p], qp, r0);
+      if constexpr (TWO) r1 = __builtin_fma(a1[p], qp, r1);
+    }
+  }
+}
+
+template <typename T, int D, bool SC0, bool TWO, class F>
+__device__ __forceinline__ void lin_poly_sweep(long long batch, const T* y0, LinCtx<T, D>& cx, __attribute__((address_space(3))) T* lds,
+                                               const T (&c0)[D / 4], const T (&c1)[TWO ? D / 4 : 1], int blk, int nblk, F&& emit) {
+  using TR = MfmaTraits<T>;
+  using acc_t = typename TR::acc_t;
+  typedef __attribute__((address_space(3))) T lds_T;
+  typedef T vec_t __attribute__((ext_vector_type(MfmaTraits<T>::VEC)));
+  typedef __attribute__((address_space(3))) vec_t lds_vec;
+  constexpr int R_ = LinCtx<T, D>::R_, KS = LinCtx<T, D>::KS, VEC = LinCtx<T, D>::VEC, LD = LinCtx<T, D>::LD, TILE = LinCtx<T, D>::TILE;
+  const long long ntiles = (batch + R_ - 1) / R_;
+  T y0n[4];
+  auto fetch = [&](long long t_i) {
+    const T* ty = y0 + t_i * R_ * cx.d;
+    const int nr = cx.rows_here(t_i, batch);
+#pragma unroll
+    for (int i = 0; i < 4; ++i) y0n[i] = (cx.row_of(i) < nr && cx.colok) ? stream_load<SC0>(ty + cx.off_of(i)) : (T)0;
+  };
+  if ((long long)blk < ntiles) fetch(blk);
+  for (long long tile_i = blk; tile_i < ntiles; tile_i += nblk) {
+    T y0e[4];
+#pragma unroll
+    for (int i = 0; i < 4; ++i) y0e[i] = y0n[i];
+    if (tile_i + nblk < ntiles) fetch(tile_i + nblk);
+    lds_T* tile = lds + cx.cur * TILE;
+    const lds_T* ap = tile + cx.li * LD + cx.lg * KS;
+    cx.cur ^= 1;
+#pragma unroll
+    for (int i = 0; i < 4; ++i) tile[TR::acc_row(cx.lane, i) * LD + cx.col] = y0e[i];
+    lds_barrier();
+    acc_t s0 = {0, 0, 0, 0}, s1 = {0, 0, 0, 0};
+#pragma unroll
+    for (int m = 0; m < KS / VEC; ++m) {
+      const vec_t a0 = *(const lds_vec*)(ap + m * VEC);
+#pragma unroll
+      for (int v = 0; v < VEC; ++v) {
+        s0 = TR::mfma(a0[v], c0[m * VEC + v], s0);
+        if constexpr (TWO) s1 = TR::mfma(a0[v], c1[m * VEC + v], s1);
+      }
+    }
+    const int nr = cx.rows_here(tile_i, batch);
+#pragma unroll
+    for (int i = 0; i < 4; ++i)
+      if (cx.row_of(i) < nr && cx.colok) emit(tile_i, i, y0e[i], s0[i], s1[i]);
+  }
+}
+
+struct LinPolyArgs {
+  const void* pk;
+  const void* qv;
+  const double* g;
+  const void* y0;
+  void* y1;
+  void* out;
+  const double* t_out;
+  long long n_plane, batch;
+  double sh;
+  double t_start, t_new;
+  int dim, j_lo, j_hi, cur, blk, nblk;
+  unsigned lds;
+};
+struct LinPolyOut { double maxa, maxb, suma; int cur; };
+
+template <typename T, int D, bool SC0>
+__device__ __forceinline__ LinPolyOut lin_poly_attempt_pass(LinPolyArgs Q) {
+  constexpr int R_ = LinCtx<T, D>::R_, KS = LinCtx<T, D>::KS;
+  const T* pk = uniform_p((const T*)Q.pk);
+  const T* qv = uniform_p((const T*)Q.qv);
+  const double* g = uniform_p(Q.g);
+  const T* y0 = uniform_p((const T*)Q.y0);
+  T* y1 = uniform_p((T*)Q.y1);
+  T* outp = uniform_p((T*)Q.out);
+  const double* t_out = uniform_p(Q.t_out);
+  const long long n_plane = ((long long)uniform_i((int)(Q.n_plane >> 32)) << 32) | (unsigned)uniform_i((int)Q.n_plane);
+  const long long batch = ((long long)uniform_i((int)(Q.batch >> 32)) << 32) | (unsigned)uniform_i((int)Q.batch);
+  const double t_start = uniform_d(Q.t_start), t_new = uniform_d(Q.t_new);
+  const int j_lo = uniform_i(Q.j_lo), j_hi = uniform_i(Q.j_hi), blk = uniform_i(Q.blk), nblk = uniform_i(Q.nblk);
+  typedef __attribute__((address_space(3))) T lds_T;
+  lds_T* const lds = (lds_T*)(size_t)(unsigned)uniform_i((int)Q.lds);
+  LinCtx<T, D> cx;
+  cx.init_geometry(nullptr, uniform_i(Q.dim), uniform_i(Q.cur));
+  Acc acc;
+  T sp[kPolyP];
+  sp[0] = (T)uniform_d(Q.sh);
+#pragma unroll
+  for (int p = 1; p < kPolyP; ++p) sp[p] = sp[p - 1] * sp[0];
+  {
+    T a_sol[kPolyP], a_err[kPolyP], c_sol[KS], c_err[KS], r_sol, r_err;
+#pragma unroll
+    for (int p = 0; p < kPolyP; ++p) { a_sol[p] = (T)g[p] * sp[p]; a_err[p] = (T)g[8 + p] * sp[p]; }
+    lin_poly_slice<T, D, true>(cx, pk, qv, a_sol, a_err, c_sol, c_err, r_sol, r_err);
+    lin_poly_sweep<T, D, SC0, true>(batch, y0, cx, lds, c_sol, c_err, blk, nblk, [&](long long tile_i, int i, T y0e, T s_sol, T s_err) {
+      const T yn = y0e + (s_sol + r_sol);
+      const T err = s_err + r_err;
+      (y1 + tile_i * R_ * cx.d)[cx.off_of(i)] = yn;
+      acc.maxa = fmax(acc.maxa, (double)fabs(y0e));
+      acc.maxb = fmax(acc.maxb, (double)fabs(yn));
+      acc.suma += (double)err * (double)err;
+    });
+  }
+  for (int j = j_lo; j < j_hi; ++j) {
+    const T x = (T)uniform_d((double)interp_x<T>(t_start, t_new, t_out[j]));
+    const T x2 = x * x, x3 = x2 * x, x4 = x3 * x;
+    const T p1 = (T)-8 * x4 + (T)14 * x3 - (T)5 * x2, pm = (T)16 * x4 - (T)32 * x3 + (T)16 * x2;
+    const T p0 = (T)-2 * x4 + (T)5 * x3 - (T)4 * x2 + x, pS = (T)2 * x4 - (T)3 * x3 + x2;
+    T a_w[kPolyP], c_w[KS], r_w;
+#pragma unroll
+    for (int p = 0; p < kPolyP; ++p) {
+      T gw = p1 * (T)g[p] + pm * (T)g[16 + p] + pS * (T)g[24 + p];
+      if (p == 0) gw = gw + p0;
+      a_w[p] = gw * sp[p];
+    }
+    T none[1] = {(T)0}, r_none;
+    lin_poly_slice<T, D, false>(cx, pk, qv, a_w, a_w, c_w, none, r_w, r_none);
+    T* out = outp + (long long)j * n_plane;
+    lin_poly_sweep<T, D, SC0, false>(batch, y0, cx, lds, c_w, none, blk, nblk, [&](long long tile_i, int i, T y0e, T s_w, T) {
+      (out + tile_i * R_ * cx.d)[cx.off_of(i)] = y0e + (s_w + r_w);
+    });
+  }
+  LinPolyOut o;
+  o.maxa = acc.maxa; o.maxb = acc.maxb; o.suma = acc.suma; o.cur = cx.cur;
+  return o;
+}
+
+template <typename T, int D, int S, bool SC0>
+__device__ __forceinline__ void lin_poly_attempt(const StepArgs& A, const StepPlanes<T, S>& P, LinCtx<T, D>& cx, Acc& acc, const double* t_out,
+                                                 int blk = (int)blockIdx.x, int nblk = (int)gridDim.x) {
+  static_assert(S + 1 == kPolyP && !LinCtx<T, D>::STREAM, "six-row pair on the resident-slice widths");
+  LinPolyArgs Q;
+  Q.pk = A.poly_pk; Q.qv = cx.has_bias ? A.poly_q : nullptr; Q.g = A.poly_g;
+  Q.y0 = P.y0; Q.y1 = P.y1; Q.out = A.out; Q.t_out = t_out;
+  Q.lds = (unsigned)(size_t)(__attribute__((address_space(3))) char*)cx.s_ys;
+  Q.n_plane = A.n_plane; Q.batch = A.batch;
+  Q.sh = (double)(cx.sign * P.hs);
+  Q.t_start = P.t_start; Q.t_new = P.t_new;
+  Q.dim = cx.d; Q.j_lo = P.j_lo; Q.j_hi = P.j_hi; Q.cur = cx.cur; Q.blk = blk; Q.nblk = nblk;
+  const LinPolyOut o = lin_poly_attempt_pass<T, D, SC0>(Q);
+  acc.maxa = fmax(acc.maxa, o.maxa); acc.maxb = fmax(acc.maxb, o.maxb); acc.suma += o.suma;
+  cx.cur = o.cur;
+}
+
+}
diff --git a/tfdiffeq_amd/csrc/mi_ode_linear_poly_host.h b/tfdiffeq_amd/csrc/mi_ode_linear_poly_host.h
--- /dev/null
+++ b/tfdiffeq_amd/csrc/mi_ode_linear_poly_host.h
@@ -0,0 +1,54 @@
+#pragma once
+#include <math.h>
+#include "../../include/mi_ode.h"
+
+namespace mi {
+
+template <int P>
+inline void stage_polynomials(const mi_ode_tableau& tb, int S, double (*pi)[P]) {
+  for (int s = 0; s < P; ++s)
+    for (int p = 0; p < P; ++p) pi[s][p] = 0.0;
+  pi[0][0] = 1.0;
+  for (int s = 1; s <= S && s < P; ++s) {
+    pi[s][0] = 1.0;
+    for (int j = 0; j < s; ++j)
+      for (int p = 1; p < P; ++p) pi[s][p] += tb.beta[s - 1][j] * pi[j][p - 1];
+  }
+}
+
+constexpr int kLinPolyP = 8;
+
+struct LinPolyTables {
+  int n;
+  double g_sol[kLinPolyP];
+  double g_err[kLinPolyP];
+  double g_mid[kLinPolyP];
+  double pi_last[kLinPolyP];
+  int err_zeroed[kLinPolyP];
+};
+
+inline bool lin_poly_tables(const mi_ode_tableau& tb, LinPolyTables* out) {
+  const int S = tb.n_stages;
+  if (S < 1 || S >= kLinPolyP) return false;
+  double pi[kLinPolyP][kLinPolyP];
+  stage_polynomials<kLinPolyP>(tb, S, pi);
+  out->n = S + 1;
+  for (int p = 0; p < kLinPolyP; ++p) {
+    double gs = 0.0, ge = 0.0, gm = 0.0, ae = 0.0;
+    for (int s = 0; s <= S; ++s) {
+      gs += tb.c_sol[s] * pi[s][p];
+      ge += tb.c_error[s] * pi[s][p];
+      ae += fabs(tb.c_error[s] * pi[s][p]);
+      gm += tb.c_mid[s] * pi[s][p];
+    }
+    const bool residue = fabs(ge) <= 16.0 * 1.1102230246251565e-16 * ae;
+    out->g_sol[p] = gs;
+    out->g_err[p] = residue ? 0.0 : ge;
+    out->err_zeroed[p] = (residue && p <= S) ? 1 : 0;
+    out->g_mid[p] = gm;
+    out->pi_last[p] = pi[S][p];
+  }
+  return true;
+}
+
+}
diff --git a/tfdiffeq_amd/csrc/mi_ode_persist.h b/tfdiffeq_amd/csrc/mi_ode_persist.h
--- a/tfdiffeq_amd/csrc/mi_ode_persist.h
+++ b/tfdiffeq_amd/csrc/mi_ode_persist.h
@@ -131,20 +131,6 @@
   return (unsigned)(w0 >> 32) == seq && (unsigned)(w1 >> 32) == seq;
 }
 
-__device__ __forceinline__ int uniform_i(int v) { return __builtin_amdgcn_readfirstlane(v); }
-__device__ __forceinline__ double uniform_d(double v) {
-  const long long b = __double_as_longlong(v);
-  const unsigned lo = (unsigned)__builtin_amdgcn_readfirstlane((int)(unsigned)b);
-  const unsigned hi = (unsigned)__builtin_amdgcn_readfirstlane((int)(unsigned)((unsigned long long)b >> 32));
-  return __longlong_as_double((long long)(((unsigned long long)hi << 32) | lo));
-}
-template <typename P>
-__device__ __forceinline__ P* uniform_p(P* p) {
-  const unsigned long long b = (unsigned long long)p;
-  const unsigned lo = (unsigned)__builtin_amdgcn_readfirstlane((int)(unsigned)b);
-  const unsigned hi = (unsigned)__builtin_amdgcn_readfirstlane((int)(unsigned)(b >> 32));
-  return (P*)(((unsigned long long)hi << 32) | lo);
-}
 
 struct PersistPub {
   double dt, t1, emit_t0, emit_t1, emit_dt;
@@ -797,8 +783,9 @@
   }
 }
 
-template <typename T, int D, int S, bool TS>
+template <typename T, int D, int S, bool TS, bool POLY = false>
 __global__ __launch_bounds__(D * 4) void k_persist_linear_mfma(PersistArgs A) {
+  static_assert(!POLY || lin_poly_capable<T, D, S, TS>(), "no polynomial pass for this instantiation");
   extern __shared__ __attribute__((aligned(16))) char smem_raw[];
   __shared__ PersistShared sh;
   Ctl& s_c = sh.c;
@@ -866,6 +853,7 @@
 
   const T* cur_y = y_user;
   T* cur_f = fa;
+  bool f_stale = false;
   while (!uniform_i(sh.pub.done)) {
     StepPlanes<T, S> P;
     const double dt_u = uniform_d(sh.pub.dt), t1_u = uniform_d(sh.pub.t1);
@@ -881,7 +869,19 @@
     if (blockIdx.x == 0 && (threadIdx.x == 0 || threadIdx.x == 256) && gen == 3u) { cx.tr = (long long*)(A.s.partials + 8192) + (threadIdx.x ? 256 : 0); cx.tn = 0; }
     else cx.tr = nullptr;
 #endif
-    lin_attempt_pass<T, D, S, TS, true>(A.s, P, cx, acc, t_out, (T*)sh.coef);
+    const int n_in = P.j_hi - P.j_lo;
+    bool poly = false;
+    if constexpr (POLY) poly = lin_takes_poly(n_in, cp);
+    if constexpr (POLY) {
+      if (poly) {
+        lin_poly_attempt<T, D, S, true>(A.s, P, cx, acc, t_out);
+      } else {
+        cx.reload_w(A.s.rhs);
+        lin_attempt_pass<T, D, S, TS, true>(A.s, P, cx, acc, t_out, (T*)sh.coef, (int)blockIdx.x, (int)gridDim.x, f_stale);
+      }
+    } else {
+      lin_attempt_pass<T, D, S, TS, true>(A.s, P, cx, acc, t_out, (T*)sh.coef);
+    }
 #ifdef MI_TRACE
     if (cx.tr != nullptr) {
       for (int q = 0; q + 3 < cx.tn && q < 4 * 14; q += 4)
@@ -900,12 +900,20 @@
     if (threadIdx.x == 0) {
       AttemptState st = sh.st;
       if (!ok) { st.status |= MI_ODE_ST_SYNC_TIMEOUT; st.done = 1; st.accepted = 0; }
-      else { fill_record(rec, r, n_tot); attempt_core(st, rec, cp); }
+      else {
+        fill_record(rec, r, n_tot);
+        attempt_core(st, rec, cp);
+        if (cp.lin_poly) lin_count_attempt(st, n_in, poly, cp);
+      }
       publish(st);
       sh.st = st;
     }
     __syncthreads();
-    if (uniform_i(sh.pub.accepted)) { cur_y = P.y1; cur_f = P.f1; }
+    if (uniform_i(sh.pub.accepted)) {
+      cur_y = P.y1;
+      if (!poly) cur_f = P.f1;
+      f_stale = poly;
+    }
   }
 
   if (cur_y == y_user) {
diff --git a/tfdiffeq_amd/csrc/mi_ode_step_fused.h b/tfdiffeq_amd/csrc/mi_ode_step_fused.h
--- a/tfdiffeq_amd/csrc/mi_ode_step_fused.h
+++ b/tfdiffeq_amd/csrc/mi_ode_step_fused.h
@@ -31,7 +31,25 @@
   RhsParams rhs;
   unsigned* ticket;
   CtrlParams cp;
+  const void* poly_pk;
+  const void* poly_q;
+  const double* poly_g;
 };
+
+__device__ __forceinline__ int uniform_i(int v) { return __builtin_amdgcn_readfirstlane(v); }
+__device__ __forceinline__ double uniform_d(double v) {
+  const long long b = __double_as_longlong(v);
+  const unsigned lo = (unsigned)__builtin_amdgcn_readfirstlane((int)(unsigned)b);
+  const unsigned hi = (unsigned)__builtin_amdgcn_readfirstlane((int)(unsigned)((unsigned long long)b >> 32));
+  return __longlong_as_double((long long)(((unsigned long long)hi << 32) | lo));
+}
+template <typename P>
+__device__ __forceinline__ P* uniform_p(P* p) {
+  const unsigned long long b = (unsigned long long)p;
+  const unsigned lo = (unsigned)__builtin_amdgcn_readfirstlane((int)(unsigned)b);
+  const unsigned hi = (unsigned)__builtin_amdgcn_readfirstlane((int)(unsigned)(b >> 32));
+  return (P*)(((unsigned long long)hi << 32) | lo);
+}
 
 __device__ __forceinline__ void finish_attempt(const StepArgs& A, const Acc& acc, double* red) {
   if (A.ticket == nullptr) {
@@ -383,6 +401,24 @@
     plain = bias == nullptr && sgn == 1.0;
     s_ys = lds;
   }
+  __device__ __forceinline__ void reload_w(const RhsParams& rhs) {
+    static_assert(!STREAM, "streamed W has no resident slice");
+    const T* W = (const T*)rhs.w[0];
+    const int cc = colok ? col : 0;
+#pragma unroll
+    for (int s = 0; s < KS; ++s) {
+      const int kk = lg * KS + s, kc = kk < d ? kk : 0;
+      const T v = W[(long long)kc * d + cc];
+      bf[s] = (colok && kk < d) ? v : (T)0;
+    }
+  }
+  __device__ __forceinline__ void init_geometry(T* lds, int dim, int cur_) {
+    const int tid = threadIdx.x;
+    lane = tid & 63; wave = tid >> 6; li = lane & 15; lg = lane >> 4;
+    col = 16 * wave + li;
+    d = dim; colok = col < dim;
+    s_ys = lds; cur = cur_;
+  }
   __device__ __forceinline__ void init_padded(const T* Mpad, const T* bias, double sgn, T* lds, int dim) {
     static_assert(!STREAM, "streamed W: init() takes the packed copy");
     const int tid = threadIdx.x;
@@ -534,7 +570,7 @@
 template <typename T, int D, int S, bool TS, bool SC0>
 __device__ __forceinline__ void lin_attempt_pass(const StepArgs& A, const StepPlanes<T, S>& P, LinCtx<T, D>& cx, Acc& acc,
                                                  const double* t_out, T* coef , int blk = (int)blockIdx.x,
-                                                 int nblk = (int)gridDim.x) {
+                                                 int nblk = (int)gridDim.x, bool k1_stale = false) {
   constexpr int R_ = LinCtx<T, D>::R_;
   using CF = LinCoef<S>;
   const long long ntiles = (A.batch + R_ - 1) / R_;
@@ -550,7 +586,7 @@
     for (int i = 0; i < 4; ++i) {
       const bool ok = cx.row_of(i) < nr && cx.colok && !(MI_ABL & 8);
       y0n[i] = ok ? stream_load<SC0>(ty + cx.off_of(i)) : (T)0;
-      f0n[i] = ok ? stream_load<SC0>(tf + cx.off_of(i)) : (T)0;
+      f0n[i] = (ok && !k1_stale) ? stream_load<SC0>(tf + cx.off_of(i)) : (T)0;
     }
   };
   if (PF && (long long)blk < ntiles) fetch(blk);
@@ -564,6 +600,11 @@
 #pragma unroll
     for (int i = 0; i < 4; ++i) { y0e[i] = y0n[i]; k[0][i] = f0n[i]; }
     if (PF && tile_i + nblk < ntiles) fetch(tile_i + nblk);
+    if (k1_stale) {
+      cx.rhs_eval(y0e, k[0]);
+      lds_barrier();
+      cx.cur ^= 1;
+    }
 
     auto stage = [&](auto sg_c) {
       constexpr int SG = decltype(sg_c)::value;
@@ -626,6 +667,10 @@
   }
 }
 
+}
+#include "mi_ode_linear_poly.h"
+namespace mi {
+
 template <typename T, int D, bool SC0, bool DOT = false>
 __device__ __forceinline__ void lin_f0_pass(const StepArgs& A, const T* y0, T* f0_out, T* copy_a, T* copy_b, LinCtx<T, D>& cx,
                                             Acc& acc, int blk = (int)blockIdx.x, int nblk = (int)gridDim.x, const T* gdot = nullptr,
@@ -708,17 +753,30 @@
   }
 }
 
-template <typename T, int D, int S, bool TS>
+template <typename T, int D, int S, bool TS, bool POLY = false>
 __global__ __launch_bounds__(D * 4) void k_step_linear_mfma(StepArgs A) {
+  static_assert(!POLY || lin_poly_capable<T, D, S, TS>(), "no polynomial pass for this instantiation");
   StepPlanes<T, S> P;
   if (!resolve_step<T, S>(A, P)) return;
   extern __shared__ __attribute__((aligned(16))) char smem_raw[];
   T* s_ys = (T*)smem_raw;
   double* red = (double*)(s_ys + LinCtx<T, D>::kBufs * LinCtx<T, D>::TILE);
   LinCtx<T, D> cx;
-  cx.init(A.rhs, s_ys, A.dim);
   Acc acc;
-  lin_attempt_pass<T, D, S, TS, false>(A, P, cx, acc, A.t_out, (T*)(red + 80));
+  if constexpr (POLY) {
+    const int n_in = P.j_hi - P.j_lo;
+    if (lin_takes_poly(n_in, A.cp)) {
+      cx.init_geometry(s_ys, A.dim, 0);
+      cx.has_bias = A.rhs.b[0] != nullptr; cx.sign = (T)A.rhs.sign;
+      lin_poly_attempt<T, D, S, false>(A, P, cx, acc, A.t_out);
+    } else {
+      cx.init(A.rhs, s_ys, A.dim);
+      lin_attempt_pass<T, D, S, TS, false>(A, P, cx, acc, A.t_out, (T*)(red + 80), (int)blockIdx.x, (int)gridDim.x, A.ctl->f_stale != 0);
+    }
+  } else {
+    cx.init(A.rhs, s_ys, A.dim);
+    lin_attempt_pass<T, D, S, TS, false>(A, P, cx, acc, A.t_out, (T*)(red + 80));
+  }
   finish_attempt(A, acc, red);
 }
 
diff --git a/tfdiffeq_amd/solvers.py b/tfdiffeq_amd/solvers.py
--- a/tfdiffeq_amd/solvers.py
+++ b/tfdiffeq_amd/solvers.py
@@ -358,6 +358,9 @@
         self._raise_for_status(rc)
         return out
 
+    def matrix_products(self):
+        return int(self.lib.mi_ode_matrix_products(self.h))
+
     def profile(self):
         out = (C.c_double * 4)()
         N.check(self.lib.mi_ode_get_profile(self.h, out), 'mi_ode_get_profile')
@@ -868,6 +871,7 @@
             out = eng.integrate(t.to(torch.float64).numpy(), self.y0[0] if self._packed is None else self._packed[0])
         finally:
             self.stats = eng.stats.as_dict()
+            self.stats['matrix_products'] = eng.matrix_products()
             self.stats['cross_rank'] = eng.transport
             if eng.transport_log:
                 self.stats['cross_rank_log'] = list(eng.transport_log)
```

Result: slower. 6.229 billion (-4.1%).
